# FrozenWolf-Cyber/Indic-CL-ASR

Measured on AMD Instinct MI355X. Metric: utterances/sec (15 s @16 kHz) Conformer-M RNNT-CTC+EWC train step, higher is better.
Workload: dtype bf16; 1 GPU; BASELINE configs[1]: Conformer-medium (d=256, 16L, H=640) hybrid RNNT-CTC + EWC, bs=32/GPU x 15 s, bf16 projections, freeze_encoder_till=12, 22x257 heads, fused_batch_size=4; global_batch=32, parallelism=dp1

## Files before the change

### include/indicasr.h

```cpp
#ifndef INDICASR_H
#define INDICASR_H

#include <stddef.h>
#include <stdint.h>

#ifdef __cplusplus
extern "C" {
#endif

typedef void* ia_stream_t;

enum ia_status {
    IA_OK = 0,
    IA_INVALID_VALUE = -1,
    IA_WORKSPACE_TOO_SMALL = -2,
    IA_LAUNCH_FAILED = -3,
    IA_UNSUPPORTED = -4,
};

const char* ia_version(void);

size_t ia_rnnt_workspace_bytes(int B, int T, int U1);
int ia_rnnt_loss(const float* logits, const int64_t* labels, const int64_t* act_lens, const int64_t* label_lens,
                 int B, int T, int U1, int V, int blank, float fastemit_lambda, float clamp,
                 float* costs, float* grads, void* workspace, size_t workspace_bytes, ia_stream_t stream);
int ia_rnnt_forward(const float* logits, const int64_t* labels, const int64_t* act_lens, const int64_t* label_lens,
                    int B, int T, int U1, int V, int blank, float fastemit_lambda, int need_backward, float* costs,
                    void* workspace, size_t workspace_bytes, ia_stream_t stream);
int ia_rnnt_backward(const float* logits, const int64_t* labels, const int64_t* act_lens, const int64_t* label_lens,
                     int B, int T, int U1, int V, int blank, float fastemit_lambda, float clamp,
                     const float* cost_grad, float* grads, void* workspace, size_t workspace_bytes, ia_stream_t stream,
                     void* grad_kernel_start_event, void* grad_kernel_stop_event);
int ia_rnnt_export_alphas_betas(const void* workspace, size_t workspace_bytes, const int64_t* act_lens,
                                const int64_t* label_lens, int B, int T, int U1, float* alphas, float* betas,
                                ia_stream_t stream);

int ia_joint_ld(int V);
int ia_joint_fwd(const void* f, const void* g, const void* W, const float* bias, const int64_t* labels,
                 const int64_t* act_lens, const int64_t* label_lens, int B, int T, int U1, int H, int V, int blank,
                 float dropout_p, unsigned seed, void* logits, int LD, void* workspace, size_t workspace_bytes,
                 ia_stream_t stream);
int ia_joint_fwd_box(const void* f, const void* g, const void* W, const float* bias, const int64_t* labels,
                     const int64_t* act_lens, const int64_t* label_lens, const int64_t* box_t, const int64_t* box_u, int B,
                     int T, int U1, int H, int V, int blank, float dropout_p, unsigned seed, void* logits, int LD,
                     void* workspace, size_t workspace_bytes, ia_stream_t stream);
int64_t ia_joint_extra_scratch_elems(void);
int ia_joint_extra_reduce(const void* logits, const void* teacher, const int64_t* box_t, const int64_t* box_u,
                          const float* w_sq, const float* w_kd, int B, int T, int U1, int V, int LD, float* sums4,
                          float* scratch, ia_stream_t stream);
int ia_joint_extra_grad(const void* logits, const void* teacher, const int64_t* box_t, const int64_t* box_u, const float* w_sq,
                        const float* w_kd, const float* upstream2, int B, int T, int U1, int V, int LD, void* E,
                        ia_stream_t stream);
int ia_lattice_add_f16(void* G, const void* E, int64_t n, ia_stream_t stream);
int ia_rnnt_lattice(const int64_t* act_lens, const int64_t* label_lens, int B, int T, int U1, float fastemit_lambda,
                    int need_backward, float* costs, void* workspace, size_t workspace_bytes, ia_stream_t stream);
int ia_joint_backward_g(void* logits_inout, const int64_t* labels, const int64_t* act_lens, const int64_t* label_lens,
                        int B, int T, int U1, int V, int LD, int blank, float fastemit_lambda, const float* cost_grad,
                        float kappa, void* gt_out, int S, int Kc, float* dbias_out, float* dbias_scratch, void* workspace,
                        size_t workspace_bytes, ia_stream_t stream, void* grad_kernel_start_event,
                        void* grad_kernel_stop_event);
int ia_joint_backward_g_skip(void* logits_inout, const int64_t* labels, const int64_t* act_lens, const int64_t* label_lens, int B,
                             int T, int U1, int V, int LD, int blank, float fastemit, const float* cost_grad, float kappa,
                             void* gt_out, int S, int Kc, float* dbias_out, float* dbias_scratch, void* workspace,
                             size_t workspace_bytes, int skip_dead_frames, ia_stream_t stream, void* ev_start, void* ev_stop);
int64_t ia_joint_backward_g_dbias_scratch_elems(int LD);
int ia_joint_hidden_t(const void* f, const void* g, void* hidden_t, int B, int T, int U1, int H, int LDH, int S, int Kc,
                      float dropout_p, unsigned seed, ia_stream_t stream);
int ia_joint_hidden(const void* f, const void* g, void* hidden, int B, int T, int U1, int H, int LDH, float dropout_p,
                    unsigned seed, ia_stream_t stream);
int ia_joint_dh_reduce(const void* dh, const void* f, const void* g, const int64_t* act_lens,
                       const int64_t* label_lens, float* df, float* dg, int B, int T, int U1, int H, float inv_kappa,
                       float dropout_p, unsigned seed, void* scratch, ia_stream_t stream);
size_t ia_joint_dh_reduce_scratch_bytes(int B, int T, int U1, int H);
int ia_joint_dh_fused_supported(int U1, int H, int LD);
int ia_joint_dh_k(void);
size_t ia_joint_dh_fused_scratch_bytes(int B, int T, int U1, int H);
int ia_joint_dh_fused(const void* G, const void* Wt, const void* f, const void* g, const int64_t* act_lens,
                      const int64_t* label_lens, float* df, float* dg, int B, int T, int U1, int H, int LD,
                      float inv_kappa, float dropout_p, unsigned seed, void* scratch, ia_stream_t stream);
int ia_joint_dh_fused_ex(const void* G, const void* Wt, const void* f, const void* g, const int64_t* act_lens,
                         const int64_t* label_lens, float* df, float* dg, void* df_bf16, void* dg_bf16, int zero_dead_df, int B,
                         int T, int U1, int H, int LD, float inv_kappa, float dropout_p, unsigned seed, void* scratch,
                         ia_stream_t stream);
int ia_joint_dw_fused_supported(int U1, int H, int LD);
int64_t ia_joint_dw_fused_scratch_elems(int B, int T, int U1, int H, int LD);
int ia_joint_dw_fused(const void* G, const void* f, const void* g, const int64_t* act_lens, int B, int T, int U1, int H, int LD,
                      float dropout_p, unsigned seed, float* dW, float* scratch, ia_stream_t stream);
int ia_joint_dw_fused_ex(const void* G, const void* f, const void* g, const int64_t* act_lens, const int64_t* label_lens, int B,
                         int T, int U1, int H, int LD, float dropout_p, unsigned seed, float* dW, float* scratch,
                         ia_stream_t stream);

int ia_gemm_bf16(const void* A, int lda, const void* W, int ldw, int M, int N, int K, const float* bias, int act,
                 float dropout_p, unsigned seed, float alpha, const float* R, int ldr, float* outF, int ldof,
                 void* outH, int ldoh, ia_stream_t stream);
int ia_gemm_bf16_ex(const void* A, int lda, const void* W, int ldw, int M, int N, int K, const float* bias, int act,
                    float dropout_p, unsigned seed, float alpha, const float* R, int ldr, float* outF, int ldof, void* outH,
                    int ldoh, void* out_pre, int ldpre, const void* aux, int ldaux, ia_stream_t stream);
int ia_gemm_bf16_ex2(const void* A, int lda, const void* W, int ldw, int M, int N, int K, const float* bias, int act,
                     float dropout_p, unsigned seed, float alpha, const float* R, int ldr, float* outF, int ldof, void* outH,
                     int ldoh, void* out_pre, int ldpre, const void* aux, int ldaux, int flags, ia_stream_t stream);
int ia_quantize_mxfp8(const void* x, int is_f32, int ld, int64_t M, int K, void* q, int ldq, void* scales, int lds, ia_stream_t stream);
int ia_gemm_mxfp8(const void* Aq, int lda, const void* a_scales, int ldsa, const void* Wq, int ldw, const void* w_scales, int ldsw,
                  int M, int N, int K, const float* bias, int act, float dropout_p, unsigned seed, float alpha, const float* R, int ldr,
                  float* outF, int ldof, void* outH, int ldoh, ia_stream_t stream);

int ia_greedy_decode_lds_bytes(int Hp, int Hj, int V);
int ia_greedy_rnnt_decode(const float* f_all, const int64_t* out_len, const float* EW, const float* Whh, const float* Wpred,
                          const float* bpred, const float* Whead, const float* bhead, int B, int T, int Hp, int Hj, int V,
                          int blank, int row_blank, int row_sos, int max_symbols, int* tokens, int cap, int* counts,
                          int* overflow, ia_stream_t stream);
int ia_greedy_rnnt_decode_bf16w(const float* f_all, const int64_t* out_len, const float* EW, const void* Whh_bf16,
                                const void* Wpred_bf16, const float* bpred, const void* Whead_bf16, const float* bhead, int B, int T,
                                int Hp, int Hj, int V, int blank, int row_blank, int row_sos, int max_symbols, int* tokens, int cap,
                                int* counts, int* overflow, ia_stream_t stream);
size_t ia_greedy_decode_scratch_bytes(int B, int Hp, int Hj);
int ia_greedy_decode_cluster(int B, int Hp, int Hj);
int ia_greedy_rnnt_decode_bf16w_ex(const float* f_all, const int64_t* out_len, const float* EW, const void* Whh_bf16,
                                   const void* Wpred_bf16, const float* bpred, const void* Whead_bf16, const float* bhead, int B,
                                   int T, int Hp, int Hj, int V, int blank, int row_blank, int row_sos, int max_symbols, int* tokens,
                                   int cap, int* counts, int* overflow, int cluster, void* scratch, size_t scratch_bytes,
                                   ia_stream_t stream);

int ia_edit_distance_batch(const int32_t* a, const int64_t* a_off, const int32_t* b, const int64_t* b_off, int n, int64_t* out);

int ia_quantize_fp8_rows(const void* x, int is_f32, int ld, int64_t M, int K, void* q, int ldq, float* scale, ia_stream_t stream);
int ia_gemm_fp8(const void* Aq, int lda, const float* a_scale, const void* Wq, int ldw, const float* w_scale, int M, int N, int K,
                const float* bias, int act, float dropout_p, unsigned seed, float alpha, const float* R, int ldr, float* outF,
                int ldof, void* outH, int ldoh, ia_stream_t stream);
int ia_subsample_conv1(const float* feats, int B, int Fm, int Tm, int C, const float* w1, const float* b1, void* out,
                       ia_stream_t stream);
int ia_subsample_conv2(const void* in_cl, int B, int T1, int F1, int C, const void* w2r, const float* b2, int N, void* out,
                       ia_stream_t stream);
int ia_gemm_bf16_ln_supported(int N, int K);
int ia_gemm_bf16_ln(const void* A, int lda, const void* W, int ldw, int M, int N, int K, const float* bias, float dropout_p,
                    unsigned seed, float alpha, const float* R, int ldr, float* outF, int ldof, const float* ln_g,
                    const float* ln_b, float ln_eps, void* outH, int ldoh, ia_stream_t stream);
int ia_layernorm(const float* x, int ldx, int N, int d, const float* g1, const float* b1, float eps, float* outF,
                 int ldf, const float* g2, const float* b2, void* outH, int ldh, ia_stream_t stream);
int ia_glu_dwconv(const void* x2, const int64_t* lens, int B, int T, int d, int ksz, const float* w, const float* bias,
                  float* z, float* bn_sum, float* bn_sumsq, float* scratch, ia_stream_t stream);
int64_t ia_dwconv_scratch_elems(int B, int T, int d, int ksz);
int ia_colsum_bf16(const void* x, int M, int N, int ld, float* out, ia_stream_t stream);
int ia_dwconv_time(const float* x, int B, int T, int d, int ksz, const float* w, const float* bias, int flip, float* y,
                   ia_stream_t stream);
int ia_dwconv_time_wgrad(const float* x, const float* dy, int B, int T, int d, int ksz, float* dw, float* db,
                         float* scratch, ia_stream_t stream);
int ia_dwconv_glu_bwd(const float* dz, const void* c2, const int64_t* lens, int B, int T, int d, int ksz, const float* w, void* dc2,
                      ia_stream_t stream);
int ia_dwconv_glu_wgrad(const void* c2, const int64_t* lens, const float* dy, int B, int T, int d, int ksz, float* dw, float* db,
                        float* scratch, ia_stream_t stream);
int ia_bn_silu(const float* z, int64_t n_rows, int d, const float* bn_sum, const float* bn_sumsq, const float* gamma,
               const float* beta, float* running_mean, float* running_var, int64_t* num_batches_tracked,
               float momentum, float eps, int training, void* out, ia_stream_t stream);

int ia_gemm_bnsilu_supported(int K);
int ia_gemm_bnsilu_bf16(const float* z, int ldz, int64_t n_rows, const float* bn_sum, const float* bn_sumsq,
                        const float* gamma, const float* beta, float* running_mean, float* running_var,
                        int64_t* num_batches_tracked, float momentum, float eps, int training, const void* W, int ldw, int M,
                        int N, int K, const float* bias, float dropout_p, unsigned seed, float alpha, const float* R, int ldr,
                        float* outF, int ldof, void* outH, int ldoh, const long long* bn_sums_fixed, ia_stream_t stream);
int ia_gemm_bnsilu_bf16_keep(const float* z, int ldz, int64_t n_rows, const float* bn_sum, const float* bn_sumsq,
                             const float* gamma, const float* beta, float* running_mean, float* running_var,
                             int64_t* num_batches_tracked, float momentum, float eps, int training, const void* W, int ldw, int M,
                             int N, int K, const float* bias, float dropout_p, unsigned seed, float alpha, const float* R, int ldr,
                             float* outF, int ldof, void* outH, int ldoh, const long long* bn_sums_fixed, void* outA, int ldoa,
                             ia_stream_t stream);
int ia_dwconv_gated_fixed(const void* g, const int64_t* lens, int B, int T, int d, int ksz, const float* w, const float* bias,
                          float* z, long long* bn_sums_fixed, ia_stream_t stream);
int ia_glu_dwconv_fixed(const void* x2, const int64_t* lens, int B, int T, int d, int ksz, const float* w, const float* bias,
                        float* z, long long* bn_sums_fixed, ia_stream_t stream);

int ia_relpos_attention_flash_supported(int T, int dk);
int ia_relpos_attention_flash(const void* qkv, const void* pos_proj, const float* bias_u, const float* bias_v,
                              const int64_t* lens, int B, int T, int H, int dk, float dropout_p, unsigned seed, void* ctx,
                              ia_stream_t stream);
int ia_relpos_attention_flash_lse(const void* qkv, const void* pos_proj, const float* bias_u, const float* bias_v,
                                  const int64_t* lens, int B, int T, int H, int dk, float dropout_p, unsigned seed, void* ctx,
                                  float* lse, ia_stream_t stream);
int ia_relpos_attention_local_supported(int T, int dk, int window);
int ia_relpos_attention_local(const void* qkv, const void* pos_proj, const float* bias_u, const float* bias_v,
                              const int64_t* lens, int B, int T, int H, int dk, int window, float dropout_p, unsigned seed,
                              void* ctx, ia_stream_t stream);
int ia_relpos_attention_local_lse(const void* qkv, const void* pos_proj, const float* bias_u, const float* bias_v,
                                  const int64_t* lens, int B, int T, int H, int dk, int window, float dropout_p, unsigned seed,
                                  void* ctx, float* lse, ia_stream_t stream);
int ia_relpos_attention_flash_bwd_dims(int T, int* Rs, int* pad0);
int64_t ia_relpos_attention_flash_bwd_ws_elems(int B, int T, int H, int dk);
int ia_relpos_attention_flash_bwd(const void* qkv, const void* pos_proj, const float* bias_u, const float* bias_v,
                                  const int64_t* lens, const void* ctx, const void* dctx, const float* lse, int B, int T, int H,
                                  int dk, float dropout_p, unsigned seed, void* dqkv, void* dpl, int pl_rows, float* dbias_u,
                                  float* dbias_v, void* dBand, void* QvHM, float* ws, ia_stream_t stream);
int ia_relpos_attention_local_bwd_dims(int T, int window, int* Rs, int* pad0);
int64_t ia_relpos_attention_local_bwd_ws_elems(int B, int T, int H, int dk, int window);
int ia_relpos_attention_local_bwd(const void* qkv, const void* pos_proj, const float* bias_u, const float* bias_v,
                                  const int64_t* lens, const void* ctx, const void* dctx, const float* lse, int B, int T, int H,
                                  int dk, int window, float dropout_p, unsigned seed, void* dqkv, void* dpl, int pl_rows,
                                  float* dbias_u, float* dbias_v, void* dBand, void* QvHM, float* ws, ia_stream_t stream);
int ia_relpos_attention_context_supported(int T, int dk, int style, int left, int right);
int ia_relpos_attention_context(const void* qkv, const void* pos_proj, const float* bias_u, const float* bias_v,
                                const int64_t* lens, int B, int T, int H, int dk, int style, int left, int right,
                                float dropout_p, unsigned seed, void* ctx, ia_stream_t stream);
int ia_relpos_attention_context_lse(const void* qkv, const void* pos_proj, const float* bias_u, const float* bias_v,
                                    const int64_t* lens, int B, int T, int H, int dk, int style, int left, int right,
                                    float dropout_p, unsigned seed, void* ctx, float* lse, ia_stream_t stream);
int ia_relpos_attention_context_bwd_dims(int T, int style, int left, int right, int* Rs, int* pad0);
int64_t ia_relpos_attention_context_bwd_ws_elems(int B, int T, int H, int dk, int style, int left, int right);
int ia_relpos_attention_context_bwd(const void* qkv, const void* pos_proj, const float* bias_u, const float* bias_v,
                                    const int64_t* lens, const void* ctx, const void* dctx, const float* lse, int B, int T, int H,
                                    int dk, int style, int left, int right, float dropout_p, unsigned seed, void* dqkv, void* dpl,
                                    int pl_rows, float* dbias_u, float* dbias_v, void* dBand, void* QvHM, float* ws,
                                    ia_stream_t stream);
size_t ia_attn_vt_elems(int B, int T, int H);
int ia_relpos_attention(const void* qkv, const void* pos_proj, const float* bias_u, const float* bias_v,
                        const int64_t* lens, int B, int T, int H, int dk, float dropout_p, unsigned seed,
                        void* vt_scratch, void* ctx, ia_stream_t stream);

size_t ia_lstm_scratch_bytes(int B, int H);
int ia_lstm_lds_bytes(int H, int backward);
int ia_lstm_forward(const float* Gx, const void* Whh_bf16, float* Hout, float* gates, float* Cs, int U, int B, int H,
                    void* scratch, size_t scratch_bytes, ia_stream_t stream);
int ia_lstm_backward(const float* dHout, const float* gates, const float* Cs, const void* WhhT_bf16, float* dG, int U,
                     int B, int H, void* scratch, size_t scratch_bytes, ia_stream_t stream);

int ia_feat_frames(const float* audio, int B, int L, int Tm, int win, int n_fft, int hop, float preemph, float dither,
                   unsigned seed, float* frames, int ldf, ia_stream_t stream);
int ia_gemm_f32(const float* A, int lda, const float* W, int ldw, int M, int N, int K, float* C, int ldc,
                ia_stream_t stream);
int ia_feat_power(const float* spec, int64_t M, int lds, int half, int nbins, float* power, int ldp, ia_stream_t stream);
int ia_feat_logmel_t(const float* mel, int B, int Tm, int F, int ldm, float guard, float* out, ia_stream_t stream);
int ia_feat_preemph(const float* audio, int B, int L, float preemph, float dither, unsigned seed, float* y,
                    ia_stream_t stream);
int ia_feat_logmel_fft_supported(int n_fft, int win, int n_mels, int n_chunks);
int ia_feat_logmel_fft(const float* y, int B, int L, int Tm, const float* window, int win, int n_fft, int hop,
                       const float* twiddle, const int* chunk_start, const float* chunk_vals, const int* filt_chunks,
                       int n_mels, int n_chunks, float guard, float* out, ia_stream_t stream);
int ia_feat_normalize(const float* x, const int64_t* seq_len, int B, int F, int T, float eps, const int* freq_starts,
                      const int* freq_widths, int n_freq_masks, const int* time_starts, const int* time_widths,
                      int n_time_masks, float mask_value, float* y, ia_stream_t stream);

size_t ia_ctc_workspace_bytes(int B, int T, int S);
int ia_ctc_forward(const float* log_probs, const int64_t* targets, const int64_t* input_lens, const int64_t* target_lens,
                   int B, int T, int V, int S, int blank, int zero_infinity, float* nll, void* workspace,
                   size_t workspace_bytes, ia_stream_t stream);
int ia_ctc_backward(const float* log_probs, const int64_t* targets, const int64_t* input_lens, const int64_t* target_lens,
                    int B, int T, int V, int S, int blank, const float* nll_grad, float* grad, void* workspace,
                    size_t workspace_bytes, ia_stream_t stream);

typedef struct ia_tn_problem {
    const void* dY; const void* X; float* dW; float* db;
    int ldy, ldx, M, n, k;
} ia_tn_problem;
int64_t ia_gemm_tn_grouped_scratch_elems(const ia_tn_problem* problems, int count);
int ia_gemm_tn_bf16_grouped(const ia_tn_problem* problems, int count, float* scratch, ia_stream_t stream);
int64_t ia_gemm_tn_scratch_elems(int M, int n, int k);
int ia_gemm_tn_bf16(const void* dY, int ldy, const void* X, int ldx, int M, int n, int k, float* dW, float* db,
                    float* scratch, ia_stream_t stream);

int ia_ffn_fused_supported(int d, int d_ff);
int ia_ffn_fused(float* x, int N, int d, int d_ff, const float* ln_g, const float* ln_b, float eps, const void* W1,
                 const float* b1, const void* W2, const float* b2, float alpha, float p_ff, unsigned seed_ff, float p_res,
                 unsigned seed_res, const float* ln2_g, const float* ln2_b, void* y_out, int ln2_to_y_only,
                 ia_stream_t stream);
int ia_ffn_fused_tail_supported(int d, int d_ff, int nt);
int ia_ffn_fused_tail(float* x, int N, int d, int d_ff, const float* ln_g, const float* ln_b, float eps, const void* W1,
                      const float* b1, const void* W2, const float* b2, float alpha, float p_ff, unsigned seed_ff, float p_res,
                      unsigned seed_res, const float* ln2_g, const float* ln2_b, void* y_out, int ln2_to_y_only, const void* Wt,
                      const float* bt, void* t_out, int nt, ia_stream_t stream);

typedef struct ia_block_params {
    const void *w_ff1a, *w_ff1b, *w_qkv, *w_pos, *w_out, *w_pw1, *w_pw2, *w_ff2a, *w_ff2b;
    const float *b_ff1a, *b_ff1b, *b_qkv, *b_out, *b_pw1, *b_pw2, *b_ff2a, *b_ff2b;
    const float *ln_ff1_g, *ln_ff1_b, *ln_att_g, *ln_att_b, *ln_conv_g, *ln_conv_b, *ln_ff2_g, *ln_ff2_b, *ln_out_g, *ln_out_b;
    const float *pos_u, *pos_v, *dw_w, *dw_b, *bn_g, *bn_b;
    float *bn_rm, *bn_rv;
    int64_t* bn_nbt;
    float ln_eps, bn_eps, bn_momentum, p_drop, p_ff, p_att, fc_factor;
    int d, d_ff, n_heads, ksz;
    const void* pl_cached;
    const void* w_pw1_glu;
    const float* b_pw1_glu;
    int att_window;
    int att_style;
    int att_left, att_right;
} ia_block_params;
size_t ia_conformer_prefix_ws_bytes(int B, int T, int d, int d_ff, int H, int ksz, int pos_rows);
int ia_conformer_prefix_fwd(const ia_block_params* layers, int n_layers, float* x, const void* pos_emb, int pos_rows,
                            const int64_t* lens, int B, int T, unsigned seed_base, unsigned seed_stride, int training,
                            void* workspace, size_t workspace_bytes, ia_stream_t stream);
size_t ia_conformer_prefix_ws_sums_offset(int B, int T, int d, int d_ff, int H, int ksz, int pos_rows);
int ia_conformer_prefix_fwd_seg(const ia_block_params* layers, int n_layers, float* x, const void* pos_emb, int pos_rows,
                                const int64_t* lens, int B, int T, unsigned seed_base, unsigned seed_stride, int training,
                                int seg_begin, int seg_end, int bn_synced, void* workspace, size_t workspace_bytes,
                                ia_stream_t stream);

typedef struct ia_block_saved {
    void *y1, *h1p, *h1; float* x1;
    void *y2, *qkv, *pl, *ctxv; float* x2;
    void *y3, *c2; float *z, *sums; void* c3; float* x3;
    void *y4, *h4p, *h4; float* x4;
    float* lse;
} ia_block_saved;
typedef struct ia_block_grads {
    float *w_ff1a, *b_ff1a, *w_ff1b, *b_ff1b, *w_qkv, *b_qkv, *w_pos, *w_out, *b_out, *w_pw1, *b_pw1, *w_pw2, *b_pw2;
    float *w_ff2a, *b_ff2a, *w_ff2b, *b_ff2b;
    float *ln_ff1_g, *ln_ff1_b, *ln_att_g, *ln_att_b, *ln_conv_g, *ln_conv_b, *ln_ff2_g, *ln_ff2_b, *ln_out_g, *ln_out_b;
    float *dw_w, *dw_b, *bn_g, *bn_b;
} ia_block_grads;
struct ia_block_params;
int ia_conformer_block_supported(int d, int d_ff, int H, int ksz, int T);
size_t ia_conformer_block_bwd_ws_bytes(int B, int T, int d, int d_ff, int ksz);
int ia_conformer_block_fwd(const struct ia_block_params* layer, const float* x0, const void* pos_emb, int pos_rows,
                           const int64_t* lens, int B, int T, unsigned seed, const ia_block_saved* saved, float* out,
                           float* dw_scratch, ia_stream_t stream);
int ia_conformer_block_bwd_a(const struct ia_block_params* layer, const ia_block_saved* saved, const ia_block_grads* grads,
                             const float* dout, const int64_t* lens, int B, int T, unsigned seed, void* workspace,
                             size_t workspace_bytes, float** dx2_out, void** dctx_out, ia_stream_t stream);
int ia_conformer_block_fwd_phase(const struct ia_block_params* layer, const float* x0, const void* pos_emb, int pos_rows,
                                 const int64_t* lens, int B, int T, unsigned seed, const ia_block_saved* saved, float* out,
                                 float* dw_scratch, int phase, ia_stream_t stream);
int ia_conformer_block_bwd_a_phase(const struct ia_block_params* layer, const ia_block_saved* saved, const ia_block_grads* grads,
                                   const float* dout, const int64_t* lens, int B, int T, unsigned seed, void* workspace,
                                   size_t workspace_bytes, float** dx2_out, void** dctx_out, int phase, const float* bn_S12,
                                   ia_stream_t stream);
int ia_conformer_block_bwd_b(const struct ia_block_params* layer, const ia_block_saved* saved, const ia_block_grads* grads,
                             const float* x0, const void* pos_emb, int pos_rows, const void* dqkv, const void* dpl, int B,
                             int T, unsigned seed, void* workspace, size_t workspace_bytes, float* dx0,
                             const void* add_table, int n_add, ia_stream_t stream);

int ia_layernorm_bwd(const float* x, int ldx, const float* dy_f32, const void* dy_bf16, int ldy, int N, int d,
                     const float* gamma, float eps, const float* dx_in, float* dx_out, int lddx, float* dgamma,
                     float* dbeta, float* scratch, ia_stream_t stream);
int ia_layernorm_bwd_drop(const float* x, int ldx, const float* dy_f32, const void* dy_bf16, int ldy, int N, int d,
                          const float* gamma, float eps, const float* dx_in, float* dx_out, int lddx, float* dgamma,
                          float* dbeta, float alpha, float dropout_p, unsigned seed, void* dx_bf16, int lddxh, float* scratch,
                          ia_stream_t stream);
typedef struct ia_finish_job { const float* part; int G, C, C0; float* out0; float* out1; } ia_finish_job;
int ia_layernorm_bwd_partial_rows(int N);
int ia_partials_finish_multi(const ia_finish_job* jobs, int count, ia_stream_t stream);
int64_t ia_layernorm_bwd_scratch_elems(int N, int d);
int ia_silu_dropout(const void* h_pre, int64_t M, int N, float dropout_p, unsigned seed, void* out, ia_stream_t stream);
int ia_silu_dropout_bwd(const void* h_pre, const void* dh, int64_t M, int N, float dropout_p, unsigned seed, void* out,
                        ia_stream_t stream);
int ia_scale_dropout_bf16(const float* dy, int64_t M, int N, float alpha, float dropout_p, unsigned seed, void* out,
                          ia_stream_t stream);
int ia_cast_pad_bf16(const float* src, int lds, int64_t M, int N, void* dst, int ldd, ia_stream_t stream);
int ia_bn_silu_bwd(const float* z, const void* dc3, int64_t n_rows, int d, const float* bn_sum, const float* bn_sumsq,
                   const float* gamma, const float* beta, float eps, float* S1, float* S2, float* dz, float* scratch,
                   ia_stream_t stream);
int64_t ia_bn_silu_bwd_scratch_elems(int64_t n_rows, int d);
int ia_bn_sync_finish(float* sums_and_count, int d, int64_t n_local_rows, float* running_mean, float* running_var,
                      int64_t* num_batches_tracked, float momentum, ia_stream_t stream);
int ia_bn_silu_bwd_reduce(const float* z, const void* dc3, int64_t n_rows, int d, const float* bn_sum, const float* bn_sumsq,
                          const float* gamma, const float* beta, float eps, float* S1, float* S2, float* scratch,
                          ia_stream_t stream);
int ia_bn_silu_bwd_apply(const float* z, const void* dc3, int64_t n_rows, int d, const float* bn_sum, const float* bn_sumsq,
                         const float* gamma, const float* beta, float eps, const float* S1, const float* S2, float* dz,
                         ia_stream_t stream);
int ia_glu_mask(const void* c2, const int64_t* lens, int B, int T, int d, float* G, ia_stream_t stream);
int ia_glu_bwd(const void* c2, const float* dG, const int64_t* lens, int B, int T, int d, void* dc2, ia_stream_t stream);

int ia_cl_chunk_elems(void);
int ia_cl_penalty(const float* theta, const float* theta_star, const float* weight, float coef, float* grad,
                  int accumulate, const int32_t* chunk_table, int nchunks, const float* seg_inv_numel,
                  float* seg_abs_mean, float* penalty_sum, ia_stream_t stream);
int ia_cl_fisher_accumulate(float* fisher, const float* grad, const float* loss_scalar, int64_t n, ia_stream_t stream);
int ia_cl_abs_accumulate(float* omega, const float* grad, int64_t n, ia_stream_t stream);
int ia_adamw_step(float* theta, const float* grad, float* exp_avg, float* exp_avg_sq, int64_t n, float lr, float beta1,
                  float beta2, float eps, float weight_decay, int step, float grad_scale, void* shadow_bf16,
                  ia_stream_t stream);
int ia_adamw_step_segmented(float* theta, const float* grad, float* exp_avg, float* exp_avg_sq, const int32_t* chunk_table,
                            int nchunks, int32_t* seg_active, int32_t* seg_step, int nseg, int all_active, float lr,
                            float beta1, float beta2, float eps, float weight_decay, float grad_scale, void* shadow_bf16,
                            ia_stream_t stream);
size_t ia_grad_norm_workspace_bytes(int nchunks);
int ia_grad_norm(const float* grad, const int32_t* chunk_table, int nchunks, const int32_t* seg_chunk_begin, int nseg,
                 float grad_scale, float max_norm, int32_t* seg_active, float* seg_norm, float* norm_state, void* workspace,
                 size_t workspace_bytes, ia_stream_t stream);
int ia_adamw_step_segmented_clipped(float* theta, const float* grad, float* exp_avg, float* exp_avg_sq,
                                    const int32_t* chunk_table, int nchunks, int32_t* seg_active, int32_t* seg_step, int nseg,
                                    int all_active, float lr, float beta1, float beta2, float eps, float weight_decay,
                                    float grad_scale, void* shadow_bf16, const float* norm_state, int skip_nonfinite,
                                    int32_t* counters, ia_stream_t stream);
int ia_adamw_step_segmented_si(float* theta, const float* grad, float* exp_avg, float* exp_avg_sq, const int32_t* chunk_table,
                               int nchunks, int32_t* seg_active, int32_t* seg_step, int nseg, int all_active, float lr,
                               float beta1, float beta2, float eps, float weight_decay, float grad_scale, void* shadow_bf16,
                               const float* norm_state, int skip_nonfinite, int32_t* counters, float* path_w,
                               const float* omega, const float* theta_star, float penalty_coef, ia_stream_t stream);
int ia_si_consolidate(const float* theta, float* theta_star, float* path_w, float* omega, float xi, int64_t n,
                      ia_stream_t stream);
int ia_adamw_step_segmented_rwalk(float* theta, const float* grad, float* exp_avg, float* exp_avg_sq,
                                  const int32_t* chunk_table, int nchunks, int32_t* seg_active, int32_t* seg_step, int nseg,
                                  int all_active, float beta1, float beta2, float eps, float grad_scale, void* shadow_bf16,
                                  const int32_t* seg_group, int ngroups, const float* group_lr, const float* group_weight_decay,
                                  const float* norm_state, int skip_nonfinite, int32_t* counters, float* fisher, float* path_w,
                                  float* anchor, float* score, const float* importance, const float* theta_star,
                                  float penalty_coef, float alpha, float fold_eps, int fold, ia_stream_t stream);
size_t ia_rwalk_workspace_bytes(int nchunks);
int ia_rwalk_consolidate(const float* theta, float* theta_star, const float* fisher, float* path_w, float* anchor, float* score,
                         float* score_acc, float* importance, float* maxima, float fold_eps, int normalize, int first, int64_t n,
                         const int32_t* chunk_table, int nchunks, void* workspace, size_t workspace_bytes, ia_stream_t stream);
size_t ia_agem_workspace_bytes(int nchunks);
int ia_agem_dots(const float* grad, const float* ref, const int32_t* chunk_table, int nchunks, int nseg, float grad_scale,
                 int32_t* seg_active, float* proj_state, void* workspace, size_t workspace_bytes, ia_stream_t stream);
int ia_grad_norm_projected(const float* grad, const int32_t* chunk_table, int nchunks, const int32_t* seg_chunk_begin, int nseg,
                           float grad_scale, float max_norm, const int32_t* seg_active, float* seg_norm, float* norm_state,
                           void* workspace, size_t workspace_bytes, const float* ref, const float* proj_state,
                           ia_stream_t stream);
int ia_adamw_step_segmented_projected(float* theta, const float* grad, float* exp_avg, float* exp_avg_sq,
                                      const int32_t* chunk_table, int nchunks, int32_t* seg_active, int32_t* seg_step, int nseg,
                                      int all_active, float lr, float beta1, float beta2, float eps, float weight_decay,
                                      float grad_scale, void* shadow_bf16, const float* norm_state, int skip_nonfinite,
                                      int32_t* counters, const float* ref, const float* proj_state, int32_t* proj_counters,
                                      ia_stream_t stream);
#define IA_GEM_MAX_TASKS 16
#define IA_GEM_STATE_FLOATS 20
#define IA_GEM_SUMS_DOUBLES 272
size_t ia_gem_workspace_bytes(int nchunks, int max_tasks);
int ia_gem_dots(const float* x, const float* refs, int64_t stride, int ntasks, const int32_t* chunk_table, int nchunks, int nseg,
                float grad_scale, int32_t* seg_active, int gram_row, double* gem_sums, void* workspace, size_t workspace_bytes,
                ia_stream_t stream);
int ia_gem_solve(const double* gem_sums, float* gem_state, int ntasks, float memory_strength, float eps, ia_stream_t stream);
int ia_grad_norm_gem(const float* grad, const int32_t* chunk_table, int nchunks, const int32_t* seg_chunk_begin, int nseg,
                     float grad_scale, float max_norm, const int32_t* seg_active, float* seg_norm, float* norm_state,
                     void* workspace, size_t workspace_bytes, const float* refs, int64_t stride, int ntasks,
                     const float* gem_state, ia_stream_t stream);
int ia_adamw_step_segmented_gem(float* theta, const float* grad, float* exp_avg, float* exp_avg_sq, const int32_t* chunk_table,
                                int nchunks, int32_t* seg_active, int32_t* seg_step, int nseg, int all_active, float beta1,
                                float beta2, float eps, float grad_scale, void* shadow_bf16, const int32_t* seg_group, int ngroups,
                                const float* group_lr, const float* group_weight_decay, const float* norm_state,
                                int skip_nonfinite, int32_t* counters, const float* refs, int64_t stride, int ntasks,
                                const float* gem_state, int32_t* gem_counters, ia_stream_t stream);
#define IA_OGD_MAX_ROWS 4096
size_t ia_ogd_workspace_bytes(int nchunks, int max_rows);
int ia_ogd_dots(const float* x, const float* basis, int64_t stride, int64_t numel, int nrows, const int32_t* chunk_table,
                int nchunks, int nseg, const int32_t* seg_scope, int32_t* seg_active, int with_sq, double* dots64,
                float* dots32, void* workspace, size_t workspace_bytes, ia_stream_t stream);
int ia_ogd_project(const float* x, const float* basis, int64_t stride, int64_t numel, int nrows, const float* coef, float alpha,
                   const int32_t* chunk_table, int nchunks, int nseg, const int32_t* seg_scope, const int32_t* seg_active,
                   float* dst, ia_stream_t stream);
#define IA_MAX_PARAM_GROUPS 64
int ia_adamw_step_segmented_grouped(float* theta, const float* grad, float* exp_avg, float* exp_avg_sq,
                                    const int32_t* chunk_table, int nchunks, int32_t* seg_active, int32_t* seg_step, int nseg,
                                    int all_active, float beta1, float beta2, float eps, float grad_scale, void* shadow_bf16,
                                    const int32_t* seg_group, int ngroups, const float* group_lr,
                                    const float* group_weight_decay, const float* norm_state, int skip_nonfinite,
                                    int32_t* counters, float* path_w, const float* omega, const float* theta_star,
                                    float penalty_coef, const float* ref, const float* proj_state, int32_t* proj_counters,
                                    ia_stream_t stream);
#define IA_MASK_FREE 0
#define IA_MASK_MASKED 1
#define IA_MASK_FROZEN 2
int ia_adamw_step_segmented_masked(float* theta, const float* grad, float* exp_avg, float* exp_avg_sq, const int32_t* chunk_table,
                                   int nchunks, int32_t* seg_active, int32_t* seg_step, int nseg, int all_active, float beta1,
                                   float beta2, float eps, float grad_scale, void* shadow_bf16, const int32_t* seg_group,
                                   int ngroups, const float* group_lr, const float* group_weight_decay, const float* norm_state,
                                   int skip_nonfinite, int32_t* counters, const float* base, float* scores,
                                   const int32_t* seg_kind, float threshold, ia_stream_t stream);
int ia_mask_pack(const float* scores, const int32_t* chunk_table, int nchunks, const int32_t* seg_kind, int nseg, float threshold,
                 uint64_t* bits, int64_t nwords, int32_t* seg_kept, ia_stream_t stream);
int ia_mask_apply(float* theta, const float* base, const uint64_t* bits, int64_t nwords, const int32_t* chunk_table, int nchunks,
                  const int32_t* seg_kind, int nseg, void* shadow_bf16, ia_stream_t stream);
int ia_adamw_step_segmented_packed(float* theta, const float* grad, float* exp_avg, float* exp_avg_sq, const int32_t* chunk_table,
                                   int nchunks, int32_t* seg_active, int32_t* seg_step, int nseg, int all_active, float beta1,
                                   float beta2, float eps, float grad_scale, void* shadow_bf16, const int32_t* seg_group,
                                   int ngroups, const float* group_lr, const float* group_weight_decay, const float* norm_state,
                                   int skip_nonfinite, int32_t* counters, const uint8_t* owner, const int32_t* seg_kind,
                                   int train_owner, ia_stream_t stream);
int ia_grad_norm_packed(const float* grad, const int32_t* chunk_table, int nchunks, const int32_t* seg_chunk_begin, int nseg,
                        float grad_scale, float max_norm, int32_t* seg_active, float* seg_norm, float* norm_state,
                        void* workspace, size_t workspace_bytes, const uint8_t* owner, const int32_t* seg_kind, int train_owner,
                        ia_stream_t stream);
size_t ia_pack_prune_workspace_bytes(int nseg);
int ia_pack_prune(float* theta, float* exp_avg, float* exp_avg_sq, uint8_t* owner, const int32_t* chunk_table, int nchunks,
                  const int32_t* seg_kind, int nseg, float fraction, int task, void* shadow_bf16, int32_t* seg_counts,
                  void* workspace, size_t workspace_bytes, ia_stream_t stream);
int ia_pack_apply(float* theta, const float* base, const uint8_t* owner, const int32_t* chunk_table, int nchunks,
                  const int32_t* seg_kind, int nseg, int lo, int hi, void* shadow_bf16, ia_stream_t stream);
#define IA_LORA_MAX_RANK 64
int ia_lora_tile_rows(void);
int ia_lora_tile_cols(void);
size_t ia_lora_workspace_bytes(int64_t m, int64_t n, int rank);
int ia_lora_grad(const float* grad, const float* factors, float* factor_grad, const int64_t* tensors, int ntensors,
                 const int32_t* tiles, int ntiles, const int32_t* factor_chunk_table, int nfchunks, int rank, float scale,
                 float grad_scale, const float* norm_state, int skip_nonfinite, int all_active, int32_t* factor_active,
                 void* workspace, size_t workspace_bytes, size_t workspace_needed, ia_stream_t stream);
int ia_lora_apply(float* theta, const float* base, const float* factors, const int64_t* tensors, int ntensors,
                  const int32_t* seg_tensor, const int32_t* chunk_table, int nchunks, int nseg, int rank, float scale,
                  void* shadow_bf16, const float* norm_state, int skip_nonfinite, ia_stream_t stream);
int ia_adamw_step_segmented_kinds(float* theta, const float* grad, float* exp_avg, float* exp_avg_sq, const int32_t* chunk_table,
                                  int nchunks, int32_t* seg_active, int32_t* seg_step, int nseg, int all_active, float beta1,
                                  float beta2, float eps, float grad_scale, void* shadow_bf16, const int32_t* seg_group,
                                  int ngroups, const float* group_lr, const float* group_weight_decay, const float* norm_state,
                                  int skip_nonfinite, int32_t* counters, const int32_t* seg_kind, int flags_preset,
                                  ia_stream_t stream);
#define IA_MERGE_MAX_TASKS 32
int ia_merge_linear(float* theta, const float* base, const float* vectors, int64_t stride, int ntasks, const float* coef,
                    float scale, const int32_t* chunk_table, int nchunks, void* shadow_bf16, ia_stream_t stream);
size_t ia_merge_trim_workspace_bytes(int ntasks, int nscope);
int ia_merge_trim(const float* vectors, int64_t stride, int ntasks, const int32_t* chunk_table, int nchunks,
                  const int32_t* seg_of_scope, int nscope, float trim, uint32_t* cutoffs, void* workspace,
                  size_t workspace_bytes, ia_stream_t stream);
int ia_merge_ties(float* theta, const float* base, const float* vectors, int64_t stride, int ntasks, const uint32_t* cutoffs,
                  const int32_t* seg_of_scope, int nscope, float scale, const int32_t* chunk_table, int nchunks, int nseg,
                  void* shadow_bf16, int32_t* seg_counts, ia_stream_t stream);
int ia_merge_fisher(float* theta, const float* base, const float* vectors, const float* importances, int64_t stride, int ntasks,
                    const float* coef, float floor, float scale, const int32_t* chunk_table, int nchunks, int nseg,
                    void* shadow_bf16, int32_t* seg_counts, ia_stream_t stream);
int ia_merge_linear_dare(float* theta, const float* base, const float* vectors, int64_t stride, int ntasks, const float* coef,
                         float scale, const int32_t* chunk_table, int nchunks, void* shadow_bf16, uint32_t seed,
                         uint32_t keep_threshold, float keep_prob, ia_stream_t stream);
int ia_merge_ties_dare(float* theta, const float* base, const float* vectors, int64_t stride, int ntasks, float scale,
                       const int32_t* chunk_table, int nchunks, int nseg, void* shadow_bf16, int32_t* seg_counts, uint32_t seed,
                       uint32_t keep_threshold, float keep_prob, ia_stream_t stream);

typedef struct ia_wave_params {
    int32_t n_in, n_out;
    int32_t new_sr;
    int32_t shift_pre, shift_post;
    int32_t noise_shift, noise_stage;
    uint32_t noise_seed;
    float gain, noise_amp;
    int32_t pad[2];
} ia_wave_params;
int ia_wave_augment_tile(void);
int ia_wave_augment(const float* x, int B, int L_in, float* y, int L_out, const ia_wave_params* params, const float* table,
                    int zero_crossings, int sr, int min_new_sr, ia_stream_t stream);

int ia_ctc_row_lse(const float* logits, int ld, int64_t M, int V, float* lse, ia_stream_t stream);
int ia_ctc_forward_logits(const float* logits, int ld, const float* lse, const int64_t* targets, const int64_t* input_lens,
                          const int64_t* target_lens, int B, int T, int V, int S, int blank, int zero_infinity, float* nll,
                          void* workspace, size_t workspace_bytes, ia_stream_t stream);
int ia_ctc_backward_logits(const float* logits, int ld, const float* lse, const int64_t* targets, const int64_t* input_lens,
                           const int64_t* target_lens, int B, int T, int V, int S, int blank, const float* nll_grad,
                           float grad_scale, void* grad_bf16, int ldg, void* workspace, size_t workspace_bytes, ia_stream_t stream);

int ia_ctc_align_max_targets(void);
size_t ia_ctc_align_workspace_bytes(int B, int T, int S);
int ia_ctc_align(const float* lp, int ld, const float* lse, const int64_t* targets, const int64_t* input_lens,
                 const int64_t* target_lens, int B, int T, int V, int S, int blank, int32_t* path, int32_t* spans, float* score,
                 void* workspace, size_t workspace_bytes, ia_stream_t stream);

int ia_ctc_beam_max_width(void);
size_t ia_ctc_beam_workspace_bytes(int B, int T, int V, int W);
int ia_ctc_beam_search(const float* x, const float* lse, const int64_t* in_lens, int B, int T, int ld, int V, int blank, int W,
                       float token_min_logp, int32_t* tokens, int32_t* lengths, float* scores, void* workspace,
                       size_t workspace_bytes, ia_stream_t stream);

typedef struct ia_ngram_lm {
    const int32_t* states; const float* backoff; const int32_t* arcs; const float* arc_logp; const float* uni_logp;
    const int32_t* uni_next;
    int32_t n_states, n_arcs, n_tokens, order, start; float unk_logp;
} ia_ngram_lm;
int ia_ctc_beam_lm_max_order(void);
size_t ia_ctc_beam_lm_workspace_bytes(int B, int T, int V, int W);
int ia_ctc_beam_search_lm(const float* x, const float* lse, const int64_t* in_lens, int B, int T, int ld, int V, int blank, int W,
                          float token_min_logp, const ia_ngram_lm* lm, float alpha, float beta, int32_t* tokens, int32_t* lengths,
                          float* scores, void* workspace, size_t workspace_bytes, ia_stream_t stream);

typedef struct ia_axpy_row {
    float* dst; const float* src; long long n; float scale; int pad;
} ia_axpy_row;
typedef struct ia_tr_job { const void* in; void* out; int rows, cols; } ia_tr_job;
int ia_transpose16_multi(const ia_tr_job* jobs_host, int njobs, ia_stream_t stream);
int ia_swap01_cast(const void* in, int in_bf16, int n0, int n1, int H, void* out, int out_bf16, ia_stream_t stream);
int ia_select_rows_cast(const float* W, int ldw, const float* bias, int row0, int nrows, int extra_row, int K, int rows_out,
                        float scale, int out_f16, void* out, void* outT, int ldt, float* bias_out, ia_stream_t stream);
int ia_rows_scatter_add(float* dst, int ldd, const float* src, int lds, int row0, int nrows, int extra_row, int K, float scale,
                        float* bias_dst, const float* bias_src, ia_stream_t stream);
int ia_loss_combine(const float* costs, const float* nll, int B, float ctc_weight, const int* flag0, const int* flag1,
                    const int* flag2, const int* flag3, float* out4, float* total, ia_stream_t stream);
int ia_loss_combine_bwd(const float* gout, int B, float ctc_weight, float* g_costs, float* g_nll, ia_stream_t stream);
int ia_embed_sos(const float* E, const int64_t* tokens, int B, int U, int H, int n_rows, int time_major, int out_bf16, void* out,
                 ia_stream_t stream);
int ia_embed_sos_bwd(const void* dX, int dx_bf16, const int64_t* tokens, int B, int U, int H, int n_rows, int pad_row,
                     int time_major, float scale, float* dE, ia_stream_t stream);
int ia_multi_axpy(const ia_axpy_row* rows_host, int nrows, int max_blocks_per_row, ia_stream_t stream);

int ia_peak_stream_copy(const void* src, void* dst, size_t bytes, ia_stream_t stream);
int ia_peak_mfma_bf16(float* sink, int workgroups, int iters, ia_stream_t stream);
double ia_peak_mfma_bf16_flops(int workgroups, int iters);

#ifdef __cplusplus
}
#endif
#endif
```

### indic_cl_asr_amd/_lib.py

```python
import ctypes
import os
import subprocess

_HERE = os.path.dirname(os.path.abspath(__file__))
LIB_PATH = os.environ.get("IA_LIB_PATH") or os.path.join(_HERE, "libindicasr_hip.so")

IA_OK = 0
_STATUS = {-1: "IA_INVALID_VALUE", -2: "IA_WORKSPACE_TOO_SMALL", -3: "IA_LAUNCH_FAILED", -4: "IA_UNSUPPORTED"}

_c = ctypes
_vp, _i, _f, _sz = _c.c_void_p, _c.c_int, _c.c_float, _c.c_size_t
_i64 = _c.c_int64

class BlockParams(_c.Structure):
    _fields_ = ([(n, _c.c_void_p) for n in (
        "w_ff1a", "w_ff1b", "w_qkv", "w_pos", "w_out", "w_pw1", "w_pw2", "w_ff2a", "w_ff2b",
        "b_ff1a", "b_ff1b", "b_qkv", "b_out", "b_pw1", "b_pw2", "b_ff2a", "b_ff2b",
        "ln_ff1_g", "ln_ff1_b", "ln_att_g", "ln_att_b", "ln_conv_g", "ln_conv_b", "ln_ff2_g", "ln_ff2_b", "ln_out_g", "ln_out_b",
        "pos_u", "pos_v", "dw_w", "dw_b", "bn_g", "bn_b", "bn_rm", "bn_rv", "bn_nbt")]
        + [(n, _c.c_float) for n in ("ln_eps", "bn_eps", "bn_momentum", "p_drop", "p_ff", "p_att", "fc_factor")]
        + [(n, _c.c_int) for n in ("d", "d_ff", "n_heads", "ksz")]
        + [("pl_cached", _c.c_void_p), ("w_pw1_glu", _c.c_void_p), ("b_pw1_glu", _c.c_void_p), ("att_window", _c.c_int),
           ("att_style", _c.c_int), ("att_left", _c.c_int), ("att_right", _c.c_int)])


class BlockSaved(_c.Structure):
    _fields_ = [(n, _c.c_void_p) for n in ("y1", "h1p", "h1", "x1", "y2", "qkv", "pl", "ctxv", "x2", "y3", "c2", "z", "sums",
                                           "c3", "x3", "y4", "h4p", "h4", "x4", "lse")]


class TnProblem(_c.Structure):
    _fields_ = [("dY", _c.c_void_p), ("X", _c.c_void_p), ("dW", _c.c_void_p), ("db", _c.c_void_p),
                ("ldy", _c.c_int), ("ldx", _c.c_int), ("M", _c.c_int), ("n", _c.c_int), ("k", _c.c_int)]


class BlockGrads(_c.Structure):
    _fields_ = [(n, _c.c_void_p) for n in (
        "w_ff1a", "b_ff1a", "w_ff1b", "b_ff1b", "w_qkv", "b_qkv", "w_pos", "w_out", "b_out", "w_pw1", "b_pw1", "w_pw2", "b_pw2",
        "w_ff2a", "b_ff2a", "w_ff2b", "b_ff2b",
        "ln_ff1_g", "ln_ff1_b", "ln_att_g", "ln_att_b", "ln_conv_g", "ln_conv_b", "ln_ff2_g", "ln_ff2_b", "ln_out_g", "ln_out_b",
        "dw_w", "dw_b", "bn_g", "bn_b")]


class NGramLM(_c.Structure):
    _fields_ = ([(n, _c.c_void_p) for n in ("states", "backoff", "arcs", "arc_logp", "uni_logp", "uni_next")]
                + [(n, _c.c_int32) for n in ("n_states", "n_arcs", "n_tokens", "order", "start")] + [("unk_logp", _c.c_float)])


class WaveParams(_c.Structure):
    _fields_ = ([(n, _c.c_int32) for n in ("n_in", "n_out", "new_sr", "shift_pre", "shift_post", "noise_shift", "noise_stage")]
                + [("noise_seed", _c.c_uint32), ("gain", _c.c_float), ("noise_amp", _c.c_float), ("pad", _c.c_int32 * 2)])


SIGNATURES = {
    "ia_version": (_c.c_char_p, []),
    "ia_wave_augment_tile": (_i, []),
    "ia_wave_augment": (_i, [_vp, _i, _i, _vp, _i, _vp, _vp, _i, _i, _i, _vp]),
    "ia_gemm_bf16_ex2": (_i, [_vp, _i, _vp, _i, _i, _i, _i, _vp, _i, _f, _c.c_uint, _f, _vp, _i, _vp, _i, _vp, _i, _vp, _i, _vp, _i, _i, _vp]),
    "ia_transpose16_multi": (_i, [_vp, _i, _vp]),
    "ia_swap01_cast": (_i, [_vp, _i, _i, _i, _i, _vp, _i, _vp]),
    "ia_ctc_row_lse": (_i, [_vp, _i, _i64, _i, _vp, _vp]),
    "ia_ctc_forward_logits": (_i, [_vp, _i, _vp, _vp, _vp, _vp, _i, _i, _i, _i, _i, _i, _vp, _vp, _sz, _vp]),
    "ia_ctc_backward_logits": (_i, [_vp, _i, _vp, _vp, _vp, _vp, _i, _i, _i, _i, _i, _vp, _f, _vp, _i, _vp, _sz, _vp]),
    "ia_select_rows_cast": (_i, [_vp, _i, _vp, _i, _i, _i, _i, _i, _f, _i, _vp, _vp, _i, _vp, _vp]),
    "ia_rows_scatter_add": (_i, [_vp, _i, _vp, _i, _i, _i, _i, _i, _f, _vp, _vp, _vp]),
    "ia_loss_combine": (_i, [_vp, _vp, _i, _f, _vp, _vp, _vp, _vp, _vp, _vp, _vp]),
    "ia_loss_combine_bwd": (_i, [_vp, _i, _f, _vp, _vp, _vp]),
    "ia_embed_sos": (_i, [_vp, _vp, _i, _i, _i, _i, _i, _i, _vp, _vp]),
    "ia_embed_sos_bwd": (_i, [_vp, _i, _vp, _i, _i, _i, _i, _i, _i, _f, _vp, _vp]),
    "ia_multi_axpy": (_i, [_vp, _i, _i, _vp]),
    "ia_peak_stream_copy": (_i, [_vp, _vp, _sz, _vp]),
    "ia_peak_mfma_bf16": (_i, [_vp, _i, _i, _vp]),
    "ia_peak_mfma_bf16_flops": (_c.c_double, [_i, _i]),
    "ia_rnnt_workspace_bytes": (_sz, [_i, _i, _i]),
    "ia_rnnt_loss": (_i, [_vp, _vp, _vp, _vp, _i, _i, _i, _i, _i, _f, _f, _vp, _vp, _vp, _sz, _vp]),
    "ia_rnnt_forward": (_i, [_vp, _vp, _vp, _vp, _i, _i, _i, _i, _i, _f, _i, _vp, _vp, _sz, _vp]),
    "ia_rnnt_backward": (_i, [_vp, _vp, _vp, _vp, _i, _i, _i, _i, _i, _f, _f, _vp, _vp, _vp, _sz, _vp, _vp, _vp]),
    "ia_rnnt_export_alphas_betas": (_i, [_vp, _sz, _vp, _vp, _i, _i, _i, _vp, _vp, _vp]),
    "ia_joint_ld": (_i, [_i]),
    "ia_joint_fwd": (_i, [_vp, _vp, _vp, _vp, _vp, _vp, _vp, _i, _i, _i, _i, _i, _i, _f, _c.c_uint, _vp, _i, _vp, _sz, _vp]),
    "ia_joint_fwd_box": (_i, [_vp, _vp, _vp, _vp, _vp, _vp, _vp, _vp, _vp, _i, _i, _i, _i, _i, _i, _f, _c.c_uint, _vp, _i, _vp, _sz, _vp]),
    "ia_joint_extra_scratch_elems": (_i64, []),
    "ia_joint_extra_reduce": (_i, [_vp, _vp, _vp, _vp, _vp, _vp, _i, _i, _i, _i, _i, _vp, _vp, _vp]),
    "ia_joint_extra_grad": (_i, [_vp, _vp, _vp, _vp, _vp, _vp, _vp, _i, _i, _i, _i, _i, _vp, _vp]),
    "ia_lattice_add_f16": (_i, [_vp, _vp, _i64, _vp]),
    "ia_relpos_attention_flash_lse": (_i, [_vp, _vp, _vp, _vp, _vp, _i, _i, _i, _i, _f, _c.c_uint, _vp, _vp, _vp]),
    "ia_relpos_attention_flash_bwd_dims": (_i, [_i, _c.POINTER(_c.c_int), _c.POINTER(_c.c_int)]),
    "ia_relpos_attention_flash_bwd_ws_elems": (_i64, [_i, _i, _i, _i]),
    "ia_relpos_attention_flash_bwd": (_i, [_vp, _vp, _vp, _vp, _vp, _vp, _vp, _vp, _i, _i, _i, _i, _f, _c.c_uint, _vp, _vp, _i, _vp,
                                           _vp, _vp, _vp, _vp, _vp]),
    "ia_relpos_attention_local_lse": (_i, [_vp, _vp, _vp, _vp, _vp, _i, _i, _i, _i, _i, _f, _c.c_uint, _vp, _vp, _vp]),
    "ia_relpos_attention_local_bwd_dims": (_i, [_i, _i, _c.POINTER(_c.c_int), _c.POINTER(_c.c_int)]),
    "ia_relpos_attention_local_bwd_ws_elems": (_i64, [_i, _i, _i, _i, _i]),
    "ia_relpos_attention_local_bwd": (_i, [_vp, _vp, _vp, _vp, _vp, _vp, _vp, _vp, _i, _i, _i, _i, _i, _f, _c.c_uint, _vp, _vp, _i, _vp,
                                           _vp, _vp, _vp, _vp, _vp]),
    "ia_relpos_attention_context_lse": (_i, [_vp, _vp, _vp, _vp, _vp, _i, _i, _i, _i, _i, _i, _i, _f, _c.c_uint, _vp, _vp, _vp]),
    "ia_relpos_attention_context_bwd_dims": (_i, [_i, _i, _i, _i, _c.POINTER(_c.c_int), _c.POINTER(_c.c_int)]),
    "ia_relpos_attention_context_bwd_ws_elems": (_i64, [_i, _i, _i, _i, _i, _i, _i]),
    "ia_relpos_attention_context_bwd": (_i, [_vp, _vp, _vp, _vp, _vp, _vp, _vp, _vp, _i, _i, _i, _i, _i, _i, _i, _f, _c.c_uint, _vp, _vp,
                                             _i, _vp, _vp, _vp, _vp, _vp, _vp]),
    "ia_quantize_fp8_rows": (_i, [_vp, _i, _i, _i64, _i, _vp, _i, _vp, _vp]),
    "ia_gemm_fp8": (_i, [_vp, _i, _vp, _vp, _i, _vp, _i, _i, _i, _vp, _i, _f, _c.c_uint, _f, _vp, _i, _vp, _i, _vp, _i, _vp]),
    "ia_gemm_tn_grouped_scratch_elems": (_i64, [_vp, _i]),
    "ia_gemm_tn_bf16_grouped": (_i, [_vp, _i, _vp, _vp]),
    "ia_greedy_decode_lds_bytes": (_i, [_i, _i, _i]),
    "ia_greedy_rnnt_decode": (_i, [_vp, _vp, _vp, _vp, _vp, _vp, _vp, _vp, _i, _i, _i, _i, _i, _i, _i, _i, _i, _vp, _i, _vp, _vp, _vp]),
    "ia_greedy_rnnt_decode_bf16w": (_i, [_vp, _vp, _vp, _vp, _vp, _vp, _vp, _vp, _i, _i, _i, _i, _i, _i, _i, _i, _i, _vp, _i, _vp, _vp, _vp]),
    "ia_edit_distance_batch": (_i, [_vp, _vp, _vp, _vp, _i, _vp]),
    "ia_greedy_decode_scratch_bytes": (_sz, [_i, _i, _i]),
    "ia_greedy_decode_cluster": (_i, [_i, _i, _i]),
    "ia_greedy_rnnt_decode_bf16w_ex": (_i, [_vp, _vp, _vp, _vp, _vp, _vp, _vp, _vp, _i, _i, _i, _i, _i, _i, _i, _i, _i, _vp, _i, _vp, _vp, _i, _vp, _sz, _vp]),
    "ia_quantize_mxfp8": (_i, [_vp, _i, _i, _i64, _i, _vp, _i, _vp, _i, _vp]),
    "ia_gemm_mxfp8": (_i, [_vp, _i, _vp, _i, _vp, _i, _vp, _i, _i, _i, _i, _vp, _i, _f, _c.c_uint, _f, _vp, _i, _vp, _i, _vp, _i, _vp]),
    "ia_cast_pad_bf16": (_i, [_vp, _i, _i64, _i, _vp, _i, _vp]),
    "ia_rnnt_lattice": (_i, [_vp, _vp, _i, _i, _i, _f, _i, _vp, _vp, _sz, _vp]),
    "ia_joint_backward_g": (_i, [_vp, _vp, _vp, _vp, _i, _i, _i, _i, _i, _i, _f, _vp, _f, _vp, _i, _i, _vp, _vp, _vp, _sz, _vp, _vp,
                                 _vp]),
    "ia_joint_backward_g_skip": (_i, [_vp, _vp, _vp, _vp, _i, _i, _i, _i, _i, _i, _f, _vp, _f, _vp, _i, _i, _vp, _vp, _vp, _sz, _i, _vp,
                                      _vp, _vp]),
    "ia_joint_backward_g_dbias_scratch_elems": (_i64, [_i]),
    "ia_joint_hidden_t": (_i, [_vp, _vp, _vp, _i, _i, _i, _i, _i, _i, _i, _f, _c.c_uint, _vp]),
    "ia_joint_hidden": (_i, [_vp, _vp, _vp, _i, _i, _i, _i, _i, _f, _c.c_uint, _vp]),
    "ia_joint_dh_reduce": (_i, [_vp, _vp, _vp, _vp, _vp, _vp, _vp, _i, _i, _i, _i, _f, _f, _c.c_uint, _vp, _vp]),
    "ia_joint_dh_reduce_scratch_bytes": (_sz, [_i, _i, _i, _i]),
    "ia_joint_dh_fused_supported": (_i, [_i, _i, _i]),
    "ia_joint_dh_k": (_i, []),
    "ia_joint_dh_fused": (_i, [_vp, _vp, _vp, _vp, _vp, _vp, _vp, _vp, _i, _i, _i, _i, _i, _f, _f, _c.c_uint, _vp, _vp]),
    "ia_joint_dh_fused_ex": (_i, [_vp, _vp, _vp, _vp, _vp, _vp, _vp, _vp, _vp, _vp, _i, _i, _i, _i, _i, _i, _f, _f, _c.c_uint, _vp, _vp]),
    "ia_joint_dh_fused_scratch_bytes": (_sz, [_i, _i, _i, _i]),
    "ia_joint_dw_fused_supported": (_i, [_i, _i, _i]),
    "ia_joint_dw_fused_scratch_elems": (_i64, [_i, _i, _i, _i, _i]),
    "ia_joint_dw_fused": (_i, [_vp, _vp, _vp, _vp, _i, _i, _i, _i, _i, _f, _c.c_uint, _vp, _vp, _vp]),
    "ia_gemm_bf16_ln_supported": (_i, [_i, _i]),
    "ia_gemm_bf16_ln": (_i, [_vp, _i, _vp, _i, _i, _i, _i, _vp, _f, _c.c_uint, _f, _vp, _i, _vp, _i, _vp, _vp, _f, _vp, _i, _vp]),
    "ia_joint_dw_fused_ex": (_i, [_vp, _vp, _vp, _vp, _vp, _i, _i, _i, _i, _i, _f, _c.c_uint, _vp, _vp, _vp]),
    "ia_gemm_bf16": (_i, [_vp, _i, _vp, _i, _i, _i, _i, _vp, _i, _f, _c.c_uint, _f, _vp, _i, _vp, _i, _vp, _i, _vp]),
    "ia_gemm_bf16_ex": (_i, [_vp, _i, _vp, _i, _i, _i, _i, _vp, _i, _f, _c.c_uint, _f, _vp, _i, _vp, _i, _vp, _i, _vp, _i, _vp, _i, _vp]),
    "ia_subsample_conv1": (_i, [_vp, _i, _i, _i, _i, _vp, _vp, _vp, _vp]),
    "ia_subsample_conv2": (_i, [_vp, _i, _i, _i, _i, _vp, _vp, _i, _vp, _vp]),
    "ia_layernorm": (_i, [_vp, _i, _i, _i, _vp, _vp, _f, _vp, _i, _vp, _vp, _vp, _i, _vp]),
    "ia_glu_dwconv": (_i, [_vp, _vp, _i, _i, _i, _i, _vp, _vp, _vp, _vp, _vp, _vp, _vp]),
    "ia_dwconv_scratch_elems": (_i64, [_i, _i, _i, _i]),
    "ia_colsum_bf16": (_i, [_vp, _i, _i, _i, _vp, _vp]),
    "ia_dwconv_time": (_i, [_vp, _i, _i, _i, _i, _vp, _vp, _i, _vp, _vp]),
    "ia_dwconv_time_wgrad": (_i, [_vp, _vp, _i, _i, _i, _i, _vp, _vp, _vp, _vp]),
    "ia_dwconv_glu_bwd": (_i, [_vp, _vp, _vp, _i, _i, _i, _i, _vp, _vp, _vp]),
    "ia_dwconv_glu_wgrad": (_i, [_vp, _vp, _vp, _i, _i, _i, _i, _vp, _vp, _vp, _vp]),
    "ia_bn_silu": (_i, [_vp, _i64, _i, _vp, _vp, _vp, _vp, _vp, _vp, _vp, _f, _f, _i, _vp, _vp]),
    "ia_gemm_bnsilu_supported": (_i, [_i]),
    "ia_gemm_bnsilu_bf16": (_i, [_vp, _i, _i64, _vp, _vp, _vp, _vp, _vp, _vp, _vp, _f, _f, _i, _vp, _i, _i, _i, _i, _vp, _f, _c.c_uint, _f,
                                 _vp, _i, _vp, _i, _vp, _i, _vp, _vp]),
    "ia_gemm_bnsilu_bf16_keep": (_i, [_vp, _i, _i64, _vp, _vp, _vp, _vp, _vp, _vp, _vp, _f, _f, _i, _vp, _i, _i, _i, _i, _vp, _f, _c.c_uint,
                                      _f, _vp, _i, _vp, _i, _vp, _i, _vp, _vp, _i, _vp]),
    "ia_glu_dwconv_fixed": (_i, [_vp, _vp, _i, _i, _i, _i, _vp, _vp, _vp, _vp, _vp]),
    "ia_dwconv_gated_fixed": (_i, [_vp, _vp, _i, _i, _i, _i, _vp, _vp, _vp, _vp, _vp]),
    "ia_attn_vt_elems": (_sz, [_i, _i, _i]),
    "ia_relpos_attention": (_i, [_vp, _vp, _vp, _vp, _vp, _i, _i, _i, _i, _f, _c.c_uint, _vp, _vp, _vp]),
    "ia_relpos_attention_flash_supported": (_i, [_i, _i]),
    "ia_relpos_attention_flash": (_i, [_vp, _vp, _vp, _vp, _vp, _i, _i, _i, _i, _f, _c.c_uint, _vp, _vp]),
    "ia_relpos_attention_local_supported": (_i, [_i, _i, _i]),
    "ia_relpos_attention_context_supported": (_i, [_i, _i, _i, _i, _i]),
    "ia_relpos_attention_context": (_i, [_vp, _vp, _vp, _vp, _vp, _i, _i, _i, _i, _i, _i, _i, _f, _c.c_uint, _vp, _vp]),
    "ia_relpos_attention_local": (_i, [_vp, _vp, _vp, _vp, _vp, _i, _i, _i, _i, _i, _f, _c.c_uint, _vp, _vp]),
    "ia_lstm_scratch_bytes": (_sz, [_i, _i]),
    "ia_lstm_lds_bytes": (_i, [_i, _i]),
    "ia_lstm_forward": (_i, [_vp, _vp, _vp, _vp, _vp, _i, _i, _i, _vp, _sz, _vp]),
    "ia_lstm_backward": (_i, [_vp, _vp, _vp, _vp, _vp, _i, _i, _i, _vp, _sz, _vp]),
    "ia_feat_frames": (_i, [_vp, _i, _i, _i, _i, _i, _i, _f, _f, _c.c_uint, _vp, _i, _vp]),
    "ia_gemm_f32": (_i, [_vp, _i, _vp, _i, _i, _i, _i, _vp, _i, _vp]),
    "ia_feat_power": (_i, [_vp, _i64, _i, _i, _i, _vp, _i, _vp]),
    "ia_feat_logmel_t": (_i, [_vp, _i, _i, _i, _i, _f, _vp, _vp]),
    "ia_feat_preemph": (_i, [_vp, _i, _i, _f, _f, _c.c_uint, _vp, _vp]),
    "ia_feat_logmel_fft_supported": (_i, [_i, _i, _i, _i]),
    "ia_feat_logmel_fft": (_i, [_vp, _i, _i, _i, _vp, _i, _i, _i, _vp, _vp, _vp, _vp, _i, _i, _f, _vp, _vp]),
    "ia_feat_normalize": (_i, [_vp, _vp, _i, _i, _i, _f, _vp, _vp, _i, _vp, _vp, _i, _f, _vp, _vp]),
    "ia_ctc_workspace_bytes": (_sz, [_i, _i, _i]),
    "ia_ctc_forward": (_i, [_vp, _vp, _vp, _vp, _i, _i, _i, _i, _i, _i, _vp, _vp, _sz, _vp]),
    "ia_ctc_backward": (_i, [_vp, _vp, _vp, _vp, _i, _i, _i, _i, _i, _vp, _vp, _vp, _sz, _vp]),
    "ia_ctc_align_max_targets": (_i, []),
    "ia_ctc_align_workspace_bytes": (_sz, [_i, _i, _i]),
    "ia_ctc_align": (_i, [_vp, _i, _vp, _vp, _vp, _vp, _i, _i, _i, _i, _i, _vp, _vp, _vp, _vp, _sz, _vp]),
    "ia_ctc_beam_max_width": (_i, []),
    "ia_ctc_beam_workspace_bytes": (_sz, [_i, _i, _i, _i]),
    "ia_ctc_beam_search": (_i, [_vp, _vp, _vp, _i, _i, _i, _i, _i, _i, _f, _vp, _vp, _vp, _vp, _sz, _vp]),
    "ia_ctc_beam_lm_max_order": (_i, []),
    "ia_ctc_beam_lm_workspace_bytes": (_sz, [_i, _i, _i, _i]),
    "ia_ctc_beam_search_lm": (_i, [_vp, _vp, _vp, _i, _i, _i, _i, _i, _i, _f, _c.POINTER(NGramLM), _f, _f, _vp, _vp, _vp, _vp, _sz,
                                   _vp]),
    "ia_gemm_tn_scratch_elems": (_i64, [_i, _i, _i]),
    "ia_gemm_tn_bf16": (_i, [_vp, _i, _vp, _i, _i, _i, _i, _vp, _vp, _vp, _vp]),
    "ia_ffn_fused_supported": (_i, [_i, _i]),
    "ia_ffn_fused": (_i, [_vp, _i, _i, _i, _vp, _vp, _f, _vp, _vp, _vp, _vp, _f, _f, _c.c_uint, _f, _c.c_uint, _vp, _vp, _vp, _i, _vp]),
    "ia_ffn_fused_tail_supported": (_i, [_i, _i, _i]),
    "ia_ffn_fused_tail": (_i, [_vp, _i, _i, _i, _vp, _vp, _f, _vp, _vp, _vp, _vp, _f, _f, _c.c_uint, _f, _c.c_uint, _vp, _vp, _vp, _i,
                               _vp, _vp, _vp, _i, _vp]),
    "ia_conformer_prefix_ws_bytes": (_sz, [_i, _i, _i, _i, _i, _i, _i]),
    "ia_conformer_prefix_ws_sums_offset": (_sz, [_i, _i, _i, _i, _i, _i, _i]),
    "ia_conformer_prefix_fwd_seg": (_i, [_vp, _i, _vp, _vp, _i, _vp, _i, _i, _c.c_uint, _c.c_uint, _i, _i, _i, _i, _vp, _sz, _vp]),
    "ia_conformer_prefix_fwd": (_i, [_vp, _i, _vp, _vp, _i, _vp, _i, _i, _c.c_uint, _c.c_uint, _i, _vp, _sz, _vp]),
    "ia_conformer_block_supported": (_i, [_i, _i, _i, _i, _i]),
    "ia_conformer_block_bwd_ws_bytes": (_sz, [_i, _i, _i, _i, _i]),
    "ia_conformer_block_fwd": (_i, [_vp, _vp, _vp, _i, _vp, _i, _i, _c.c_uint, _vp, _vp, _vp, _vp]),
    "ia_conformer_block_fwd_phase": (_i, [_vp, _vp, _vp, _i, _vp, _i, _i, _c.c_uint, _vp, _vp, _vp, _i, _vp]),
    "ia_conformer_block_bwd_a": (_i, [_vp, _vp, _vp, _vp, _vp, _i, _i, _c.c_uint, _vp, _sz, _vp, _vp, _vp]),
    "ia_conformer_block_bwd_a_phase": (_i, [_vp, _vp, _vp, _vp, _vp, _i, _i, _c.c_uint, _vp, _sz, _vp, _vp, _i, _vp, _vp]),
    "ia_conformer_block_bwd_b": (_i, [_vp, _vp, _vp, _vp, _vp, _i, _vp, _vp, _i, _i, _c.c_uint, _vp, _sz, _vp, _vp, _i, _vp]),
    "ia_layernorm_bwd": (_i, [_vp, _i, _vp, _vp, _i, _i, _i, _vp, _f, _vp, _vp, _i, _vp, _vp, _vp, _vp]),
    "ia_layernorm_bwd_drop": (_i, [_vp, _i, _vp, _vp, _i, _i, _i, _vp, _f, _vp, _vp, _i, _vp, _vp, _f, _f, _c.c_uint, _vp, _i, _vp, _vp]),
    "ia_layernorm_bwd_partial_rows": (_i, [_i]),
    "ia_partials_finish_multi": (_i, [_vp, _i, _vp]),
    "ia_layernorm_bwd_scratch_elems": (_i64, [_i, _i]),
    "ia_silu_dropout": (_i, [_vp, _i64, _i, _f, _c.c_uint, _vp, _vp]),
    "ia_silu_dropout_bwd": (_i, [_vp, _vp, _i64, _i, _f, _c.c_uint, _vp, _vp]),
    "ia_scale_dropout_bf16": (_i, [_vp, _i64, _i, _f, _f, _c.c_uint, _vp, _vp]),
    "ia_bn_silu_bwd": (_i, [_vp, _vp, _i64, _i, _vp, _vp, _vp, _vp, _f, _vp, _vp, _vp, _vp, _vp]),
    "ia_bn_silu_bwd_scratch_elems": (_i64, [_i64, _i]),
    "ia_bn_sync_finish": (_i, [_vp, _i, _i64, _vp, _vp, _vp, _f, _vp]),
    "ia_bn_silu_bwd_reduce": (_i, [_vp, _vp, _i64, _i, _vp, _vp, _vp, _vp, _f, _vp, _vp, _vp, _vp]),
    "ia_bn_silu_bwd_apply": (_i, [_vp, _vp, _i64, _i, _vp, _vp, _vp, _vp, _f, _vp, _vp, _vp, _vp]),
    "ia_glu_mask": (_i, [_vp, _vp, _i, _i, _i, _vp, _vp]),
    "ia_glu_bwd": (_i, [_vp, _vp, _vp, _i, _i, _i, _vp, _vp]),
    "ia_cl_chunk_elems": (_i, []),
    "ia_cl_penalty": (_i, [_vp, _vp, _vp, _f, _vp, _i, _vp, _i, _vp, _vp, _vp, _vp]),
    "ia_cl_fisher_accumulate": (_i, [_vp, _vp, _vp, _i64, _vp]),
    "ia_cl_abs_accumulate": (_i, [_vp, _vp, _i64, _vp]),
    "ia_adamw_step": (_i, [_vp, _vp, _vp, _vp, _i64, _f, _f, _f, _f, _f, _i, _f, _vp, _vp]),
    "ia_adamw_step_segmented": (_i, [_vp, _vp, _vp, _vp, _vp, _i, _vp, _vp, _i, _i, _f, _f, _f, _f, _f, _f, _vp, _vp]),
    "ia_grad_norm_workspace_bytes": (_sz, [_i]),
    "ia_grad_norm": (_i, [_vp, _vp, _i, _vp, _i, _f, _f, _vp, _vp, _vp, _vp, _sz, _vp]),
    "ia_adamw_step_segmented_clipped": (_i, [_vp, _vp, _vp, _vp, _vp, _i, _vp, _vp, _i, _i, _f, _f, _f, _f, _f, _f, _vp, _vp, _i,
                                             _vp, _vp]),
    "ia_adamw_step_segmented_si": (_i, [_vp, _vp, _vp, _vp, _vp, _i, _vp, _vp, _i, _i, _f, _f, _f, _f, _f, _f, _vp, _vp, _i,
                                        _vp, _vp, _vp, _vp, _f, _vp]),
    "ia_si_consolidate": (_i, [_vp, _vp, _vp, _vp, _f, _i64, _vp]),
    "ia_adamw_step_segmented_rwalk": (_i, [_vp, _vp, _vp, _vp, _vp, _i, _vp, _vp, _i, _i, _f, _f, _f, _f, _vp, _vp, _i, _vp, _vp,
                                           _vp, _i, _vp, _vp, _vp, _vp, _vp, _vp, _vp, _f, _f, _f, _i, _vp]),
    "ia_rwalk_workspace_bytes": (_sz, [_i]),
    "ia_rwalk_consolidate": (_i, [_vp, _vp, _vp, _vp, _vp, _vp, _vp, _vp, _vp, _f, _i, _i, _i64, _vp, _i, _vp, _sz, _vp]),
    "ia_agem_workspace_bytes": (_sz, [_i]),
    "ia_agem_dots": (_i, [_vp, _vp, _vp, _i, _i, _f, _vp, _vp, _vp, _sz, _vp]),
    "ia_grad_norm_projected": (_i, [_vp, _vp, _i, _vp, _i, _f, _f, _vp, _vp, _vp, _vp, _sz, _vp, _vp, _vp]),
    "ia_adamw_step_segmented_projected": (_i, [_vp, _vp, _vp, _vp, _vp, _i, _vp, _vp, _i, _i, _f, _f, _f, _f, _f, _f, _vp, _vp, _i,
                                               _vp, _vp, _vp, _vp, _vp]),
    "ia_gem_workspace_bytes": (_sz, [_i, _i]),
    "ia_gem_dots": (_i, [_vp, _vp, _i64, _i, _vp, _i, _i, _f, _vp, _i, _vp, _vp, _sz, _vp]),
    "ia_gem_solve": (_i, [_vp, _vp, _i, _f, _f, _vp]),
    "ia_grad_norm_gem": (_i, [_vp, _vp, _i, _vp, _i, _f, _f, _vp, _vp, _vp, _vp, _sz, _vp, _i64, _i, _vp, _vp]),
    "ia_adamw_step_segmented_gem": (_i, [_vp, _vp, _vp, _vp, _vp, _i, _vp, _vp, _i, _i, _f, _f, _f, _f, _vp, _vp, _i, _vp, _vp,
                                         _vp, _i, _vp, _vp, _i64, _i, _vp, _vp, _vp]),
    "ia_ogd_workspace_bytes": (_sz, [_i, _i]),
    "ia_ogd_dots": (_i, [_vp, _vp, _i64, _i64, _i, _vp, _i, _i, _vp, _vp, _i, _vp, _vp, _vp, _sz, _vp]),
    "ia_ogd_project": (_i, [_vp, _vp, _i64, _i64, _i, _vp, _f, _vp, _i, _i, _vp, _vp, _vp, _vp]),
    "ia_adamw_step_segmented_grouped": (_i, [_vp, _vp, _vp, _vp, _vp, _i, _vp, _vp, _i, _i, _f, _f, _f, _f, _vp, _vp, _i, _vp, _vp,
                                             _vp, _i, _vp, _vp, _vp, _vp, _f, _vp, _vp, _vp, _vp]),
    "ia_adamw_step_segmented_masked": (_i, [_vp, _vp, _vp, _vp, _vp, _i, _vp, _vp, _i, _i, _f, _f, _f, _f, _vp, _vp, _i, _vp, _vp,
                                            _vp, _i, _vp, _vp, _vp, _vp, _f, _vp]),
    "ia_mask_pack": (_i, [_vp, _vp, _i, _vp, _i, _f, _vp, _i64, _vp, _vp]),
    "ia_mask_apply": (_i, [_vp, _vp, _vp, _i64, _vp, _i, _vp, _i, _vp, _vp]),
    "ia_adamw_step_segmented_packed": (_i, [_vp, _vp, _vp, _vp, _vp, _i, _vp, _vp, _i, _i, _f, _f, _f, _f, _vp, _vp, _i, _vp, _vp,
                                            _vp, _i, _vp, _vp, _vp, _i, _vp]),
    "ia_grad_norm_packed": (_i, [_vp, _vp, _i, _vp, _i, _f, _f, _vp, _vp, _vp, _vp, _sz, _vp, _vp, _i, _vp]),
    "ia_pack_prune_workspace_bytes": (_sz, [_i]),
    "ia_pack_prune": (_i, [_vp, _vp, _vp, _vp, _vp, _i, _vp, _i, _f, _i, _vp, _vp, _vp, _sz, _vp]),
    "ia_pack_apply": (_i, [_vp, _vp, _vp, _vp, _i, _vp, _i, _i, _i, _vp, _vp]),
    "ia_lora_tile_rows": (_i, []),
    "ia_lora_tile_cols": (_i, []),
    "ia_lora_workspace_bytes": (_sz, [_i64, _i64, _i]),
    "ia_lora_grad": (_i, [_vp, _vp, _vp, _vp, _i, _vp, _i, _vp, _i, _i, _f, _f, _vp, _i, _i, _vp, _vp, _sz, _sz, _vp]),
    "ia_lora_apply": (_i, [_vp, _vp, _vp, _vp, _i, _vp, _vp, _i, _i, _i, _f, _vp, _vp, _i, _vp]),
    "ia_adamw_step_segmented_kinds": (_i, [_vp, _vp, _vp, _vp, _vp, _i, _vp, _vp, _i, _i, _f, _f, _f, _f, _vp, _vp, _i, _vp, _vp,
                                           _vp, _i, _vp, _vp, _i, _vp]),
    "ia_merge_linear": (_i, [_vp, _vp, _vp, _i64, _i, _vp, _f, _vp, _i, _vp, _vp]),
    "ia_merge_trim_workspace_bytes": (_sz, [_i, _i]),
    "ia_merge_trim": (_i, [_vp, _i64, _i, _vp, _i, _vp, _i, _f, _vp, _vp, _sz, _vp]),
    "ia_merge_ties": (_i, [_vp, _vp, _vp, _i64, _i, _vp, _vp, _i, _f, _vp, _i, _i, _vp, _vp, _vp]),
    "ia_merge_fisher": (_i, [_vp, _vp, _vp, _vp, _i64, _i, _vp, _f, _f, _vp, _i, _i, _vp, _vp, _vp]),
    "ia_merge_linear_dare": (_i, [_vp, _vp, _vp, _i64, _i, _vp, _f, _vp, _i, _vp, _c.c_uint32, _c.c_uint32, _f, _vp]),
    "ia_merge_ties_dare": (_i, [_vp, _vp, _vp, _i64, _i, _f, _vp, _i, _i, _vp, _vp, _c.c_uint32, _c.c_uint32, _f, _vp]),
}

_lib = None


def build(verbose=False):
    out = None if verbose else subprocess.DEVNULL
    subprocess.check_call(["make", "-C", os.path.join(_HERE, "csrc")], stdout=out)


def lib():
    global _lib
    if _lib is None:
        if not os.path.exists(LIB_PATH):
            raise RuntimeError(
                f"{LIB_PATH} is missing: the HIP extension is the product path and has no fallback. "
                "Build it with `python -c 'import __graft_entry__ as g; g.build()'` or `make -C indic_cl_asr_amd/csrc`.")
        import torch
        l = ctypes.CDLL(LIB_PATH)
        for name, (res, args) in SIGNATURES.items():
            fn = getattr(l, name)
            fn.restype, fn.argtypes = res, args
        _lib = l
    return _lib


def check(status, what):
    if status != IA_OK:
        raise RuntimeError(f"{what} failed with status {status} ({_STATUS.get(status, 'unknown')})")


def version():
    return lib().ia_version().decode()


def stream_ptr():
    import torch
    return ctypes.c_void_p(torch.cuda.current_stream().cuda_stream)


def ptr(t):
    return ctypes.c_void_p(t.data_ptr()) if t is not None else None
```

### indic_cl_asr_amd/csrc/block_train.hip

```cpp
#include <hip/hip_bf16.h>
#include <hip/hip_runtime.h>

#include <cstdint>

#include <cstdlib>

#include "ia_common.h"

namespace {

inline size_t up256(size_t x) { return (x + 255) / 256 * 256; }

#define IA_TRY(call)                  \
    do {                              \
        const int rc_ = (call);       \
        if (rc_ != IA_OK) return rc_; \
    } while (0)

__global__ __launch_bounds__(256) void transpose_bf16_kernel(const unsigned short* __restrict__ in, int rows, int cols,
                                                             unsigned short* __restrict__ out) {
    __shared__ unsigned short tile[64][72];
    const int tiles_c = (cols + 63) / 64;
    const int tr = blockIdx.x / tiles_c, tc = blockIdx.x - tr * tiles_c;
    const int r0 = tr * 64, c0 = tc * 64;
    for (int i = threadIdx.x; i < 64 * 8; i += 256) {
        const int r = i >> 3, v = i & 7;
        uint4 x = make_uint4(0, 0, 0, 0);
        if (r0 + r < rows && c0 + v * 8 < cols) x = *reinterpret_cast<const uint4*>(in + (size_t)(r0 + r) * cols + c0 + v * 8);
        *reinterpret_cast<uint4*>(&tile[r][v * 8]) = x;
    }
    __syncthreads();
    for (int i = threadIdx.x; i < 64 * 8; i += 256) {
        const int c = i >> 3, v = i & 7;
        if (c0 + c < cols && r0 + v * 8 < rows) {
            union { uint4 u; unsigned short h[8]; } o;
#pragma unroll
            for (int j = 0; j < 8; ++j) o.h[j] = tile[v * 8 + j][c];
            *reinterpret_cast<uint4*>(out + (size_t)(c0 + c) * rows + r0 + v * 8) = o.u;
        }
    }
}

int transpose_bf16(const void* in, int rows, int cols, void* out, hipStream_t st) {
    if (rows % 8 != 0 || cols % 8 != 0) return IA_UNSUPPORTED;
    const int grid = ((rows + 63) / 64) * ((cols + 63) / 64);
    hipLaunchKernelGGL(transpose_bf16_kernel, dim3(grid), dim3(256), 0, st, (const unsigned short*)in, rows, cols, (unsigned short*)out);
    IA_RETURN_IF_LAUNCH_FAILED();
    return IA_OK;
}

struct TrJob { const unsigned short* in; unsigned short* out; int rows, cols, tile_begin, tiles_c; };
struct TrJobs { TrJob j[8]; int count; };
__global__ __launch_bounds__(256) void transpose_bf16_multi_kernel(TrJobs jobs) {
    __shared__ unsigned short tile[64][72];
    int ji = 0;
#pragma unroll
    for (int i = 1; i < 8; ++i)
        if (i < jobs.count && (int)blockIdx.x >= jobs.j[i].tile_begin) ji = i;
    const TrJob& J = jobs.j[ji];
    const int local = blockIdx.x - J.tile_begin;
    const int tr = local / J.tiles_c, tc = local - tr * J.tiles_c;
    const int r0 = tr * 64, c0 = tc * 64, rows = J.rows, cols = J.cols;
    for (int i = threadIdx.x; i < 64 * 8; i += 256) {
        const int r = i >> 3, v = i & 7;
        uint4 x = make_uint4(0, 0, 0, 0);
        if (r0 + r < rows && c0 + v * 8 < cols) x = *reinterpret_cast<const uint4*>(J.in + (size_t)(r0 + r) * cols + c0 + v * 8);
        *reinterpret_cast<uint4*>(&tile[r][v * 8]) = x;
    }
    __syncthreads();
    for (int i = threadIdx.x; i < 64 * 8; i += 256) {
        const int c = i >> 3, v = i & 7;
        if (c0 + c < cols && r0 + v * 8 < rows) {
            union { uint4 u; unsigned short h[8]; } o;
#pragma unroll
            for (int j = 0; j < 8; ++j) o.h[j] = tile[v * 8 + j][c];
            *reinterpret_cast<uint4*>(J.out + (size_t)(c0 + c) * rows + r0 + v * 8) = o.u;
        }
    }
}
struct TrList { TrJobs jobs; int tiles; };
inline void tr_add(TrList* l, const void* in, int rows, int cols, void* out) {
    TrJob& J = l->jobs.j[l->jobs.count++];
    J.in = (const unsigned short*)in; J.out = (unsigned short*)out; J.rows = rows; J.cols = cols;
    J.tile_begin = l->tiles; J.tiles_c = (cols + 63) / 64;
    l->tiles += ((rows + 63) / 64) * J.tiles_c;
}
int tr_launch(const TrList& l, hipStream_t st) {
    for (int i = 0; i < l.jobs.count; ++i)
        if (l.jobs.j[i].rows % 8 != 0 || l.jobs.j[i].cols % 8 != 0) return IA_UNSUPPORTED;
    hipLaunchKernelGGL(transpose_bf16_multi_kernel, dim3(l.tiles), dim3(256), 0, st, l.jobs);
    IA_RETURN_IF_LAUNCH_FAILED();
    return IA_OK;
}

struct AddRow { float* dst; const float* src; int64_t n; };
__global__ __launch_bounds__(256) void multi_add_kernel(const AddRow* __restrict__ table, int rows) {
    for (int k = blockIdx.y; k < rows; k += gridDim.y) {
        const AddRow r = table[k];
        const int64_t n4 = ((reinterpret_cast<uintptr_t>(r.dst) | reinterpret_cast<uintptr_t>(r.src)) & 15) ? 0 : (r.n >> 2);
        for (int64_t i = (int64_t)blockIdx.x * 256 + threadIdx.x; i < n4; i += (int64_t)gridDim.x * 256) {
            float4 a = reinterpret_cast<float4*>(r.dst)[i];
            const float4 b = reinterpret_cast<const float4*>(r.src)[i];
            a.x += b.x; a.y += b.y; a.z += b.z; a.w += b.w;
            reinterpret_cast<float4*>(r.dst)[i] = a;
        }
        for (int64_t i = (n4 << 2) + (int64_t)blockIdx.x * 256 + threadIdx.x; i < r.n; i += (int64_t)gridDim.x * 256) r.dst[i] += r.src[i];
    }
}

struct BwdWs {
    size_t dxa, dxb, dB, dB1, dB2, dB3, dh, dhp, dy, dc3, dz, dG, dc2, dctx, wt, scr, total;
};

size_t max3(size_t a, size_t b, size_t c) { return a > b ? (a > c ? a : c) : (b > c ? b : c); }

BwdWs bwd_ws(int B, int T, int d, int d_ff, int ksz) {
    const size_t N = (size_t)B * T;
    BwdWs w;
    size_t o = 0;
    w.dxa = o;  o = up256(o + N * d * 4);
    w.dxb = o;  o = up256(o + N * d * 4);
    w.dB = o;   o = up256(o + N * d * 2);
    w.dB1 = o;  o = up256(o + N * d * 2);
    w.dB2 = o;  o = up256(o + N * d * 2);
    w.dB3 = o;  o = up256(o + N * d * 2);
    w.dh = o;   o = up256(o + N * d_ff * 2);
    w.dhp = o;  o = up256(o + N * d_ff * 2);
    w.dy = o;   o = up256(o + N * d * 2);
    w.dc3 = o;  o = up256(o + N * d * 2);
    w.dz = o;   o = up256(o + N * d * 4);
    w.dG = o;   o = up256(o + (size_t)5 * (size_t)ia_layernorm_bwd_scratch_elems((int)N, d) * 4);
    w.dc2 = o;  o = up256(o + N * 2 * d * 2);
    w.dctx = o; o = up256(o + N * d * 2);
    w.wt = o;   o = up256(o + ((size_t)4 * d_ff * d + (size_t)7 * d * d) * 2);
    size_t scr = (size_t)ia_layernorm_bwd_scratch_elems((int)N, d);
    const int shapes[5][2] = {{d, d_ff}, {d_ff, d}, {d, d}, {2 * d, d}, {3 * d, d}};
    for (int i = 0; i < 5; ++i) {
        const size_t e = (size_t)ia_gemm_tn_scratch_elems((int)N, shapes[i][0], shapes[i][1]);
        scr = e > scr ? e : scr;
    }
    scr = max3(scr, (size_t)ia_bn_silu_bwd_scratch_elems((int64_t)N, d), (size_t)ia_dwconv_scratch_elems(B, T, d, ksz));
    {
        const ia_tn_problem ga[5] = {{nullptr, nullptr, nullptr, nullptr, d, d_ff, (int)N, d, d_ff},
                                     {nullptr, nullptr, nullptr, nullptr, d_ff, d, (int)N, d_ff, d},
                                     {nullptr, nullptr, nullptr, nullptr, d, d, (int)N, d, d},
                                     {nullptr, nullptr, nullptr, nullptr, 2 * d, d, (int)N, 2 * d, d},
                                     {nullptr, nullptr, nullptr, nullptr, d, d, (int)N, d, d}};
        const ia_tn_problem gb[4] = {{nullptr, nullptr, nullptr, nullptr, 3 * d, d, (int)N, 3 * d, d},
                                     {nullptr, nullptr, nullptr, nullptr, d, d, (int)(N > (size_t)64 * 512 ? N : (size_t)64 * 512), d, d},
                                     {nullptr, nullptr, nullptr, nullptr, d, d_ff, (int)N, d, d_ff},
                                     {nullptr, nullptr, nullptr, nullptr, d_ff, d, (int)N, d_ff, d}};
        scr = max3(scr, (size_t)ia_gemm_tn_grouped_scratch_elems(ga, 5), (size_t)ia_gemm_tn_grouped_scratch_elems(gb, 4));
        scr = max3(scr, (size_t)ia_gemm_tn_grouped_scratch_elems(gb, 2), (size_t)ia_gemm_tn_grouped_scratch_elems(gb + 2, 2));
        ia_tn_problem gall[9];
        for (int i = 0; i < 5; ++i) gall[i] = ga[i];
        for (int i = 0; i < 4; ++i) gall[5 + i] = gb[i];
        scr = scr > (size_t)ia_gemm_tn_grouped_scratch_elems(gall, 9) ? scr : (size_t)ia_gemm_tn_grouped_scratch_elems(gall, 9);
    }
    w.scr = o;  o = up256(o + scr * 4);
    w.total = o;
    return w;
}

int linear_bwd(const void* dY, const void* X, const void* W, int M, int n, int k, void* dX, float* dW, float* db, void* wt,
               float* scr, ia_stream_t stream) {
    if (dX) {
        IA_TRY(transpose_bf16(W, n, k, wt, (hipStream_t)stream));
        IA_TRY(ia_gemm_bf16(dY, n, wt, n, M, k, n, nullptr, 0, 0.f, 0, 1.f, nullptr, 0, nullptr, 0, dX, k, stream));
    }
    return ia_gemm_tn_bf16(dY, n, X, k, M, n, k, dW, db, scr, stream);
}

bool tn_grouping_enabled() {
    static const bool on = [] { const char* e = getenv("IA_TN_GROUPED"); return !(e && e[0] == '0'); }();
    return on;
}
int flush_group(const ia_tn_problem* grp, int ngrp, float* scr, ia_stream_t stream) {
    if (tn_grouping_enabled()) return ia_gemm_tn_bf16_grouped(grp, ngrp, scr, stream);
    for (int i = 0; i < ngrp; ++i)
        IA_TRY(ia_gemm_tn_bf16(grp[i].dY, grp[i].ldy, grp[i].X, grp[i].ldx, grp[i].M, grp[i].n, grp[i].k, grp[i].dW, grp[i].db, scr, stream));
    return IA_OK;
}
int linear_bwd_deferred(const void* dY, const void* X, const void* W, int M, int n, int k, void* dX, float* dW, float* db, const void* wt,
                        ia_tn_problem* grp, int* ngrp, ia_stream_t stream) {
    (void)W;
    if (dX) IA_TRY(ia_gemm_bf16(dY, n, wt, n, M, k, n, nullptr, 0, 0.f, 0, 1.f, nullptr, 0, nullptr, 0, dX, k, stream));
    grp[*ngrp] = ia_tn_problem{dY, X, dW, db, n, k, M, n, k};
    ++*ngrp;
    return IA_OK;
}

struct SideCtx {
    hipStream_t s = nullptr;
    hipEvent_t ev[8] = {};
    bool ok = false, tried = false;
    bool a_pending = false;
};
SideCtx* side_ctx() {
    static SideCtx ctx[16];
    const char* e = getenv("IA_WGRAD_SIDE");
    if (!(e && e[0] == '1')) return nullptr;
    int dev = 0;
    if (hipGetDevice(&dev) != hipSuccess || dev < 0 || dev >= 16) return nullptr;
    SideCtx& c = ctx[dev];
    if (!c.tried) {
        c.tried = true;
        bool ok = hipStreamCreateWithFlags(&c.s, hipStreamNonBlocking) == hipSuccess;
        for (int i = 0; ok && i < 8; ++i) ok = hipEventCreateWithFlags(&c.ev[i], hipEventDisableTiming) == hipSuccess;
        c.ok = ok;
    }
    return c.ok ? &c : nullptr;
}
struct PendingGroup { ia_tn_problem grp[8]; int n = 0; const void* ws = nullptr; };
PendingGroup* pending_group() {
    static PendingGroup pg[16];
    int dev = 0;
    if (hipGetDevice(&dev) != hipSuccess || dev < 0 || dev >= 16) return nullptr;
    return &pg[dev];
}
bool merged_wgrads() {
    const char* e = getenv("IA_TN_MERGE");
    return !(e && e[0] == '0') && tn_grouping_enabled();
}

int stream_after(hipStream_t from, hipStream_t to, hipEvent_t ev) {
    if (hipEventRecord(ev, from) != hipSuccess || hipStreamWaitEvent(to, ev, 0) != hipSuccess) return IA_LAUNCH_FAILED;
    return IA_OK;
}

}

extern "C" size_t ia_conformer_block_bwd_ws_bytes(int B, int T, int d, int d_ff, int ksz) {
    if (B <= 0 || T <= 0 || d <= 0 || d_ff <= 0 || ksz <= 0) return 0;
    return bwd_ws(B, T, d, d_ff, ksz).total;
}

extern "C" int ia_conformer_block_supported(int d, int d_ff, int H, int ksz, int T) {
    if (d <= 0 || H <= 0 || d % H != 0) return 0;
    const int dk = d / H;
    return (d % 8 == 0 && d <= 1024 && d_ff % 8 == 0 && ksz <= 31 && (ksz & 1) == 1 && dk <= 64 && dk % 4 == 0 && T >= 1) ? 1 : 0;
}

extern "C" int ia_conformer_block_fwd(const ia_block_params* Lp, const float* x0, const void* pos_emb, int pos_rows,
                                      const int64_t* lens, int B, int T, unsigned seed, const ia_block_saved* Sp, float* out,
                                      float* dw_scratch, ia_stream_t stream) {
    return ia_conformer_block_fwd_phase(Lp, x0, pos_emb, pos_rows, lens, B, T, seed, Sp, out, dw_scratch, 0, stream);
}

extern "C" int ia_conformer_block_fwd_phase(const ia_block_params* Lp, const float* x0, const void* pos_emb, int pos_rows,
                                            const int64_t* lens, int B, int T, unsigned seed, const ia_block_saved* Sp,
                                            float* out, float* dw_scratch, int phase, ia_stream_t stream) {
    if (phase < 0 || phase > 2) return IA_INVALID_VALUE;
    if (!Lp || !x0 || !pos_emb || !lens || !Sp || !out || !dw_scratch || B <= 0 || T <= 0) return IA_INVALID_VALUE;
    const ia_block_params& L = *Lp;
    const ia_block_saved& S = *Sp;
    const int d = L.d, d_ff = L.d_ff, H = L.n_heads, dk = d / (H > 0 ? H : 1), ksz = L.ksz, N = B * T;
    if (!ia_conformer_block_supported(d, d_ff, H, ksz, T) || pos_rows < 2 * T - 1 || L.att_window != 0 || L.att_style != 0) return IA_UNSUPPORTED;
    const float p = L.p_drop, pff = L.p_ff, patt = L.p_att;
    if (phase != 2) {
    IA_TRY(ia_layernorm(x0, d, N, d, L.ln_ff1_g, L.ln_ff1_b, L.ln_eps, nullptr, 0, nullptr, nullptr, S.y1, d, stream));
    IA_TRY(ia_gemm_bf16_ex(S.y1, d, L.w_ff1a, d, N, d_ff, d, L.b_ff1a, 1, pff, seed + 1, 1.f, nullptr, 0, nullptr, 0, S.h1, d_ff,
                           S.h1p, d_ff, nullptr, 0, stream));
    IA_TRY(ia_gemm_bf16(S.h1, d_ff, L.w_ff1b, d_ff, N, d, d_ff, L.b_ff1b, 0, p, seed + 2, L.fc_factor, x0, d, S.x1, d, nullptr, 0, stream));
    IA_TRY(ia_layernorm(S.x1, d, N, d, L.ln_att_g, L.ln_att_b, L.ln_eps, nullptr, 0, nullptr, nullptr, S.y2, d, stream));
    IA_TRY(ia_gemm_bf16(S.y2, d, L.w_qkv, d, N, 3 * d, d, L.b_qkv, 0, 0.f, 0, 1.f, nullptr, 0, nullptr, 0, S.qkv, 3 * d, stream));
    IA_TRY(ia_gemm_bf16(pos_emb, d, L.w_pos, d, pos_rows, d, d, nullptr, 0, 0.f, 0, 1.f, nullptr, 0, nullptr, 0, S.pl, d, stream));
    IA_TRY(ia_relpos_attention_flash_lse(S.qkv, S.pl, L.pos_u, L.pos_v, lens, B, T, H, dk, patt, seed + 7, S.ctxv, S.lse, stream));
    IA_TRY(ia_gemm_bf16(S.ctxv, d, L.w_out, d, N, d, d, L.b_out, 0, p, seed + 3, 1.f, S.x1, d, S.x2, d, nullptr, 0, stream));
    IA_TRY(ia_layernorm(S.x2, d, N, d, L.ln_conv_g, L.ln_conv_b, L.ln_eps, nullptr, 0, nullptr, nullptr, S.y3, d, stream));
    IA_TRY(ia_gemm_bf16(S.y3, d, L.w_pw1, d, N, 2 * d, d, L.b_pw1, 0, 0.f, 0, 1.f, nullptr, 0, nullptr, 0, S.c2, 2 * d, stream));
    IA_TRY(ia_glu_dwconv(S.c2, lens, B, T, d, ksz, L.dw_w, L.dw_b, S.z, S.sums, S.sums + d, dw_scratch, stream));
    }
    if (phase == 1) return IA_OK;
    const bool synced = phase == 2;
    if (ia_gemm_bnsilu_supported(d)) {
        IA_TRY(ia_gemm_bnsilu_bf16_keep(S.z, d, N, S.sums, S.sums + d, L.bn_g, L.bn_b, synced ? nullptr : L.bn_rm,
                                        synced ? nullptr : L.bn_rv, synced ? nullptr : L.bn_nbt, L.bn_momentum, L.bn_eps, 1, L.w_pw2,
                                        d, N, d, d, L.b_pw2, p, seed + 4, 1.f, S.x2, d, S.x3, d, nullptr, 0, nullptr, S.c3, d, stream));
    } else {
        IA_TRY(ia_bn_silu(S.z, N, d, S.sums, S.sums + d, L.bn_g, L.bn_b, synced ? nullptr : L.bn_rm, synced ? nullptr : L.bn_rv,
                          synced ? nullptr : L.bn_nbt, L.bn_momentum, L.bn_eps, 1, S.c3, stream));
        IA_TRY(ia_gemm_bf16(S.c3, d, L.w_pw2, d, N, d, d, L.b_pw2, 0, p, seed + 4, 1.f, S.x2, d, S.x3, d, nullptr, 0, stream));
    }
    IA_TRY(ia_layernorm(S.x3, d, N, d, L.ln_ff2_g, L.ln_ff2_b, L.ln_eps, nullptr, 0, nullptr, nullptr, S.y4, d, stream));
    IA_TRY(ia_gemm_bf16_ex(S.y4, d, L.w_ff2a, d, N, d_ff, d, L.b_ff2a, 1, pff, seed + 5, 1.f, nullptr, 0, nullptr, 0, S.h4, d_ff,
                           S.h4p, d_ff, nullptr, 0, stream));
    IA_TRY(ia_gemm_bf16(S.h4, d_ff, L.w_ff2b, d_ff, N, d, d_ff, L.b_ff2b, 0, p, seed + 6, L.fc_factor, S.x3, d, S.x4, d, nullptr, 0, stream));
    return ia_layernorm(S.x4, d, N, d, L.ln_out_g, L.ln_out_b, L.ln_eps, out, d, nullptr, nullptr, nullptr, 0, stream);
}

extern "C" int ia_conformer_block_bwd_a(const ia_block_params* Lp, const ia_block_saved* Sp, const ia_block_grads* Gp,
                                        const float* dout, const int64_t* lens, int B, int T, unsigned seed, void* workspace,
                                        size_t workspace_bytes, float** dx2_out, void** dctx_out, ia_stream_t stream) {
    return ia_conformer_block_bwd_a_phase(Lp, Sp, Gp, dout, lens, B, T, seed, workspace, workspace_bytes, dx2_out, dctx_out, 0, nullptr,
                                          stream);
}

extern "C" int ia_conformer_block_bwd_a_phase(const ia_block_params* Lp, const ia_block_saved* Sp, const ia_block_grads* Gp,
                                              const float* dout, const int64_t* lens, int B, int T, unsigned seed,
                                              void* workspace, size_t workspace_bytes, float** dx2_out, void** dctx_out,
                                              int phase, const float* bn_S12, ia_stream_t stream) {
    if (phase < 0 || phase > 2 || (phase == 2 && !bn_S12)) return IA_INVALID_VALUE;
    if (!Lp || !Sp || !Gp || !dout || !lens || !workspace || !dx2_out || !dctx_out || B <= 0 || T <= 0) return IA_INVALID_VALUE;
    const ia_block_params& L = *Lp;
    const ia_block_saved& S = *Sp;
    const ia_block_grads& G = *Gp;
    const int d = L.d, d_ff = L.d_ff, ksz = L.ksz, N = B * T;
    const BwdWs w = bwd_ws(B, T, d, d_ff, ksz);
    if (workspace_bytes < w.total) return IA_WORKSPACE_TOO_SMALL;
    char* ws = (char*)workspace;
    float *dxa = (float*)(ws + w.dxa), *dxb = (float*)(ws + w.dxb), *dz = (float*)(ws + w.dz), *scr = (float*)(ws + w.scr);
    float* lnp = (float*)(ws + w.dG);
    const size_t lnp_set = (size_t)ia_layernorm_bwd_scratch_elems(N, d);
    void *dB = ws + w.dB, *dB1 = ws + w.dB1, *dB2 = ws + w.dB2, *dhp = ws + w.dhp, *dy = ws + w.dy, *dc3 = ws + w.dc3, *dc2 = ws + w.dc2,
         *dctx = ws + w.dctx, *wt = ws + w.wt;
    const float p = L.p_drop, pff = L.p_ff;
    ia_tn_problem grp[8];
    int ngrp = 0;
    char* wtb = (char*)wt;
    void *wt_ff2b = wtb, *wt_ff2a = wtb + (size_t)d * d_ff * 2, *wt_pw2 = wtb + (size_t)2 * d * d_ff * 2,
         *wt_pw1 = wtb + ((size_t)2 * d * d_ff + (size_t)d * d) * 2, *wt_out = wtb + ((size_t)2 * d * d_ff + (size_t)3 * d * d) * 2;
    if (phase != 2) {
        TrList tl{};
        tr_add(&tl, L.w_ff2b, d, d_ff, wt_ff2b); tr_add(&tl, L.w_ff2a, d_ff, d, wt_ff2a); tr_add(&tl, L.w_pw2, d, d, wt_pw2);
        tr_add(&tl, L.w_pw1, 2 * d, d, wt_pw1); tr_add(&tl, L.w_out, d, d, wt_out);
        IA_TRY(tr_launch(tl, (hipStream_t)stream));
    }
    if (phase != 2) {
    IA_TRY(ia_layernorm_bwd_drop(S.x4, d, dout, nullptr, d, N, d, L.ln_out_g, L.ln_eps, nullptr, dxa, d, nullptr, nullptr,
                                 L.fc_factor, p, seed + 6, dB, d, lnp + 0 * lnp_set, stream));
    IA_TRY(ia_gemm_bf16_ex(dB, d, wt_ff2b, d, N, d_ff, d, nullptr, 3, pff, seed + 5, 1.f, nullptr, 0, nullptr, 0, dhp, d_ff, nullptr, 0,
                           S.h4p, d_ff, stream));
    IA_TRY(linear_bwd_deferred(dB, S.h4, L.w_ff2b, N, d, d_ff, nullptr, G.w_ff2b, G.b_ff2b, wt_ff2b, grp, &ngrp, stream));
    IA_TRY(linear_bwd_deferred(dhp, S.y4, L.w_ff2a, N, d_ff, d, dy, G.w_ff2a, G.b_ff2a, wt_ff2a, grp, &ngrp, stream));
    IA_TRY(ia_layernorm_bwd_drop(S.x3, d, nullptr, dy, d, N, d, L.ln_ff2_g, L.ln_eps, dxa, dxb, d, nullptr, nullptr, 1.f, p,
                                 seed + 4, dB1, d, lnp + 1 * lnp_set, stream));
    IA_TRY(linear_bwd_deferred(dB1, S.c3, L.w_pw2, N, d, d, dc3, G.w_pw2, G.b_pw2, wt_pw2, grp, &ngrp, stream));
    if (phase == 0)
        IA_TRY(ia_bn_silu_bwd(S.z, dc3, N, d, S.sums, S.sums + d, L.bn_g, L.bn_b, L.bn_eps, G.bn_b, G.bn_g, dz, scr, stream));
    else
        IA_TRY(ia_bn_silu_bwd_reduce(S.z, dc3, N, d, S.sums, S.sums + d, L.bn_g, L.bn_b, L.bn_eps, G.bn_b, G.bn_g, scr, stream));
    }
    if (phase == 1) {
        IA_TRY(flush_group(grp, ngrp, scr, stream));
        return IA_OK;
    }
    if (phase == 2)
        IA_TRY(ia_bn_silu_bwd_apply(S.z, dc3, N, d, S.sums, S.sums + d, L.bn_g, L.bn_b, L.bn_eps, bn_S12, bn_S12 + d, dz, stream));
    IA_TRY(ia_dwconv_glu_bwd(dz, S.c2, lens, B, T, d, ksz, L.dw_w, dc2, stream));
    SideCtx* side = phase == 0 ? side_ctx() : nullptr;
    hipStream_t main = (hipStream_t)stream;
    if (side) {
        IA_TRY(stream_after(main, side->s, side->ev[0]));
        IA_TRY(ia_dwconv_glu_wgrad(S.c2, lens, dz, B, T, d, ksz, G.dw_w, G.dw_b, scr, (ia_stream_t)side->s));
    } else {
        IA_TRY(ia_dwconv_glu_wgrad(S.c2, lens, dz, B, T, d, ksz, G.dw_w, G.dw_b, scr, stream));
    }
    IA_TRY(linear_bwd_deferred(dc2, S.y3, L.w_pw1, N, 2 * d, d, dy, G.w_pw1, G.b_pw1, wt_pw1, grp, &ngrp, stream));
    IA_TRY(ia_layernorm_bwd_drop(S.x2, d, nullptr, dy, d, N, d, L.ln_conv_g, L.ln_eps, dxb, dxa, d, nullptr, nullptr, 1.f, p,
                                 seed + 3, dB2, d, lnp + 2 * lnp_set, stream));
    IA_TRY(linear_bwd_deferred(dB2, S.ctxv, L.w_out, N, d, d, dctx, G.w_out, G.b_out, wt_out, grp, &ngrp, stream));
    if (side) {
        IA_TRY(stream_after(main, side->s, side->ev[1]));
        IA_TRY(flush_group(grp, ngrp, scr, (ia_stream_t)side->s));
        if (hipEventRecord(side->ev[2], side->s) != hipSuccess) return IA_LAUNCH_FAILED;
        side->a_pending = true;
    } else if (phase == 0 && merged_wgrads() && pending_group()) {
        PendingGroup* pg = pending_group();
        for (int i = 0; i < ngrp; ++i) pg->grp[i] = grp[i];
        pg->n = ngrp; pg->ws = workspace;
    } else {
        IA_TRY(flush_group(grp, ngrp, scr, stream));
    }
    *dx2_out = dxa;
    *dctx_out = dctx;
    return IA_OK;
}

extern "C" int ia_conformer_block_bwd_b(const ia_block_params* Lp, const ia_block_saved* Sp, const ia_block_grads* Gp,
                                        const float* x0, const void* pos_emb, int pos_rows, const void* dqkv, const void* dpl,
                                        int B, int T, unsigned seed, void* workspace, size_t workspace_bytes, float* dx0,
                                        const void* add_table, int n_add, ia_stream_t stream) {
    if (!Lp || !Sp || !Gp || !x0 || !pos_emb || !dqkv || !dpl || !workspace || !dx0 || B <= 0 || T <= 0) return IA_INVALID_VALUE;
    const ia_block_params& L = *Lp;
    const ia_block_saved& S = *Sp;
    const ia_block_grads& G = *Gp;
    const int d = L.d, d_ff = L.d_ff, ksz = L.ksz, N = B * T;
    const BwdWs w = bwd_ws(B, T, d, d_ff, ksz);
    if (workspace_bytes < w.total) return IA_WORKSPACE_TOO_SMALL;
    char* ws = (char*)workspace;
    float *dxa = (float*)(ws + w.dxa), *dxb = (float*)(ws + w.dxb), *scr = (float*)(ws + w.scr);
    float* lnp = (float*)(ws + w.dG);
    const size_t lnp_set = (size_t)ia_layernorm_bwd_scratch_elems(N, d);
    PendingGroup* pg = pending_group();
    const bool carried = pg && pg->n > 0 && pg->ws == workspace;
    void *dB = ws + (carried ? w.dB3 : w.dB), *dhp = ws + (carried ? w.dh : w.dhp), *dy = ws + w.dy, *wt = ws + w.wt;
    const float p = L.p_drop, pff = L.p_ff;
    ia_tn_problem grp[12];
    int ngrp = 0;
    if (carried) {
        for (int i = 0; i < pg->n; ++i) grp[ngrp++] = pg->grp[i];
        pg->n = 0;
    }
    char* wtb = (char*)wt + ((size_t)2 * d * d_ff + (size_t)4 * d * d) * 2;
    void *wt_qkv = wtb, *wt_ff1b = wtb + (size_t)3 * d * d * 2, *wt_ff1a = wtb + ((size_t)3 * d * d + (size_t)d * d_ff) * 2;
    {
        TrList tl{};
        tr_add(&tl, L.w_qkv, 3 * d, d, wt_qkv); tr_add(&tl, L.w_ff1b, d, d_ff, wt_ff1b); tr_add(&tl, L.w_ff1a, d_ff, d, wt_ff1a);
        IA_TRY(tr_launch(tl, (hipStream_t)stream));
    }
    SideCtx* side = carried ? nullptr : side_ctx();
    hipStream_t main = (hipStream_t)stream;
    IA_TRY(linear_bwd_deferred(dqkv, S.y2, L.w_qkv, N, 3 * d, d, dy, G.w_qkv, G.b_qkv, wt_qkv, grp, &ngrp, stream));
    grp[ngrp++] = ia_tn_problem{dpl, pos_emb, G.w_pos, nullptr, d, d, pos_rows, d, d};
    if (side) {
        IA_TRY(stream_after(main, side->s, side->ev[3]));
        IA_TRY(flush_group(grp, ngrp, scr, (ia_stream_t)side->s));
        ngrp = 0;
        if (side->a_pending) {
            if (hipStreamWaitEvent(main, side->ev[2], 0) != hipSuccess) return IA_LAUNCH_FAILED;
            side->a_pending = false;
        }
    }
    IA_TRY(ia_layernorm_bwd_drop(S.x1, d, nullptr, dy, d, N, d, L.ln_att_g, L.ln_eps, dxa, dxb, d, nullptr, nullptr, L.fc_factor,
                                 p, seed + 2, dB, d, lnp + 3 * lnp_set, stream));
    IA_TRY(ia_gemm_bf16_ex(dB, d, wt_ff1b, d, N, d_ff, d, nullptr, 3, pff, seed + 1, 1.f, nullptr, 0, nullptr, 0, dhp, d_ff, nullptr, 0,
                           S.h1p, d_ff, stream));
    IA_TRY(linear_bwd_deferred(dB, S.h1, L.w_ff1b, N, d, d_ff, nullptr, G.w_ff1b, G.b_ff1b, wt_ff1b, grp, &ngrp, stream));
    if (side) {
        grp[ngrp++] = ia_tn_problem{dhp, S.y1, G.w_ff1a, G.b_ff1a, d_ff, d, N, d_ff, d};
        IA_TRY(stream_after(main, side->s, side->ev[4]));
        IA_TRY(flush_group(grp, ngrp, scr, (ia_stream_t)side->s));
        ngrp = 0;
        IA_TRY(ia_gemm_bf16(dhp, d_ff, wt_ff1a, d_ff, N, d, d_ff, nullptr, 0, 0.f, 0, 1.f, nullptr, 0, nullptr, 0, dy, d, stream));
    } else {
        IA_TRY(linear_bwd_deferred(dhp, S.y1, L.w_ff1a, N, d_ff, d, dy, G.w_ff1a, G.b_ff1a, wt_ff1a, grp, &ngrp, stream));
    }
    IA_TRY(ia_layernorm_bwd(x0, d, nullptr, dy, d, N, d, L.ln_ff1_g, L.ln_eps, dxb, dx0, d, nullptr, nullptr, lnp + 4 * lnp_set, stream));
    if (side) {
        IA_TRY(stream_after(main, side->s, side->ev[5]));
        stream = (ia_stream_t)side->s;
    } else {
        IA_TRY(flush_group(grp, ngrp, scr, stream));
    }
    {
        const int rows = ia_layernorm_bwd_partial_rows(N);
        const ia_finish_job jobs[5] = {{lnp + 0 * lnp_set, rows, 2 * d, d, G.ln_out_g, G.ln_out_b},
                                       {lnp + 1 * lnp_set, rows, 2 * d, d, G.ln_ff2_g, G.ln_ff2_b},
                                       {lnp + 2 * lnp_set, rows, 2 * d, d, G.ln_conv_g, G.ln_conv_b},
                                       {lnp + 3 * lnp_set, rows, 2 * d, d, G.ln_att_g, G.ln_att_b},
                                       {lnp + 4 * lnp_set, rows, 2 * d, d, G.ln_ff1_g, G.ln_ff1_b}};
        IA_TRY(ia_partials_finish_multi(jobs, 5, stream));
    }
    if (add_table && n_add > 0) {
        hipLaunchKernelGGL(multi_add_kernel, dim3(64, n_add < 64 ? n_add : 64), dim3(256), 0, (hipStream_t)stream,
                           (const AddRow*)add_table, n_add);
        IA_RETURN_IF_LAUNCH_FAILED();
    }
    if (side) IA_TRY(stream_after(side->s, main, side->ev[6]));
    return IA_OK;
}
```

### indic_cl_asr_amd/csrc/ffn_fused.hip

```cpp
#include <type_traits>
#include <hip/hip_bf16.h>

#include <stdlib.h>

#include "ia_common.h"
#include "dropout_mask.h"

namespace {

typedef __bf16 bf8 __attribute__((ext_vector_type(8)));
typedef float f16v __attribute__((ext_vector_type(16)));

constexpr int FF_M = 64;
constexpr int FF_THREADS = 512;
constexpr int FF_JC = 128;

struct FfnArgs {
    float* x; int N;
    const float* ln_g; const float* ln_b; float eps;
    const __bf16* W1; const float* b1;
    const __bf16* W2; const float* b2;
    int dff;
    float alpha;
    unsigned thr_ff, seed_ff; float ks_ff;
    unsigned thr_res, seed_res; float ks_res;
    const float* ln2_g; const float* ln2_b;
    __bf16* y_out;
    int ln2_y_only;
    int mode;
    const __bf16* Wt; const float* bt; __bf16* t_out; int nt;
};

__device__ __forceinline__ float half_wave_sum(float v) {
    v += IA_DPP_F(0.f, v, 0xB1, 0xF);
    v += IA_DPP_F(0.f, v, 0x4E, 0xF);
    v += IA_DPP_F(0.f, v, 0x141, 0xF);
    v += IA_DPP_F(0.f, v, 0x140, 0xF);
    v += __shfl_xor(v, 16, 64);
    return v;
}

template <int D, bool DROP_FF, bool DIAG, bool TAIL = false>
__global__ __launch_bounds__(FF_THREADS, 2) void ffn_fused_kernel(FfnArgs a) {
    const int mode = DIAG ? a.mode : 0;
    static_assert(D == 256, "wave decomposition below is written for d_model = 256");
    constexpr int SLOT = 32768;
    constexpr int YROW = D * 2;
    constexpr int XROW = FF_JC * 2;
    constexpr int EROW = D * 4 + 16;
    extern __shared__ __attribute__((aligned(16))) unsigned char smem[];
    unsigned char* sRing = smem;
    unsigned char* sX = smem + 4 * SLOT;
    float* sB1 = reinterpret_cast<float*>(smem + 4 * SLOT + FF_M * XROW);
    unsigned char* sY = smem + 3 * SLOT;
    unsigned char* sE = smem;

    const int tid = threadIdx.x, lane = tid & 63, wave = tid >> 6;
    const int l31 = lane & 31, hh = lane >> 5, sw = l31 & 15;
    const int mi = wave & 1, q = wave >> 1;
    const int m0 = blockIdx.x * FF_M;
    const int nchunks = a.dff / FF_JC;
    const int total = nchunks * 4;
    if ((mode & 4) && (blockIdx.x & 1)) return;

    const int wv = __builtin_amdgcn_readfirstlane(wave);
    const unsigned off1 = (unsigned)((16 * wv + (lane >> 4)) * (D * 2) + (((lane & 15) ^ (lane >> 4)) * 16));
    const unsigned off2 = (unsigned)((32 * wv + (lane >> 3)) * (a.dff * 2) + (((lane & 7) ^ (lane >> 4)) * 16));
    auto issue_slot = [&](int sq) {
        int kindB, c, h;
        if (sq < 4) { kindB = 0; c = sq >> 1; h = sq & 1; }
        else if (sq < total - 4) { const int r = sq - 4, j = 2 + (r >> 2), k = r & 3; kindB = k >> 1; c = kindB ? j - 2 : j; h = k & 1; }
        else { const int r = sq - (total - 4); kindB = 1; c = nchunks - 2 + (r >> 1); h = r & 1; }
        unsigned char* dst = sRing + (sq & 3) * SLOT + wv * 4096;
        const unsigned char* base;
        unsigned off, stride, xm1;
        if (DIAG && (mode & 8)) {
            base = reinterpret_cast<const unsigned char*>(kindB ? a.W2 : a.W1) + (size_t)(c * 2 + h) * SLOT;
            off = (unsigned)(wv * 4096 + lane * 16); stride = 1024; xm1 = 0;
        } else {
            base = kindB ? reinterpret_cast<const unsigned char*>(a.W2) + (size_t)(c * FF_JC + h * 64) * 2
                         : reinterpret_cast<const unsigned char*>(a.W1) + ((size_t)c * FF_JC * D + h * 128) * 2;
            off = kindB ? off2 : off1;
            stride = kindB ? (unsigned)(16 * a.dff) : (unsigned)(4 * D * 2);
            xm1 = kindB ? 0u : 64u;
        }
#pragma unroll
        for (int i = 0; i < 4; ++i) {
            const unsigned xm = (unsigned)(i & 1) * 64u + (unsigned)(i >> 1) * 2u * xm1;
            const unsigned vo = (off ^ xm) + (unsigned)i * stride;
            ia_lds_dma16(base + vo, dst + i * 1024);
        }
    };
    int sq = 0;
    auto step_sync = [&](int vm) {
        if (vm == 8) asm volatile("s_waitcnt vmcnt(8)" ::: "memory");
        else if (vm == 4) asm volatile("s_waitcnt vmcnt(4)" ::: "memory");
        else asm volatile("s_waitcnt vmcnt(0)" ::: "memory");
        asm volatile("s_waitcnt lgkmcnt(0)" ::: "memory");
        __builtin_amdgcn_s_barrier();
    };
    auto issue_next = [&](bool issue) {
        if (issue && !(mode & 1)) issue_slot(sq + 3);
        ++sq;
    };

    issue_slot(0); issue_slot(1); issue_slot(2);
    for (int i = tid; i < a.dff; i += FF_THREADS) sB1[i] = a.b1[i];

#pragma unroll
    for (int pass = 0; pass < FF_M / 16; ++pass) {
        const int r = pass * 16 + (tid >> 5), vec = tid & 31;
        const int gm = (m0 + r < a.N) ? (m0 + r) : (a.N - 1);
        const float4 x0 = *reinterpret_cast<const float4*>(a.x + (size_t)gm * D + vec * 8);
        const float4 x1 = *reinterpret_cast<const float4*>(a.x + (size_t)gm * D + vec * 8 + 4);
        float v[8] = {x0.x, x0.y, x0.z, x0.w, x1.x, x1.y, x1.z, x1.w};
        float s = 0.f;
#pragma unroll
        for (int j = 0; j < 8; ++j) s += v[j];
        const float mean = half_wave_sum(s) * (1.f / D);
        float qq = 0.f;
#pragma unroll
        for (int j = 0; j < 8; ++j) { v[j] -= mean; qq += v[j] * v[j]; }
        const float rstd = rsqrtf(half_wave_sum(qq) * (1.f / D) + a.eps);
        const float4 g0 = *reinterpret_cast<const float4*>(a.ln_g + vec * 8), g1 = *reinterpret_cast<const float4*>(a.ln_g + vec * 8 + 4);
        const float4 c0 = *reinterpret_cast<const float4*>(a.ln_b + vec * 8), c1 = *reinterpret_cast<const float4*>(a.ln_b + vec * 8 + 4);
        const float gg[8] = {g0.x, g0.y, g0.z, g0.w, g1.x, g1.y, g1.z, g1.w};
        const float bb[8] = {c0.x, c0.y, c0.z, c0.w, c1.x, c1.y, c1.z, c1.w};
        union { uint4 u; __bf16 h[8]; } o;
#pragma unroll
        for (int j = 0; j < 8; ++j) o.h[j] = (__bf16)(v[j] * rstd * gg[j] + bb[j]);
        const int phys = (vec & 16) | ((vec & 15) ^ (r & 15));
        *reinterpret_cast<uint4*>(sY + r * YROW + phys * 16) = o.u;
    }
    __syncthreads();
    constexpr int KS = D / 16;
    bf8 yf[KS];
    const int t16 = (hh ^ sw) * 16;
    {
        const unsigned char* yrow = sY + (mi * 32 + l31) * YROW;
#pragma unroll
        for (int s = 0; s < KS; ++s) yf[s] = *reinterpret_cast<const bf8*>(yrow + ((s & 8) * 32) + (((s & 7) * 32) ^ t16));
    }

    f16v o[2];
#pragma unroll
    for (int nt = 0; nt < 2; ++nt)
#pragma unroll
        for (int r = 0; r < 16; ++r) o[nt][r] = 0.f;

    const unsigned char* w1row = sRing + (q * 32 + l31) * 256;
    const int w2sw = (((q * 64 + l31) >> 1) & 7);
    const unsigned char* w2row = sRing + (q * 64 + l31) * 128;
    const unsigned char* xrow = sX + (mi * 32 + l31) * XROW;
    const unsigned gm_drop = (unsigned)(m0 + mi * 32 + l31);
    const bool do_mfma = !(mode & 2);
    const unsigned sm_ff = ia_dm_hash32(a.seed_ff);

    struct Act { float v[4]; unsigned w; };
    auto act_begin = [&](int c, int g, Act& st) {
        if (DROP_FF) st.w = ia_dm_word24(sm_ff, gm_drop * (unsigned)(a.dff >> 2) + (unsigned)((c * FF_JC + q * 32 + g * 8 + hh * 4) >> 2));
    };
    auto bias_init = [&](int c, f16v& acc) {
        float4 b0, b1v, b2v, b3;
        const unsigned baddr = (unsigned)(4 * SLOT + FF_M * XROW) + (unsigned)((c * FF_JC + q * 32 + hh * 4) * 4);
        asm volatile("ds_read_b128 %0, %4\n\tds_read_b128 %1, %4 offset:32\n\tds_read_b128 %2, %4 offset:64\n\t"
                     "ds_read_b128 %3, %4 offset:96\n\ts_waitcnt lgkmcnt(0)"
                     : "=&v"(b0), "=&v"(b1v), "=&v"(b2v), "=&v"(b3) : "v"(baddr) : "memory");
        acc[0] = b0.x; acc[1] = b0.y; acc[2] = b0.z; acc[3] = b0.w; acc[4] = b1v.x; acc[5] = b1v.y; acc[6] = b1v.z; acc[7] = b1v.w;
        acc[8] = b2v.x; acc[9] = b2v.y; acc[10] = b2v.z; acc[11] = b2v.w; acc[12] = b3.x; acc[13] = b3.y; acc[14] = b3.z; acc[15] = b3.w;
    };
    typedef float f2v __attribute__((ext_vector_type(2)));
    auto act_stage = [&](int g, const f16v& acc, Act& st, int k) {
        if (k < 4) {
            const int pr = k >> 1;
            if (!(k & 1)) {
                f2v t = {acc[4 * g + 2 * pr], acc[4 * g + 2 * pr + 1]};
                asm volatile("" : "+v"(t));
                const f2v m = t * (f2v){-1.44269504088896341f, -1.44269504088896341f};
                f2v e = {__builtin_amdgcn_exp2f(m.x), __builtin_amdgcn_exp2f(m.y)};
                asm volatile("" : "+v"(e));
                st.v[2 * pr] = e.x; st.v[2 * pr + 1] = e.y;
            } else {
                f2v e = {st.v[2 * pr], st.v[2 * pr + 1]};
                asm volatile("" : "+v"(e));
                const f2v d = e + (f2v){1.f, 1.f};
                const f2v r = {__builtin_amdgcn_rcpf(d.x), __builtin_amdgcn_rcpf(d.y)};
                f2v o2 = (f2v){acc[4 * g + 2 * pr], acc[4 * g + 2 * pr + 1]} * r;
                asm volatile("" : "+v"(o2));
                st.v[2 * pr] = o2.x; st.v[2 * pr + 1] = o2.y;
            }
        } else if (DROP_FF) {
            const int i = k - 4;
            float t = st.v[i];
            asm volatile("" : "+v"(t));
            t = (((st.w >> (8 * i)) & 0xFFu) >= a.thr_ff) ? t : 0.f;
            asm volatile("" : "+v"(t));
            st.v[i] = t;
        }
    };
    auto act_end = [&](const Act& st) -> uint2 {
        typedef __bf16 bf2v __attribute__((ext_vector_type(2)));
        union { uint2 u; bf2v h[2]; } pk;
        pk.h[0] = __builtin_convertvector((f2v){st.v[0], st.v[1]}, bf2v);
        pk.h[1] = __builtin_convertvector((f2v){st.v[2], st.v[3]}, bf2v);
        return pk.u;
    };
    auto interval = [&](auto isB, auto ngc, int pos, int p, f16v& accT, int c, int g0, const f16v& accS, uint2* out, bool issue = true, int cinit = -1) {
        constexpr bool IS_B = decltype(isB)::value;
        constexpr int NG = decltype(ngc)::value;
        bf8 fa[4][2], fb[4];
        auto load_batch = [&](int b) {
            if (!do_mfma) return;
            if (!IS_B) {
                fa[b][0] = *reinterpret_cast<const bf8*>(w1row + pos * SLOT + (((2 * b) * 32) ^ t16));
                fa[b][1] = *reinterpret_cast<const bf8*>(w1row + pos * SLOT + (((2 * b + 1) * 32) ^ t16));
            } else {
                const int woff = pos * SLOT + (((b * 2 + hh) ^ w2sw) * 16);
                fb[b] = *reinterpret_cast<const bf8*>(xrow + (((p * 8 + b * 2 + hh) ^ sw) * 16));
                fa[b][0] = *reinterpret_cast<const bf8*>(w2row + woff);
                fa[b][1] = *reinterpret_cast<const bf8*>(w2row + 32 * 128 + woff);
            }
        };
        load_batch(0); load_batch(1);
        issue_next(issue);
        if (cinit >= 0) bias_init(cinit, accT);
        Act st[NG > 0 ? NG : 1];
#pragma unroll
        for (int i = 0; i < NG; ++i) act_begin(c, g0 + i, st[i]);
#pragma unroll
        for (int s = 0; s < 8; ++s) {
            if (do_mfma) {
                if (!IS_B) { accT = __builtin_amdgcn_mfma_f32_32x32x16_bf16(fa[s >> 1][s & 1], yf[p * 8 + s], accT, 0, 0, 0); asm volatile("" : "+v"(accT)); }
                else { o[s & 1] = __builtin_amdgcn_mfma_f32_32x32x16_bf16(fa[s >> 1][s & 1], fb[s >> 1], o[s & 1], 0, 0, 0); asm volatile("" : "+v"(o[s & 1])); }
            }
            if (NG == 1) act_stage(g0, accS, st[0], s);
            if (NG == 2) { act_stage(g0 + (s >> 2), accS, st[NG > 1 ? (s >> 2) : 0], 2 * (s & 3)); act_stage(g0 + (s >> 2), accS, st[NG > 1 ? (s >> 2) : 0], 2 * (s & 3) + 1); }
            if ((s & 1) && (s >> 1) + 2 < 4) load_batch((s >> 1) + 2);
        }
#pragma unroll
        for (int i = 0; i < NG; ++i) {
            out[i] = act_end(st[i]);
            asm volatile("" :: "v"(out[i].x), "v"(out[i].y));
        }
    };
    const std::integral_constant<bool, false> PA{};
    const std::integral_constant<bool, true> PB{};
    const std::integral_constant<int, 0> G0{};
    const std::integral_constant<int, 1> G1{};
    const std::integral_constant<int, 2> G2{};
    auto store_x = [&](const uint2 (&xp)[4]) {
#pragma unroll
        for (int g = 0; g < 4; ++g) {
            const unsigned xaddr = (unsigned)(4 * SLOT) + (unsigned)((mi * 32 + l31) * XROW + (((q * 4 + g) ^ sw) * 16) + hh * 8);
            asm volatile("ds_write_b64 %0, %1" :: "v"(xaddr), "v"(xp[g]) : "memory");
        }
    };

    f16v acc, accn;
    uint2 xp[4];
    step_sync(8); interval(PA, G0, 0, 0, acc, 0, 0, acc, nullptr, true, 0);
    step_sync(8); interval(PA, G0, 1, 1, acc, 0, 0, acc, nullptr);
    step_sync(8); interval(PA, G2, 2, 0, accn, 0, 0, acc, xp, true, 1);
    step_sync(8); interval(PA, G2, 3, 1, accn, 0, 2, acc, xp + 2);
    acc = accn;
    for (int j = 2; j < nchunks; ++j) {
        step_sync(8); store_x(xp); interval(PA, G1, 0, 0, accn, j - 1, 0, acc, xp, true, j);
        step_sync(8); interval(PA, G1, 1, 1, accn, j - 1, 1, acc, xp + 1);
        step_sync(8); interval(PB, G1, 2, 0, accn, j - 1, 2, acc, xp + 2);
        step_sync(8); interval(PB, G1, 3, 1, accn, j - 1, 3, acc, xp + 3);
        acc = accn;
    }
    {
        uint2 xl[4];
        step_sync(8); store_x(xp);
        asm volatile("s_waitcnt lgkmcnt(0)" ::: "memory");
        __builtin_amdgcn_s_barrier();
        interval(PB, G2, 0, 0, accn, nchunks - 1, 0, acc, xl, true);
        step_sync(8); interval(PB, G2, 1, 1, accn, nchunks - 1, 2, acc, xl + 2, false);
        step_sync(4); store_x(xl);
        asm volatile("s_waitcnt lgkmcnt(0)" ::: "memory");
        __builtin_amdgcn_s_barrier();
        interval(PB, G0, 2, 0, accn, 0, 0, acc, nullptr, false);
        step_sync(0); interval(PB, G0, 3, 1, accn, 0, 0, acc, nullptr, false);
    }
    __syncthreads();
    int tide = tid;
    asm volatile("" : "+v"(tide));

#pragma unroll
    for (int nt = 0; nt < 2; ++nt)
#pragma unroll
        for (int g = 0; g < 4; ++g) {
            const int n0 = q * 64 + nt * 32 + g * 8 + hh * 4;
            *reinterpret_cast<float4*>(sE + (mi * 32 + l31) * EROW + n0 * 4) =
                make_float4(o[nt][4 * g], o[nt][4 * g + 1], o[nt][4 * g + 2], o[nt][4 * g + 3]);
        }
    __syncthreads();
#pragma unroll
    for (int pass = 0; pass < FF_M / 16; ++pass) {
        const int r = pass * 16 + (tide >> 5), vec = tide & 31;
        const int gm = m0 + r;
        const bool live = gm < a.N;
        const int gmc = live ? gm : (a.N - 1);
        const float4 e0 = *reinterpret_cast<const float4*>(sE + r * EROW + vec * 32);
        const float4 e1 = *reinterpret_cast<const float4*>(sE + r * EROW + vec * 32 + 16);
        float v[8] = {e0.x, e0.y, e0.z, e0.w, e1.x, e1.y, e1.z, e1.w};
        const float4 b0 = *reinterpret_cast<const float4*>(a.b2 + vec * 8), b1 = *reinterpret_cast<const float4*>(a.b2 + vec * 8 + 4);
        if (DROP_FF) {
#pragma unroll
            for (int j = 0; j < 8; ++j) v[j] *= a.ks_ff;
        }
        v[0] += b0.x; v[1] += b0.y; v[2] += b0.z; v[3] += b0.w; v[4] += b1.x; v[5] += b1.y; v[6] += b1.z; v[7] += b1.w;
        float sc = a.alpha;
        if (a.thr_res > 0) {
            const unsigned mk = ia_keep8(a.seed_res, (unsigned)gmc, (unsigned)D, (unsigned)(vec * 8), a.thr_res);
#pragma unroll
            for (int j = 0; j < 8; ++j)
                if (!((mk >> j) & 1u)) v[j] = 0.f;
            sc *= a.ks_res;
        }
        const float4 r0 = *reinterpret_cast<const float4*>(a.x + (size_t)gmc * D + vec * 8);
        const float4 r1 = *reinterpret_cast<const float4*>(a.x + (size_t)gmc * D + vec * 8 + 4);
        const float rr[8] = {r0.x, r0.y, r0.z, r0.w, r1.x, r1.y, r1.z, r1.w};
#pragma unroll
        for (int j = 0; j < 8; ++j) v[j] = v[j] * sc + rr[j];
        if (a.ln2_y_only && live) {
            *reinterpret_cast<float4*>(a.x + (size_t)gm * D + vec * 8) = make_float4(v[0], v[1], v[2], v[3]);
            *reinterpret_cast<float4*>(a.x + (size_t)gm * D + vec * 8 + 4) = make_float4(v[4], v[5], v[6], v[7]);
        }
        if (a.ln2_g) {
            float s = 0.f;
#pragma unroll
            for (int j = 0; j < 8; ++j) s += v[j];
            const float mean = half_wave_sum(s) * (1.f / D);
            float qq = 0.f;
#pragma unroll
            for (int j = 0; j < 8; ++j) { v[j] -= mean; qq += v[j] * v[j]; }
            const float rstd = rsqrtf(half_wave_sum(qq) * (1.f / D) + a.eps);
            const float4 g0 = *reinterpret_cast<const float4*>(a.ln2_g + vec * 8), g1 = *reinterpret_cast<const float4*>(a.ln2_g + vec * 8 + 4);
            const float4 c0 = *reinterpret_cast<const float4*>(a.ln2_b + vec * 8), c1 = *reinterpret_cast<const float4*>(a.ln2_b + vec * 8 + 4);
            const float gg[8] = {g0.x, g0.y, g0.z, g0.w, g1.x, g1.y, g1.z, g1.w};
            const float bb[8] = {c0.x, c0.y, c0.z, c0.w, c1.x, c1.y, c1.z, c1.w};
#pragma unroll
            for (int j = 0; j < 8; ++j) v[j] = v[j] * rstd * gg[j] + bb[j];
        }
        union { uint4 u; __bf16 h[8]; } ob;
        if (TAIL || a.y_out) {
#pragma unroll
            for (int j = 0; j < 8; ++j) ob.h[j] = (__bf16)v[j];
        }
        if (TAIL)
            *reinterpret_cast<uint4*>(sY + r * YROW + ((vec & 16) | ((vec & 15) ^ (r & 15))) * 16) = ob.u;
        if (live) {
            if (!a.ln2_y_only) {
                *reinterpret_cast<float4*>(a.x + (size_t)gm * D + vec * 8) = make_float4(v[0], v[1], v[2], v[3]);
                *reinterpret_cast<float4*>(a.x + (size_t)gm * D + vec * 8 + 4) = make_float4(v[4], v[5], v[6], v[7]);
            }
            if (a.y_out) *reinterpret_cast<uint4*>(a.y_out + (size_t)gm * D + vec * 8) = ob.u;
        }
    }
    if constexpr (TAIL) {
        __syncthreads();
        const unsigned char* Wt = reinterpret_cast<const unsigned char*>(a.Wt);
        const int nslots = a.nt / 64;
        const int c16 = lane & 15, q4 = lane >> 4, cg = wave & 3, fh = wave >> 2;
        unsigned toff[4];
#pragma unroll
        for (int i = 0; i < 4; ++i) {
            const int row = 2 * (4 * wv + i) + (lane >> 5);
            const int pc = lane & 31;
            toff[i] = (unsigned)((row * D + ((pc & 16) | ((pc & 15) ^ (row & 15))) * 8) * 2);
        }
        auto issue_t = [&](int sl) {
            unsigned char* dst = sRing + (sl & 3) * SLOT + wv * 4096;
            const unsigned char* base = Wt + (size_t)sl * (64 * D * 2);
#pragma unroll
            for (int i = 0; i < 4; ++i) ia_lds_dma16(base + toff[i], dst + i * 1024);
        };
        for (int i = tid; i < a.nt; i += FF_THREADS) sB1[i] = a.bt ? a.bt[i] : 0.f;
        issue_t(0);
        if (nslots > 1) issue_t(1);
        if (nslots > 2) issue_t(2);
        bf8 yt[2][8];
        {
            const unsigned ybase = (unsigned)(3 * SLOT) + (unsigned)((fh * 32 + c16) * YROW);
#pragma unroll
            for (int tl = 0; tl < 2; ++tl)
#pragma unroll
                for (int ks = 0; ks < 8; ++ks) {
                    const unsigned ad = ybase + (unsigned)(tl * 16 * YROW) + (unsigned)((((4 * ks + q4) & 16) | (((4 * ks + q4) & 15) ^ c16)) * 16);
                    asm volatile("ds_read_b128 %0, %1" : "=&v"(yt[tl][ks]) : "v"(ad));
                }
            asm volatile("s_waitcnt lgkmcnt(0)" : "+v"(yt[0][0]), "+v"(yt[0][1]), "+v"(yt[0][2]), "+v"(yt[0][3]), "+v"(yt[0][4]), "+v"(yt[0][5]),
                         "+v"(yt[0][6]), "+v"(yt[0][7]), "+v"(yt[1][0]), "+v"(yt[1][1]), "+v"(yt[1][2]), "+v"(yt[1][3]), "+v"(yt[1][4]),
                         "+v"(yt[1][5]), "+v"(yt[1][6]), "+v"(yt[1][7]));
        }
        typedef float f4v __attribute__((ext_vector_type(4)));
        unsigned ooff[2];
        bool olive[2];
#pragma unroll
        for (int tl = 0; tl < 2; ++tl) {
            const int gm = m0 + fh * 32 + tl * 16 + c16;
            olive[tl] = gm < a.N;
            ooff[tl] = (unsigned)((olive[tl] ? gm : 0) * a.nt + cg * 16 + 4 * q4);
        }
        for (int sl = 0; sl < nslots; ++sl) {
            const int later = nslots - 1 - sl;
            if (later >= 2) asm volatile("s_waitcnt vmcnt(8)" ::: "memory");
            else if (later == 1) asm volatile("s_waitcnt vmcnt(4)" ::: "memory");
            else asm volatile("s_waitcnt vmcnt(0)" ::: "memory");
            __builtin_amdgcn_s_barrier();
            if (sl + 3 < nslots) issue_t(sl + 3);
            const unsigned wbase = (unsigned)((sl & 3) * SLOT) + (unsigned)((cg * 16 + c16) * YROW);
            bf8 wf[8];
#pragma unroll
            for (int ks = 0; ks < 8; ++ks) {
                const unsigned ad = wbase + (unsigned)((((4 * ks + q4) & 16) | (((4 * ks + q4) & 15) ^ c16)) * 16);
                asm volatile("ds_read_b128 %0, %1" : "=&v"(wf[ks]) : "v"(ad));
            }
            asm volatile("s_waitcnt lgkmcnt(0)" : "+v"(wf[0]), "+v"(wf[1]), "+v"(wf[2]), "+v"(wf[3]), "+v"(wf[4]), "+v"(wf[5]), "+v"(wf[6]), "+v"(wf[7]));
            f4v t0 = {0.f, 0.f, 0.f, 0.f}, t1 = {0.f, 0.f, 0.f, 0.f};
#pragma unroll
            for (int ks = 0; ks < 8; ++ks) {
                t0 = __builtin_amdgcn_mfma_f32_16x16x32_bf16(wf[ks], yt[0][ks], t0, 0, 0, 0);
                t1 = __builtin_amdgcn_mfma_f32_16x16x32_bf16(wf[ks], yt[1][ks], t1, 0, 0, 0);
            }
            float4 bv;
            {
                const unsigned baddr = (unsigned)(4 * SLOT + FF_M * XROW) + (unsigned)((sl * 64 + cg * 16 + 4 * q4) * 4);
                asm volatile("ds_read_b128 %0, %1\n\ts_waitcnt lgkmcnt(0)" : "=&v"(bv) : "v"(baddr) : "memory");
            }
            __bf16* orow = a.t_out + (size_t)sl * 64;
#pragma unroll
            for (int tl = 0; tl < 2; ++tl) {
                const f4v t = tl ? t1 : t0;
                union { uint2 u; __bf16 h[4]; } pk;
                pk.h[0] = (__bf16)(t[0] + bv.x); pk.h[1] = (__bf16)(t[1] + bv.y); pk.h[2] = (__bf16)(t[2] + bv.z); pk.h[3] = (__bf16)(t[3] + bv.w);
                if (olive[tl]) *reinterpret_cast<uint2*>(orow + ooff[tl]) = pk.u;
            }
        }
    }
}

}

extern "C" int ia_ffn_fused_supported(int d, int d_ff) { return (d == 256 && d_ff >= 2 * FF_JC && d_ff % FF_JC == 0 && d_ff <= 2048) ? 1 : 0; }

namespace {
int ffn_launch(float* x, int N, int d, int d_ff, const float* ln_g, const float* ln_b, float eps, const void* W1,
               const float* b1, const void* W2, const float* b2, float alpha, float p_ff, unsigned seed_ff,
               float p_res, unsigned seed_res, const float* ln2_g, const float* ln2_b, void* y_out,
               int ln2_to_y_only, const void* Wt, const float* bt, void* t_out, int nt, ia_stream_t stream);
}

extern "C" int ia_ffn_fused(float* x, int N, int d, int d_ff, const float* ln_g, const float* ln_b, float eps, const void* W1,
                            const float* b1, const void* W2, const float* b2, float alpha, float p_ff, unsigned seed_ff,
                            float p_res, unsigned seed_res, const float* ln2_g, const float* ln2_b, void* y_out,
                            int ln2_to_y_only, ia_stream_t stream) {
    return ffn_launch(x, N, d, d_ff, ln_g, ln_b, eps, W1, b1, W2, b2, alpha, p_ff, seed_ff, p_res, seed_res, ln2_g, ln2_b, y_out,
                      ln2_to_y_only, nullptr, nullptr, nullptr, 0, stream);
}

extern "C" int ia_ffn_fused_tail_supported(int d, int d_ff, int nt) { return (ia_ffn_fused_supported(d, d_ff) && nt > 0 && nt % 64 == 0) ? 1 : 0; }

extern "C" int ia_ffn_fused_tail(float* x, int N, int d, int d_ff, const float* ln_g, const float* ln_b, float eps, const void* W1,
                                 const float* b1, const void* W2, const float* b2, float alpha, float p_ff, unsigned seed_ff,
                                 float p_res, unsigned seed_res, const float* ln2_g, const float* ln2_b, void* y_out,
                                 int ln2_to_y_only, const void* Wt, const float* bt, void* t_out, int nt, ia_stream_t stream) {
    if (!Wt || !t_out || !ln2_g || !ln2_b) return IA_INVALID_VALUE;
    if (!ia_ffn_fused_tail_supported(d, d_ff, nt)) return IA_UNSUPPORTED;
    if (!ia_is_aligned(Wt, 16) || !ia_is_aligned(t_out, 16) || (bt && !ia_is_aligned(bt, 16))) return IA_INVALID_VALUE;
    if ((long long)N * nt >= (1ll << 31) || nt > d_ff) return IA_UNSUPPORTED;
    return ffn_launch(x, N, d, d_ff, ln_g, ln_b, eps, W1, b1, W2, b2, alpha, p_ff, seed_ff, p_res, seed_res, ln2_g, ln2_b, y_out,
                      ln2_to_y_only, Wt, bt, t_out, nt, stream);
}

namespace {
int ffn_launch(float* x, int N, int d, int d_ff, const float* ln_g, const float* ln_b, float eps, const void* W1,
               const float* b1, const void* W2, const float* b2, float alpha, float p_ff, unsigned seed_ff,
               float p_res, unsigned seed_res, const float* ln2_g, const float* ln2_b, void* y_out,
               int ln2_to_y_only, const void* Wt, const float* bt, void* t_out, int nt, ia_stream_t stream) {
    if (!x || !ln_g || !ln_b || !W1 || !b1 || !W2 || !b2 || N <= 0 || (ln2_g && !ln2_b)) return IA_INVALID_VALUE;
    if (!ia_ffn_fused_supported(d, d_ff)) return IA_UNSUPPORTED;
    if (p_ff < 0.f || p_ff >= 1.f || p_res < 0.f || p_res >= 1.f) return IA_INVALID_VALUE;
    if (!ia_is_aligned(x, 16) || !ia_is_aligned(W1, 16) || !ia_is_aligned(W2, 16) || !ia_is_aligned(b1, 16) ||
        !ia_is_aligned(b2, 16) || !ia_is_aligned(ln_g, 16) || !ia_is_aligned(ln_b, 16) || (ln2_g && !ia_is_aligned(ln2_g, 16)) ||
        (ln2_b && !ia_is_aligned(ln2_b, 16)) || (y_out && !ia_is_aligned(y_out, 16)))
        return IA_INVALID_VALUE;
    FfnArgs a;
    a.x = x; a.N = N; a.ln_g = ln_g; a.ln_b = ln_b; a.eps = eps;
    a.W1 = (const __bf16*)W1; a.b1 = b1; a.W2 = (const __bf16*)W2; a.b2 = b2; a.dff = d_ff; a.alpha = alpha;
    const ia_dropout_t drop_ff = ia_dropout_rule(p_ff), drop_res = ia_dropout_rule(p_res);
    a.thr_ff = drop_ff.thr; a.ks_ff = drop_ff.keep_scale; a.seed_ff = seed_ff;
    a.thr_res = drop_res.thr; a.ks_res = drop_res.keep_scale; a.seed_res = seed_res;
    if (ln2_to_y_only && (!ln2_g || (!y_out && !Wt))) return IA_INVALID_VALUE;
    a.ln2_g = ln2_g; a.ln2_b = ln2_b; a.y_out = (__bf16*)y_out; a.ln2_y_only = ln2_to_y_only ? 1 : 0;
    a.Wt = (const __bf16*)Wt; a.bt = bt; a.t_out = (__bf16*)t_out; a.nt = nt;
    if (d_ff > 2048) return IA_UNSUPPORTED;
    const int LDS = 4 * 32768 + FF_M * FF_JC * 2 + d_ff * 4;
    static_assert(FF_M * (256 * 4 + 16) <= 4 * 32768, "epilogue tile aliases the ring");
    { const char* e = getenv("IA_FFN_MODE"); a.mode = (e && *e) ? atoi(e) : 0; }
    const dim3 grid((N + FF_M - 1) / FF_M), blk(FF_THREADS);
    if (Wt) {
        if (a.thr_ff > 0) {
            IA_SET_MAX_LDS_ONCE((ffn_fused_kernel<256, true, false, true>), LDS);
            hipLaunchKernelGGL((ffn_fused_kernel<256, true, false, true>), grid, blk, LDS, (hipStream_t)stream, a);
        } else {
            IA_SET_MAX_LDS_ONCE((ffn_fused_kernel<256, false, false, true>), LDS);
            hipLaunchKernelGGL((ffn_fused_kernel<256, false, false, true>), grid, blk, LDS, (hipStream_t)stream, a);
        }
    } else if (a.mode) {
        IA_SET_MAX_LDS_ONCE((ffn_fused_kernel<256, true, true>), LDS);
        hipLaunchKernelGGL((ffn_fused_kernel<256, true, true>), grid, blk, LDS, (hipStream_t)stream, a);
    } else if (a.thr_ff > 0) {
        IA_SET_MAX_LDS_ONCE((ffn_fused_kernel<256, true, false>), LDS);
        hipLaunchKernelGGL((ffn_fused_kernel<256, true, false>), grid, blk, LDS, (hipStream_t)stream, a);
    } else {
        IA_SET_MAX_LDS_ONCE((ffn_fused_kernel<256, false, false>), LDS);
        hipLaunchKernelGGL((ffn_fused_kernel<256, false, false>), grid, blk, LDS, (hipStream_t)stream, a);
    }
    IA_RETURN_IF_LAUNCH_FAILED();
    return IA_OK;
}
}
```

### indic_cl_asr_amd/ops/block.py

```python
import torch

from .. import _lib
from . import fast


def _ptr(t):
    return _lib.ptr(t)


def _ln_bwd(x, ln, dy_f32=None, dy_bf16=None, dx_in=None):
    N, d = x.shape
    dev = x.device
    dx = torch.empty(N, d, dtype=torch.float32, device=dev)
    dgb = torch.empty(2, d, dtype=torch.float32, device=dev)
    dy = dy_f32 if dy_f32 is not None else dy_bf16
    L = _lib.lib()
    st = L.ia_layernorm_bwd(_ptr(x), x.stride(0), _ptr(dy_f32), _ptr(dy_bf16), dy.stride(0), N, d, _ptr(ln.weight),
                            float(ln.eps), _ptr(dx_in), _ptr(dx), d, _ptr(dgb[0]), _ptr(dgb[1]),
                            _ptr(fast.scratch(dev, L.ia_layernorm_bwd_scratch_elems(N, d))), _lib.stream_ptr())
    _lib.check(st, "ia_layernorm_bwd")
    return dx, dgb[0], dgb[1]


def _branch_grad(dxr, alpha, p, seed):
    N, d = dxr.shape
    out = torch.empty(N, d, dtype=torch.bfloat16, device=dxr.device)
    st = _lib.lib().ia_scale_dropout_bf16(_ptr(dxr), N, d, float(alpha), float(p), int(seed) & 0xFFFFFFFF, _ptr(out),
                                          _lib.stream_ptr())
    _lib.check(st, "ia_scale_dropout_bf16")
    return out


def _lin_bwd(dyb, xb, wb, need_dx=True):
    M, n = dyb.shape
    k = xb.shape[1]
    dx = torch.mm(dyb, wb) if need_dx else None
    L = _lib.lib()
    buf = torch.empty(n * k + n, dtype=torch.float32, device=dyb.device)
    dW, db = buf[:n * k].view(n, k), buf[n * k:]
    st = L.ia_gemm_tn_bf16(_ptr(dyb), dyb.stride(0), _ptr(xb), xb.stride(0), M, n, k, _ptr(dW), _ptr(db),
                           _ptr(fast.scratch(dyb.device, L.ia_gemm_tn_scratch_elems(M, n, k))), _lib.stream_ptr())
    _lib.check(st, "ia_gemm_tn_bf16")
    return dx, dW, db


def _silu_dropout(h_pre, p, seed):
    M, N = h_pre.shape
    out = torch.empty_like(h_pre)
    _lib.check(_lib.lib().ia_silu_dropout(_ptr(h_pre), M, N, float(p), int(seed) & 0xFFFFFFFF, _ptr(out), _lib.stream_ptr()),
               "ia_silu_dropout")
    return out


def _silu_dropout_bwd(h_pre, dh, p, seed):
    M, N = h_pre.shape
    out = torch.empty_like(h_pre)
    _lib.check(_lib.lib().ia_silu_dropout_bwd(_ptr(h_pre), _ptr(dh), M, N, float(p), int(seed) & 0xFFFFFFFF, _ptr(out),
                                              _lib.stream_ptr()), "ia_silu_dropout_bwd")
    return out


DIRECT_ACCUMULATE = True


def block_supported(layer, x2d, T):
    d = x2d.shape[-1]
    bn = layer.conv.batch_norm
    w = getattr(layer.self_attn, "att_window", None)
    c = getattr(layer.self_attn, "att_context", None)
    if c is not None:
        att_ok = w is None and fast.attention_context_supported(T, layer.self_attn.d_k, c)
    else:
        att_ok = (fast.attention_flash_supported(T, layer.self_attn.d_k) if w is None
                  else fast.attention_local_supported(T, layer.self_attn.d_k, w))
    return (x2d.is_cuda and d % 8 == 0 and d <= 1024 and fast.bn_module_ok(bn)
            and layer.conv.depthwise_conv.weight.shape[-1] <= 31 and att_ok)


class _ConformerBlockFn(torch.autograd.Function):
    @staticmethod
    def forward(ctx, x, layer, lens, pe, B, T, seed, *params):
        L = _lib.lib()
        N, d = x.shape
        dev = x.device
        tr = layer.training
        p = float(layer.dropout.p) if tr else 0.0
        ff1, ff2, att, cv = layer.feed_forward1, layer.feed_forward2, layer.self_attn, layer.conv
        pff1 = float(ff1.dropout.p) if tr else 0.0
        pff2 = float(ff2.dropout.p) if tr else 0.0
        patt = float(att.dropout_rate) if tr else 0.0
        window = getattr(att, "att_window", None)
        context = getattr(att, "att_context", None)
        W = dict(w1=fast.bf16_shadow(ff1.linear1.weight), w2=fast.bf16_shadow(ff1.linear2.weight),
                 wqkv=fast.bf16_shadow(att.linear_q.weight, att.linear_k.weight, att.linear_v.weight),
                 wpos=fast.bf16_shadow(att.linear_pos.weight), wo=fast.bf16_shadow(att.linear_out.weight),
                 wp1=fast.bf16_shadow(cv.pointwise_conv1.weight), wp2=fast.bf16_shadow(cv.pointwise_conv2.weight),
                 w1b=fast.bf16_shadow(ff2.linear1.weight), w2b=fast.bf16_shadow(ff2.linear2.weight))
        new = lambda: torch.empty(N, d, dtype=torch.float32, device=dev)
        x0 = x.contiguous()
        y1 = fast.layernorm(x0, layer.norm_feed_forward1.weight, layer.norm_feed_forward1.bias, layer.norm_feed_forward1.eps)
        _, h1p = fast.gemm(y1, W["w1"], ff1.linear1.bias)
        h1 = _silu_dropout(h1p, pff1, seed + 1)
        x1, _ = fast.gemm(h1, W["w2"], ff1.linear2.bias, dropout_p=p, seed=seed + 2, alpha=layer.fc_factor, residual=x0,
                          out_f32=new(), want_bf16=False)
        y2 = fast.layernorm(x1, layer.norm_self_att.weight, layer.norm_self_att.bias, layer.norm_self_att.eps)
        _, qkv = fast.gemm(y2, W["wqkv"], fast.f32_cat(att.linear_q.bias, att.linear_k.bias, att.linear_v.bias))
        _, pl = fast.gemm(pe, W["wpos"])
        if context is not None:
            ctxv, lse = fast.relpos_attention_context(qkv, pl, att.pos_bias_u, att.pos_bias_v, lens, B, T, att.h, att.d_k, context, patt,
                                                      seed + 7, want_lse=True)
        elif window is None:
            ctxv, lse = fast.relpos_attention_flash(qkv, pl, att.pos_bias_u, att.pos_bias_v, lens, B, T, att.h, att.d_k, patt, seed + 7,
                                                    want_lse=True)
        else:
            ctxv, lse = fast.relpos_attention_local(qkv, pl, att.pos_bias_u, att.pos_bias_v, lens, B, T, att.h, att.d_k, window, patt,
                                                    seed + 7, want_lse=True)
        x2, _ = fast.gemm(ctxv, W["wo"], att.linear_out.bias, dropout_p=p, seed=seed + 3, residual=x1, out_f32=new(),
                          want_bf16=False)
        y3 = fast.layernorm(x2, layer.norm_conv.weight, layer.norm_conv.bias, layer.norm_conv.eps)
        _, c2 = fast.gemm(y3, W["wp1"], cv.pointwise_conv1.bias)
        bn = cv.batch_norm
        use_batch = bool(tr or not bn.track_running_stats)
        c3, z, sums = fast.glu_dwconv_bn_silu_fast(c2, lens, B, T, d, cv.depthwise_conv.weight, cv.depthwise_conv.bias, bn, tr,
                                                   keep=True)
        x3, _ = fast.gemm(c3, W["wp2"], cv.pointwise_conv2.bias, dropout_p=p, seed=seed + 4, residual=x2, out_f32=new(),
                          want_bf16=False)
        y4 = fast.layernorm(x3, layer.norm_feed_forward2.weight, layer.norm_feed_forward2.bias, layer.norm_feed_forward2.eps)
        _, h4p = fast.gemm(y4, W["w1b"], ff2.linear1.bias)
        h4 = _silu_dropout(h4p, pff2, seed + 5)
        x4, _ = fast.gemm(h4, W["w2b"], ff2.linear2.bias, dropout_p=p, seed=seed + 6, alpha=layer.fc_factor, residual=x3,
                          out_f32=new(), want_bf16=False)
        out = new()
        fast.layernorm(x4, layer.norm_out.weight, layer.norm_out.bias, layer.norm_out.eps, out_f32=out, want_bf16=False)
        if not use_batch:
            raise RuntimeError("trainable fused block expects train-mode BatchNorm (batch statistics)")
        ctx.S = dict(x0=x0, y1=y1, h1p=h1p, h1=h1, x1=x1, y2=y2, qkv=qkv, pl=pl, ctxv=ctxv, lse=lse, x2=x2, y3=y3, c2=c2, z=z, sums=sums,
                     c3=c3, x3=x3, y4=y4, h4p=h4p, h4=h4, x4=x4, W=W, pe=pe, lens=lens)
        ctx.meta = (layer, B, T, seed, p, pff1, pff2, patt, (window, context), [n for n, _ in layer.named_parameters()],
                    [q.requires_grad for q in params], params)
        return out

    @staticmethod
    def backward(ctx, dout):
        L = _lib.lib()
        S = ctx.S
        ctx.S = None
        layer, B, T, seed, p, pff1, pff2, patt, (window, context), names, req, params = ctx.meta
        W = S["W"]
        ff1, ff2, att, cv = layer.feed_forward1, layer.feed_forward2, layer.self_attn, layer.conv
        d = S["x0"].shape[1]
        N = B * T
        dev = dout.device
        G = {}
        dout = dout.float().contiguous()
        dx4, G["norm_out.weight"], G["norm_out.bias"] = _ln_bwd(S["x4"], layer.norm_out, dy_f32=dout)
        dB = _branch_grad(dx4, layer.fc_factor, p, seed + 6)
        dh, G["feed_forward2.linear2.weight"], G["feed_forward2.linear2.bias"] = _lin_bwd(dB, S["h4"], W["w2b"])
        dhp = _silu_dropout_bwd(S["h4p"], dh, pff2, seed + 5)
        dy, G["feed_forward2.linear1.weight"], G["feed_forward2.linear1.bias"] = _lin_bwd(dhp, S["y4"], W["w1b"])
        dx3, G["norm_feed_forward2.weight"], G["norm_feed_forward2.bias"] = _ln_bwd(S["x3"], layer.norm_feed_forward2,
                                                                                  dy_bf16=dy, dx_in=dx4)
        del dx4, dh, dhp
        dB = _branch_grad(dx3, 1.0, p, seed + 4)
        dc3, dWp2, G["conv.pointwise_conv2.bias"] = _lin_bwd(dB, S["c3"], W["wp2"])
        G["conv.pointwise_conv2.weight"] = dWp2.unsqueeze(-1)
        bn = cv.batch_norm
        S12 = torch.empty(2, d, dtype=torch.float32, device=dev)
        dz = torch.empty(N, d, dtype=torch.float32, device=dev)
        sums = S["sums"]
        group = fast.bn_sync_group(bn)
        bn_scr = _ptr(fast.scratch(dev, L.ia_bn_silu_bwd_scratch_elems(N, d)))
        if group is None:
            _lib.check(L.ia_bn_silu_bwd(_ptr(S["z"]), _ptr(dc3), N, d, _ptr(sums[:d]), _ptr(sums[d:2 * d]), _ptr(bn.weight),
                                        _ptr(bn.bias), float(bn.eps), _ptr(S12[0]), _ptr(S12[1]), _ptr(dz), bn_scr,
                                        _lib.stream_ptr()), "ia_bn_silu_bwd")
        else:
            import torch.distributed as dist
            _lib.check(L.ia_bn_silu_bwd_reduce(_ptr(S["z"]), _ptr(dc3), N, d, _ptr(sums[:d]), _ptr(sums[d:2 * d]), _ptr(bn.weight),
                                               _ptr(bn.bias), float(bn.eps), _ptr(S12[0]), _ptr(S12[1]), bn_scr,
                                               _lib.stream_ptr()), "ia_bn_silu_bwd_reduce")
            Sg = torch.cat([S12.reshape(-1), torch.full((1,), float(N), dtype=torch.float32, device=dev)])
            dist.all_reduce(Sg, group=group)
            Sg = Sg[:2 * d] * (float(N) / Sg[2 * d])
            _lib.check(L.ia_bn_silu_bwd_apply(_ptr(S["z"]), _ptr(dc3), N, d, _ptr(sums[:d]), _ptr(sums[d:2 * d]), _ptr(bn.weight),
                                              _ptr(bn.bias), float(bn.eps), _ptr(Sg[:d]), _ptr(Sg[d:]), _ptr(dz),
                                              _lib.stream_ptr()), "ia_bn_silu_bwd_apply")
        G["conv.batch_norm.bias"], G["conv.batch_norm.weight"] = S12[0], S12[1]
        ksz = cv.depthwise_conv.weight.shape[-1]
        w2 = cv.depthwise_conv.weight.detach().float().reshape(d, ksz).contiguous()
        dG = torch.empty(N, d, dtype=torch.float32, device=dev)
        _lib.check(L.ia_dwconv_time(_ptr(dz), B, T, d, ksz, _ptr(w2), None, 1, _ptr(dG), _lib.stream_ptr()), "ia_dwconv_time")
        Gm = torch.empty(N, d, dtype=torch.float32, device=dev)
        _lib.check(L.ia_glu_mask(_ptr(S["c2"]), _ptr(S["lens"]), B, T, d, _ptr(Gm), _lib.stream_ptr()), "ia_glu_mask")
        dwd = torch.empty(d, ksz, dtype=torch.float32, device=dev)
        dbd = torch.empty(d, dtype=torch.float32, device=dev)
        _lib.check(L.ia_dwconv_time_wgrad(_ptr(Gm), _ptr(dz), B, T, d, ksz, _ptr(dwd), _ptr(dbd),
                                          _ptr(fast.scratch(dev, L.ia_dwconv_scratch_elems(B, T, d, ksz))), _lib.stream_ptr()),
                   "ia_dwconv_time_wgrad")
        G["conv.depthwise_conv.weight"], G["conv.depthwise_conv.bias"] = dwd.view(d, 1, ksz), dbd
        dc2 = torch.empty(N, 2 * d, dtype=torch.bfloat16, device=dev)
        _lib.check(L.ia_glu_bwd(_ptr(S["c2"]), _ptr(dG), _ptr(S["lens"]), B, T, d, _ptr(dc2), _lib.stream_ptr()), "ia_glu_bwd")
        dy, dWp1, G["conv.pointwise_conv1.bias"] = _lin_bwd(dc2, S["y3"], W["wp1"])
        G["conv.pointwise_conv1.weight"] = dWp1.unsqueeze(-1)
        dx2, G["norm_conv.weight"], G["norm_conv.bias"] = _ln_bwd(S["x2"], layer.norm_conv, dy_bf16=dy, dx_in=dx3)
        del dx3, dz, dG, Gm, dc2, dc3
        dB = _branch_grad(dx2, 1.0, p, seed + 3)
        dctx, G["self_attn.linear_out.weight"], G["self_attn.linear_out.bias"] = _lin_bwd(dB, S["ctxv"], W["wo"])
        if context is not None:
            dqkv, dpl, du, dv = fast.relpos_attention_context_bwd(S["qkv"], S["pl"], att.pos_bias_u, att.pos_bias_v, S["lens"], S["ctxv"],
                                                                  dctx, S["lse"], B, T, att.h, att.d_k, context, patt, seed + 7)
        elif window is None:
            dqkv, dpl, du, dv = fast.relpos_attention_flash_bwd(S["qkv"], S["pl"], att.pos_bias_u, att.pos_bias_v, S["lens"], S["ctxv"],
                                                                dctx, S["lse"], B, T, att.h, att.d_k, patt, seed + 7)
        else:
            dqkv, dpl, du, dv = fast.relpos_attention_local_bwd(S["qkv"], S["pl"], att.pos_bias_u, att.pos_bias_v, S["lens"], S["ctxv"],
                                                                dctx, S["lse"], B, T, att.h, att.d_k, window, patt, seed + 7)
        G["self_attn.pos_bias_u"], G["self_attn.pos_bias_v"] = du, dv
        dy, dWqkv, dbqkv = _lin_bwd(dqkv, S["y2"], W["wqkv"])
        for i, nm in enumerate(("q", "k", "v")):
            G[f"self_attn.linear_{nm}.weight"] = dWqkv[i * d:(i + 1) * d]
            G[f"self_attn.linear_{nm}.bias"] = dbqkv[i * d:(i + 1) * d]
        G["self_attn.linear_pos.weight"] = _lin_bwd(dpl, S["pe"], None, need_dx=False)[1]
        dx1, G["norm_self_att.weight"], G["norm_self_att.bias"] = _ln_bwd(S["x1"], layer.norm_self_att, dy_bf16=dy, dx_in=dx2)
        del dx2, dqkv, dctx
        dB = _branch_grad(dx1, layer.fc_factor, p, seed + 2)
        dh, G["feed_forward1.linear2.weight"], G["feed_forward1.linear2.bias"] = _lin_bwd(dB, S["h1"], W["w2"])
        dhp = _silu_dropout_bwd(S["h1p"], dh, pff1, seed + 1)
        dy, G["feed_forward1.linear1.weight"], G["feed_forward1.linear1.bias"] = _lin_bwd(dhp, S["y1"], W["w1"])
        dx0, G["norm_feed_forward1.weight"], G["norm_feed_forward1.bias"] = _ln_bwd(S["x0"], layer.norm_feed_forward1,
                                                                                  dy_bf16=dy, dx_in=dx1)
        outs, dst, src = [], [], []
        for n, r, q in zip(names, req, params):
            if not r:
                outs.append(None)
            elif DIRECT_ACCUMULATE and q.grad is not None and q.grad.dtype == torch.float32:
                dst.append(q.grad); src.append(G[n].reshape(q.grad.shape)); outs.append(None)
            else:
                outs.append(G[n].reshape(q.shape))
        if dst:
            torch._foreach_add_(dst, src)
        return (dx0, None, None, None, None, None, None) + tuple(outs)


def pad_pos_emb(pos_emb, d):
    pe = pos_emb.detach().reshape(-1, d)
    rows = (pe.shape[0] + 7) // 8 * 8
    out = torch.zeros(rows, d, dtype=torch.bfloat16, device=pe.device)
    out[:pe.shape[0]] = pe
    return out


def conformer_block(x2d, layer, lens, pe_bf16, B, T, seed):
    if (USE_NATIVE_BLOCKS and layer.training and getattr(layer.self_attn, "att_window", None) is None
            and getattr(layer.self_attn, "att_context", None) is None):
        att = layer.self_attn
        if _lib.lib().ia_conformer_block_supported(x2d.shape[-1], layer.feed_forward1.linear1.weight.shape[0], att.h,
                                                   layer.conv.depthwise_conv.weight.shape[-1], T):
            return conformer_block_native(x2d, layer, lens, pe_bf16, B, T, seed)
    return _ConformerBlockFn.apply(x2d, layer, lens, pe_bf16, B, T, seed, *list(layer.parameters()))


USE_NATIVE_BLOCKS = True

_SAVED_FIELDS = ("y1", "h1p", "h1", "x1", "y2", "qkv", "pl", "ctxv", "x2", "y3", "c2", "z", "sums", "c3", "x3", "y4", "h4p", "h4", "x4", "lse")


def _saved_layout(N, d, dff, pos_rows, H):
    sizes = dict(y1=N * d * 2, h1p=N * dff * 2, h1=N * dff * 2, x1=N * d * 4, y2=N * d * 2, qkv=N * 3 * d * 2, pl=pos_rows * d * 2,
                 ctxv=N * d * 2, x2=N * d * 4, y3=N * d * 2, c2=N * 2 * d * 2, z=N * d * 4, sums=(2 * d + 64) * 4, c3=N * d * 2,
                 x3=N * d * 4, y4=N * d * 2, h4p=N * dff * 2, h4=N * dff * 2, x4=N * d * 4, lse=N * H * 4)
    lay, o = {}, 0
    for f in _SAVED_FIELDS:
        lay[f] = (o, sizes[f])
        o = (o + sizes[f] + 255) // 256 * 256
    return lay, o


class _BlockRuntime:

    def __init__(self, layer, dev):
        import ctypes
        d = layer.norm_out.weight.shape[0]
        dff = layer.feed_forward1.linear1.weight.shape[0]
        ksz = layer.conv.depthwise_conv.weight.shape[-1]
        self.d, self.dff, self.ksz = d, dff, ksz
        blocks = [("w_ff1a", dff * d), ("b_ff1a", dff), ("w_ff1b", d * dff), ("b_ff1b", d), ("w_qkv", 3 * d * d), ("b_qkv", 3 * d),
                  ("w_pos", d * d), ("w_out", d * d), ("b_out", d), ("w_pw1", 2 * d * d), ("b_pw1", 2 * d), ("w_pw2", d * d), ("b_pw2", d),
                  ("w_ff2a", dff * d), ("b_ff2a", dff), ("w_ff2b", d * dff), ("b_ff2b", d)]
        for nm in ("ln_ff1", "ln_att", "ln_conv", "ln_ff2", "ln_out"):
            blocks += [(nm + "_g", d), (nm + "_b", d)]
        blocks += [("dw_w", d * ksz), ("dw_b", d), ("bn_g", d), ("bn_b", d), ("pos_u", d), ("pos_v", d)]
        off, o = {}, 0
        for nm, n in blocks:
            off[nm] = (o, n)
            o += (n + 3) // 4 * 4
        self.arena = torch.zeros(o, dtype=torch.float32, device=dev)
        self.off = off
        base = self.arena.data_ptr()
        self.grads = _lib.BlockGrads()
        for nm, _ in _lib.BlockGrads._fields_:
            setattr(self.grads, nm, base + 4 * off[nm][0])
        self.pos_u = self.arena[off["pos_u"][0]:off["pos_u"][0] + d]
        self.pos_v = self.arena[off["pos_v"][0]:off["pos_v"][0] + d]
        att, cv, ff1, ff2 = layer.self_attn, layer.conv, layer.feed_forward1, layer.feed_forward2
        self.param_src = [
            (ff1.linear1.weight, "w_ff1a", 0), (ff1.linear1.bias, "b_ff1a", 0), (ff1.linear2.weight, "w_ff1b", 0), (ff1.linear2.bias, "b_ff1b", 0),
            (att.linear_q.weight, "w_qkv", 0), (att.linear_k.weight, "w_qkv", d * d), (att.linear_v.weight, "w_qkv", 2 * d * d),
            (att.linear_q.bias, "b_qkv", 0), (att.linear_k.bias, "b_qkv", d), (att.linear_v.bias, "b_qkv", 2 * d),
            (att.linear_pos.weight, "w_pos", 0), (att.linear_out.weight, "w_out", 0), (att.linear_out.bias, "b_out", 0),
            (att.pos_bias_u, "pos_u", 0), (att.pos_bias_v, "pos_v", 0),
            (cv.pointwise_conv1.weight, "w_pw1", 0), (cv.pointwise_conv1.bias, "b_pw1", 0), (cv.pointwise_conv2.weight, "w_pw2", 0),
            (cv.pointwise_conv2.bias, "b_pw2", 0), (cv.depthwise_conv.weight, "dw_w", 0), (cv.depthwise_conv.bias, "dw_b", 0),
            (cv.batch_norm.weight, "bn_g", 0), (cv.batch_norm.bias, "bn_b", 0),
            (ff2.linear1.weight, "w_ff2a", 0), (ff2.linear1.bias, "b_ff2a", 0), (ff2.linear2.weight, "w_ff2b", 0), (ff2.linear2.bias, "b_ff2b", 0),
            (layer.norm_feed_forward1.weight, "ln_ff1_g", 0), (layer.norm_feed_forward1.bias, "ln_ff1_b", 0),
            (layer.norm_self_att.weight, "ln_att_g", 0), (layer.norm_self_att.bias, "ln_att_b", 0),
            (layer.norm_conv.weight, "ln_conv_g", 0), (layer.norm_conv.bias, "ln_conv_b", 0),
            (layer.norm_feed_forward2.weight, "ln_ff2_g", 0), (layer.norm_feed_forward2.bias, "ln_ff2_b", 0),
            (layer.norm_out.weight, "ln_out_g", 0), (layer.norm_out.bias, "ln_out_b", 0)]
        self._table_key, self._table = None, None

    def add_table(self):
        key = tuple((q.grad.data_ptr() if (q.requires_grad and q.grad is not None) else 0) for q, _, _ in self.param_src)
        if key != self._table_key:
            rows = []
            base = self.arena.data_ptr()
            for (q, blk, sub), gp in zip(self.param_src, key):
                if gp:
                    rows.append((gp, base + 4 * (self.off[blk][0] + sub), q.numel()))
            self._table = torch.tensor(rows, dtype=torch.int64).to(self.arena.device) if rows else None
            self._table_key = key
            self._n_rows = len(rows)
        return self._table, (self._n_rows if self._table is not None else 0)


_RUNTIMES = {}
_BWD_WS = {}


def _runtime(layer, dev):
    rt = _RUNTIMES.get(id(layer))
    if rt is None or rt.arena.device != dev:
        import weakref
        rt = _RUNTIMES[id(layer)] = _BlockRuntime(layer, dev)
        weakref.finalize(layer, _RUNTIMES.pop, id(layer), None)
    return rt


class _ConformerBlockNativeFn(torch.autograd.Function):
    @staticmethod
    def forward(ctx, x, layer, lens, pe, B, T, seed, *params):
        import ctypes
        L = _lib.lib()
        N, d = x.shape
        dev = x.device
        rt = _runtime(layer, dev)
        tr = layer.training
        if not tr:
            raise RuntimeError("trainable fused block expects train-mode BatchNorm (batch statistics)")
        bp = fast._block_params(layer)
        x0 = x.contiguous()
        lay, nbytes = _saved_layout(N, d, rt.dff, pe.shape[0], layer.self_attn.h)
        arena = torch.empty(nbytes, dtype=torch.uint8, device=dev)
        saved = _lib.BlockSaved()
        base = arena.data_ptr()
        for f in _SAVED_FIELDS:
            setattr(saved, f, base + lay[f][0])
        out = torch.empty(N, d, dtype=torch.float32, device=dev)
        dw_scr = fast.scratch(dev, L.ia_dwconv_scratch_elems(B, T, d, rt.ksz))
        bn = layer.conv.batch_norm
        group = fast.bn_sync_group(bn)
        fwd_args = (ctypes.addressof(bp), _ptr(x0), _ptr(pe), pe.shape[0], _ptr(lens), B, T, int(seed) & 0xFFFFFFFF,
                    ctypes.addressof(saved), _ptr(out), _ptr(dw_scr))
        if group is None:
            _lib.check(L.ia_conformer_block_fwd(*fwd_args, _lib.stream_ptr()), "ia_conformer_block_fwd")
        else:
            _lib.check(L.ia_conformer_block_fwd_phase(*fwd_args, 1, _lib.stream_ptr()), "ia_conformer_block_fwd_phase")
            o = lay["sums"][0]
            fast.bn_sync_sums(arena[o:o + (2 * d + 1) * 4].view(torch.float32), N, d, bn, group)
            _lib.check(L.ia_conformer_block_fwd_phase(*fwd_args, 2, _lib.stream_ptr()), "ia_conformer_block_fwd_phase")
        ctx.group = group
        ctx.keep = (x0, arena, saved, lay, pe, lens, bp)
        ctx.meta = (layer, B, T, seed, [q.requires_grad for q in params], params)
        return out

    @staticmethod
    def backward(ctx, dout):
        import ctypes
        if ctx.keep is None:
            raise RuntimeError("fused Conformer block: trying to backward through the graph a second time (its saved "
                               "activations were released by the first backward)")
        L = _lib.lib()
        x0, arena, saved, lay, pe, lens, bp = ctx.keep
        ctx.keep = None
        layer, B, T, seed, req, params = ctx.meta
        N, d = x0.shape
        dev = x0.device
        rt = _runtime(layer, dev)
        att = layer.self_attn
        n_ws = L.ia_conformer_block_bwd_ws_bytes(B, T, d, rt.dff, rt.ksz)
        key = (dev.index, torch.cuda.current_stream(dev).cuda_stream)
        ws = _BWD_WS.get(key)
        if ws is None or ws.numel() < n_ws:
            ws = _BWD_WS[key] = torch.empty(n_ws, dtype=torch.uint8, device=dev)
        dout = dout.float().contiguous()
        dx2_p, dctx_p = ctypes.c_void_p(), ctypes.c_void_p()
        sp = _lib.stream_ptr()
        a_args = (ctypes.addressof(bp), ctypes.addressof(saved), ctypes.addressof(rt.grads), _ptr(dout), _ptr(lens), B, T,
                  int(seed) & 0xFFFFFFFF, _ptr(ws), n_ws, ctypes.addressof(dx2_p), ctypes.addressof(dctx_p))
        if ctx.group is None:
            _lib.check(L.ia_conformer_block_bwd_a(*a_args, sp), "ia_conformer_block_bwd_a")
        else:
            import torch.distributed as dist
            _lib.check(L.ia_conformer_block_bwd_a_phase(*a_args, 1, None, sp), "ia_conformer_block_bwd_a_phase")
            ob, og = rt.off["bn_b"][0], rt.off["bn_g"][0]
            Sg = torch.cat([rt.arena[ob:ob + d], rt.arena[og:og + d], torch.full((1,), float(N), dtype=torch.float32, device=dev)])
            fast.SYNC_BN_COLLECTIVES += 1
            dist.all_reduce(Sg, group=ctx.group)
            Sg = (Sg[:2 * d] * (float(N) / Sg[2 * d])).contiguous()
            _lib.check(L.ia_conformer_block_bwd_a_phase(*a_args, 2, _ptr(Sg), sp), "ia_conformer_block_bwd_a_phase")
        def view(buf, off, shape, dtype):
            n = 1
            for s_ in shape:
                n *= s_
            return buf[off:off + n * torch.empty(0, dtype=dtype).element_size()].view(dtype).view(*shape)
        qkv = view(arena, lay["qkv"][0], (N, 3 * d), torch.bfloat16)
        pl = view(arena, lay["pl"][0], (pe.shape[0], d), torch.bfloat16)
        ctxv = view(arena, lay["ctxv"][0], (N, d), torch.bfloat16)
        dctx = view(ws, dctx_p.value - ws.data_ptr(), (N, d), torch.bfloat16)
        lse = view(arena, lay["lse"][0], (B * att.h, T), torch.float32)
        patt = float(att.dropout_rate)
        dqkv, dpl, du, dv = fast.relpos_attention_flash_bwd(qkv, pl, att.pos_bias_u, att.pos_bias_v, lens, ctxv, dctx, lse, B, T, att.h,
                                                            att.d_k, patt, seed + 7, dub_out=(rt.pos_u, rt.pos_v))
        dx0 = torch.empty(N, d, dtype=torch.float32, device=dev)
        table, n_rows = rt.add_table() if DIRECT_ACCUMULATE else (None, 0)
        st = L.ia_conformer_block_bwd_b(ctypes.addressof(bp), ctypes.addressof(saved), ctypes.addressof(rt.grads), _ptr(x0), _ptr(pe), pe.shape[0],
                                        _ptr(dqkv), _ptr(dpl), B, T, int(seed) & 0xFFFFFFFF, _ptr(ws), n_ws, _ptr(dx0), _ptr(table),
                                        n_rows, sp)
        _lib.check(st, "ia_conformer_block_bwd_b")
        outs = []
        by_id = {id(q): (blk, sub) for q, blk, sub in rt.param_src}
        for r, q in zip(req, params):
            if not r:
                outs.append(None)
            elif DIRECT_ACCUMULATE and q.grad is not None and q.grad.dtype == torch.float32:
                outs.append(None)
            else:
                blk, sub = by_id[id(q)]
                o = rt.off[blk][0] + sub
                outs.append(rt.arena[o:o + q.numel()].view(q.shape).clone())
        return (dx0, None, None, None, None, None, None) + tuple(outs)


def conformer_block_native(x2d, layer, lens, pe_bf16, B, T, seed):
    return _ConformerBlockNativeFn.apply(x2d, layer, lens, pe_bf16, B, T, seed, *list(layer.parameters()))
```

Measured before the change: 3800 utterances/s.

## Use fused LN-FFN-residual-LN kernel in trainable Conformer block forward

Adds a training variant of the fused FFN kernel that runs layernorm, both FFN GEMMs, SiLU, dropout, the residual and the following layernorm in one launch. It also writes out the activations that backward needs (y, pre-activation, post-dropout h, x_out). Both macaron FFNs in the trainable block forward, in C and in Python, now use it by default. The aim is to cut kernel launches and the round trips of intermediates through global memory. In exchange, the kernel does extra stores and keeps more registers live. Dropout hashing and rounding are rewritten to match the unfused path bit-for-bit, which adds some ALU work.

```diff
diff --git a/include/indicasr.h b/include/indicasr.h
--- a/include/indicasr.h
+++ b/include/indicasr.h
@@ -266,6 +266,10 @@
                       const float* b1, const void* W2, const float* b2, float alpha, float p_ff, unsigned seed_ff, float p_res,
                       unsigned seed_res, const float* ln2_g, const float* ln2_b, void* y_out, int ln2_to_y_only, const void* Wt,
                       const float* bt, void* t_out, int nt, ia_stream_t stream);
+int ia_ffn_fused_train(const float* x_in, float* x_out, int N, int d, int d_ff, const float* ln_g, const float* ln_b, float eps,
+                       const void* W1, const float* b1, const void* W2, const float* b2, float alpha, float p_ff, unsigned seed_ff,
+                       float p_res, unsigned seed_res, void* y_save, void* hp_save, void* h_save, const float* ln2_g,
+                       const float* ln2_b, void* ln2_bf16, float* ln2_f32, ia_stream_t stream);
 
 typedef struct ia_block_params {
     const void *w_ff1a, *w_ff1b, *w_qkv, *w_pos, *w_out, *w_pw1, *w_pw2, *w_ff2a, *w_ff2b;
diff --git a/indic_cl_asr_amd/_lib.py b/indic_cl_asr_amd/_lib.py
--- a/indic_cl_asr_amd/_lib.py
+++ b/indic_cl_asr_amd/_lib.py
@@ -191,6 +191,8 @@
     "ia_gemm_tn_bf16": (_i, [_vp, _i, _vp, _i, _i, _i, _i, _vp, _vp, _vp, _vp]),
     "ia_ffn_fused_supported": (_i, [_i, _i]),
     "ia_ffn_fused": (_i, [_vp, _i, _i, _i, _vp, _vp, _f, _vp, _vp, _vp, _vp, _f, _f, _c.c_uint, _f, _c.c_uint, _vp, _vp, _vp, _i, _vp]),
+    "ia_ffn_fused_train": (_i, [_vp, _vp, _i, _i, _i, _vp, _vp, _f, _vp, _vp, _vp, _vp, _f, _f, _c.c_uint, _f, _c.c_uint, _vp, _vp, _vp,
+                                _vp, _vp, _vp, _vp, _vp]),
     "ia_ffn_fused_tail_supported": (_i, [_i, _i, _i]),
     "ia_ffn_fused_tail": (_i, [_vp, _i, _i, _i, _vp, _vp, _f, _vp, _vp, _vp, _vp, _f, _f, _c.c_uint, _f, _c.c_uint, _vp, _vp, _vp, _i,
                                _vp, _vp, _vp, _i, _vp]),
diff --git a/indic_cl_asr_amd/csrc/block_train.hip b/indic_cl_asr_amd/csrc/block_train.hip
--- a/indic_cl_asr_amd/csrc/block_train.hip
+++ b/indic_cl_asr_amd/csrc/block_train.hip
@@ -241,6 +241,11 @@
     return (d % 8 == 0 && d <= 1024 && d_ff % 8 == 0 && ksz <= 31 && (ksz & 1) == 1 && dk <= 64 && dk % 4 == 0 && T >= 1) ? 1 : 0;
 }
 
+static bool train_ffn_fused(int N, int d, int d_ff) {
+    const char* e = getenv("IA_TRAIN_FFN");
+    return !(e && e[0] == '0') && ia_ffn_fused_supported(d, d_ff) && (long long)N * d_ff < (1ll << 31);
+}
+
 extern "C" int ia_conformer_block_fwd(const ia_block_params* Lp, const float* x0, const void* pos_emb, int pos_rows,
                                       const int64_t* lens, int B, int T, unsigned seed, const ia_block_saved* Sp, float* out,
                                       float* dw_scratch, ia_stream_t stream) {
@@ -257,12 +262,18 @@
     const int d = L.d, d_ff = L.d_ff, H = L.n_heads, dk = d / (H > 0 ? H : 1), ksz = L.ksz, N = B * T;
     if (!ia_conformer_block_supported(d, d_ff, H, ksz, T) || pos_rows < 2 * T - 1 || L.att_window != 0 || L.att_style != 0) return IA_UNSUPPORTED;
     const float p = L.p_drop, pff = L.p_ff, patt = L.p_att;
+    const bool ffn_fused = train_ffn_fused(N, d, d_ff);
     if (phase != 2) {
+    if (ffn_fused) {
+        IA_TRY(ia_ffn_fused_train(x0, S.x1, N, d, d_ff, L.ln_ff1_g, L.ln_ff1_b, L.ln_eps, L.w_ff1a, L.b_ff1a, L.w_ff1b, L.b_ff1b, L.fc_factor,
+                                  pff, seed + 1, p, seed + 2, S.y1, S.h1p, S.h1, L.ln_att_g, L.ln_att_b, S.y2, nullptr, stream));
+    } else {
     IA_TRY(ia_layernorm(x0, d, N, d, L.ln_ff1_g, L.ln_ff1_b, L.ln_eps, nullptr, 0, nullptr, nullptr, S.y1, d, stream));
     IA_TRY(ia_gemm_bf16_ex(S.y1, d, L.w_ff1a, d, N, d_ff, d, L.b_ff1a, 1, pff, seed + 1, 1.f, nullptr, 0, nullptr, 0, S.h1, d_ff,
                            S.h1p, d_ff, nullptr, 0, stream));
     IA_TRY(ia_gemm_bf16(S.h1, d_ff, L.w_ff1b, d_ff, N, d, d_ff, L.b_ff1b, 0, p, seed + 2, L.fc_factor, x0, d, S.x1, d, nullptr, 0, stream));
     IA_TRY(ia_layernorm(S.x1, d, N, d, L.ln_att_g, L.ln_att_b, L.ln_eps, nullptr, 0, nullptr, nullptr, S.y2, d, stream));
+    }
     IA_TRY(ia_gemm_bf16(S.y2, d, L.w_qkv, d, N, 3 * d, d, L.b_qkv, 0, 0.f, 0, 1.f, nullptr, 0, nullptr, 0, S.qkv, 3 * d, stream));
     IA_TRY(ia_gemm_bf16(pos_emb, d, L.w_pos, d, pos_rows, d, d, nullptr, 0, 0.f, 0, 1.f, nullptr, 0, nullptr, 0, S.pl, d, stream));
     IA_TRY(ia_relpos_attention_flash_lse(S.qkv, S.pl, L.pos_u, L.pos_v, lens, B, T, H, dk, patt, seed + 7, S.ctxv, S.lse, stream));
@@ -282,6 +293,9 @@
                           synced ? nullptr : L.bn_nbt, L.bn_momentum, L.bn_eps, 1, S.c3, stream));
         IA_TRY(ia_gemm_bf16(S.c3, d, L.w_pw2, d, N, d, d, L.b_pw2, 0, p, seed + 4, 1.f, S.x2, d, S.x3, d, nullptr, 0, stream));
     }
+    if (ffn_fused)
+        return ia_ffn_fused_train(S.x3, S.x4, N, d, d_ff, L.ln_ff2_g, L.ln_ff2_b, L.ln_eps, L.w_ff2a, L.b_ff2a, L.w_ff2b, L.b_ff2b, L.fc_factor,
+                                  pff, seed + 5, p, seed + 6, S.y4, S.h4p, S.h4, L.ln_out_g, L.ln_out_b, nullptr, out, stream);
     IA_TRY(ia_layernorm(S.x3, d, N, d, L.ln_ff2_g, L.ln_ff2_b, L.ln_eps, nullptr, 0, nullptr, nullptr, S.y4, d, stream));
     IA_TRY(ia_gemm_bf16_ex(S.y4, d, L.w_ff2a, d, N, d_ff, d, L.b_ff2a, 1, pff, seed + 5, 1.f, nullptr, 0, nullptr, 0, S.h4, d_ff,
                            S.h4p, d_ff, nullptr, 0, stream));
diff --git a/indic_cl_asr_amd/csrc/ffn_fused.hip b/indic_cl_asr_amd/csrc/ffn_fused.hip
--- a/indic_cl_asr_amd/csrc/ffn_fused.hip
+++ b/indic_cl_asr_amd/csrc/ffn_fused.hip
@@ -29,6 +29,7 @@
     int ln2_y_only;
     int mode;
     const __bf16* Wt; const float* bt; __bf16* t_out; int nt;
+    float* x_out; __bf16* y_save; __bf16* hp_save; __bf16* h_save; float* ln2_f32;
 };
 
 __device__ __forceinline__ float half_wave_sum(float v) {
@@ -40,7 +41,7 @@
     return v;
 }
 
-template <int D, bool DROP_FF, bool DIAG, bool TAIL = false>
+template <int D, bool DROP_FF, bool DIAG, bool TAIL = false, bool TRAIN = false>
 __global__ __launch_bounds__(FF_THREADS, 2) void ffn_fused_kernel(FfnArgs a) {
     const int mode = DIAG ? a.mode : 0;
     static_assert(D == 256, "wave decomposition below is written for d_model = 256");
@@ -114,13 +115,28 @@
         const float4 x0 = *reinterpret_cast<const float4*>(a.x + (size_t)gm * D + vec * 8);
         const float4 x1 = *reinterpret_cast<const float4*>(a.x + (size_t)gm * D + vec * 8 + 4);
         float v[8] = {x0.x, x0.y, x0.z, x0.w, x1.x, x1.y, x1.z, x1.w};
-        float s = 0.f;
-#pragma unroll
-        for (int j = 0; j < 8; ++j) s += v[j];
+        float s = 0.f, qq = 0.f;
+        if constexpr (TRAIN) {
+            float sa = 0.f, sb = 0.f;
+            sa += v[0] + v[1] + v[2] + v[3];
+            sb += v[4] + v[5] + v[6] + v[7];
+            s = sa + sb;
+        } else {
+#pragma unroll
+            for (int j = 0; j < 8; ++j) s += v[j];
+        }
         const float mean = half_wave_sum(s) * (1.f / D);
-        float qq = 0.f;
-#pragma unroll
-        for (int j = 0; j < 8; ++j) { v[j] -= mean; qq += v[j] * v[j]; }
+        if constexpr (TRAIN) {
+#pragma unroll
+            for (int j = 0; j < 8; ++j) v[j] -= mean;
+            float qa = 0.f, qb = 0.f;
+            qa += v[0] * v[0] + v[1] * v[1] + v[2] * v[2] + v[3] * v[3];
+            qb += v[4] * v[4] + v[5] * v[5] + v[6] * v[6] + v[7] * v[7];
+            qq = qa + qb;
+        } else {
+#pragma unroll
+            for (int j = 0; j < 8; ++j) { v[j] -= mean; qq += v[j] * v[j]; }
+        }
         const float rstd = rsqrtf(half_wave_sum(qq) * (1.f / D) + a.eps);
         const float4 g0 = *reinterpret_cast<const float4*>(a.ln_g + vec * 8), g1 = *reinterpret_cast<const float4*>(a.ln_g + vec * 8 + 4);
         const float4 c0 = *reinterpret_cast<const float4*>(a.ln_b + vec * 8), c1 = *reinterpret_cast<const float4*>(a.ln_b + vec * 8 + 4);
@@ -131,6 +147,9 @@
         for (int j = 0; j < 8; ++j) o.h[j] = (__bf16)(v[j] * rstd * gg[j] + bb[j]);
         const int phys = (vec & 16) | ((vec & 15) ^ (r & 15));
         *reinterpret_cast<uint4*>(sY + r * YROW + phys * 16) = o.u;
+        if constexpr (TRAIN) {
+            if (m0 + r < a.N) *reinterpret_cast<uint4*>(a.y_save + (size_t)gm * D + vec * 8) = o.u;
+        }
     }
     __syncthreads();
     constexpr int KS = D / 16;
@@ -152,15 +171,39 @@
     const int w2sw = (((q * 64 + l31) >> 1) & 7);
     const unsigned char* w2row = sRing + (q * 64 + l31) * 128;
     const unsigned char* xrow = sX + (mi * 32 + l31) * XROW;
-    const unsigned gm_drop = (unsigned)(m0 + mi * 32 + l31);
+    const unsigned gm_drop = (TRAIN && m0 + mi * 32 + l31 >= a.N) ? (unsigned)(a.N - 1) : (unsigned)(m0 + mi * 32 + l31);
+    unsigned save_off = 0;
+    if constexpr (TRAIN) save_off = gm_drop * (unsigned)a.dff + (unsigned)(q * 32 + hh * 8);
+    uint2 hp_even = make_uint2(0u, 0u);
+    auto save_pair = [&](int c, int g, uint2 va, uint2 vb, __bf16* dst) {
+        typedef unsigned u2v __attribute__((ext_vector_type(2)));
+        const u2v s0 = __builtin_amdgcn_permlane32_swap(va.x, vb.x, false, false);
+        const u2v s1 = __builtin_amdgcn_permlane32_swap(va.y, vb.y, false, false);
+        *reinterpret_cast<uint4*>(dst + save_off + (unsigned)(c * FF_JC + g * 8)) = make_uint4(s0[0], s1[0], s0[1], s1[1]);
+    };
     const bool do_mfma = !(mode & 2);
     const unsigned sm_ff = ia_dm_hash32(a.seed_ff);
 
-    struct Act { float v[4]; unsigned w; };
+    struct Act { float v[4]; unsigned w; float x[TRAIN ? 4 : 1]; unsigned hp[TRAIN ? 2 : 1]; float b[TRAIN ? 4 : 1]; };
     auto act_begin = [&](int c, int g, Act& st) {
+        if constexpr (TRAIN) {
+            const unsigned baddr = (unsigned)(4 * SLOT + FF_M * XROW) + (unsigned)((c * FF_JC + q * 32 + g * 8 + hh * 4) * 4);
+            float4 bv;
+            asm volatile("ds_read_b128 %0, %1\n\ts_waitcnt lgkmcnt(0)" : "=&v"(bv) : "v"(baddr) : "memory");
+            st.b[0] = bv.x; st.b[TRAIN ? 1 : 0] = bv.y; st.b[TRAIN ? 2 : 0] = bv.z; st.b[TRAIN ? 3 : 0] = bv.w;
+            if (DROP_FF) {
+                const unsigned base = (gm_drop * (unsigned)a.dff + (unsigned)(c * FF_JC + q * 32 + g * 8)) * 0x9E3779B1u + a.seed_ff;
+                st.w = ia_dm_hash32(hh ? (base ^ 0x68E31DA4u) : base);
+            }
+        } else
         if (DROP_FF) st.w = ia_dm_word24(sm_ff, gm_drop * (unsigned)(a.dff >> 2) + (unsigned)((c * FF_JC + q * 32 + g * 8 + hh * 4) >> 2));
     };
     auto bias_init = [&](int c, f16v& acc) {
+        if constexpr (TRAIN) {
+#pragma unroll
+            for (int r = 0; r < 16; ++r) acc[r] = 0.f;
+            return;
+        }
         float4 b0, b1v, b2v, b3;
         const unsigned baddr = (unsigned)(4 * SLOT + FF_M * XROW) + (unsigned)((c * FF_JC + q * 32 + hh * 4) * 4);
         asm volatile("ds_read_b128 %0, %4\n\tds_read_b128 %1, %4 offset:32\n\tds_read_b128 %2, %4 offset:64\n\t"
@@ -176,6 +219,15 @@
             if (!(k & 1)) {
                 f2v t = {acc[4 * g + 2 * pr], acc[4 * g + 2 * pr + 1]};
                 asm volatile("" : "+v"(t));
+                if constexpr (TRAIN) {
+                    typedef __bf16 bf2v __attribute__((ext_vector_type(2)));
+                    union { bf2v h; unsigned u; } pk;
+                    t += (f2v){st.b[TRAIN ? 2 * pr : 0], st.b[TRAIN ? 2 * pr + 1 : 0]};
+                    pk.h = __builtin_convertvector(t, bf2v);
+                    st.hp[pr] = pk.u;
+                    t = (f2v){__uint_as_float(pk.u << 16), __uint_as_float(pk.u & 0xFFFF0000u)};
+                    st.x[2 * pr] = t.x; st.x[2 * pr + 1] = t.y;
+                }
                 const f2v m = t * (f2v){-1.44269504088896341f, -1.44269504088896341f};
                 f2v e = {__builtin_amdgcn_exp2f(m.x), __builtin_amdgcn_exp2f(m.y)};
                 asm volatile("" : "+v"(e));
@@ -185,7 +237,7 @@
                 asm volatile("" : "+v"(e));
                 const f2v d = e + (f2v){1.f, 1.f};
                 const f2v r = {__builtin_amdgcn_rcpf(d.x), __builtin_amdgcn_rcpf(d.y)};
-                f2v o2 = (f2v){acc[4 * g + 2 * pr], acc[4 * g + 2 * pr + 1]} * r;
+                f2v o2 = (TRAIN ? (f2v){st.x[TRAIN ? 2 * pr : 0], st.x[TRAIN ? 2 * pr + 1 : 0]} : (f2v){acc[4 * g + 2 * pr], acc[4 * g + 2 * pr + 1]}) * r;
                 asm volatile("" : "+v"(o2));
                 st.v[2 * pr] = o2.x; st.v[2 * pr + 1] = o2.y;
             }
@@ -193,7 +245,8 @@
             const int i = k - 4;
             float t = st.v[i];
             asm volatile("" : "+v"(t));
-            t = (((st.w >> (8 * i)) & 0xFFu) >= a.thr_ff) ? t : 0.f;
+            if constexpr (TRAIN) t = (((st.w >> (8 * i)) & 0xFFu) >= a.thr_ff) ? t * a.ks_ff : 0.f;
+            else t = (((st.w >> (8 * i)) & 0xFFu) >= a.thr_ff) ? t : 0.f;
             asm volatile("" : "+v"(t));
             st.v[i] = t;
         }
@@ -242,6 +295,17 @@
             out[i] = act_end(st[i]);
             asm volatile("" :: "v"(out[i].x), "v"(out[i].y));
         }
+        if constexpr (TRAIN && NG > 0) {
+            if (NG == 2) {
+                save_pair(c, g0, make_uint2(st[0].hp[0], st[0].hp[1]), make_uint2(st[NG - 1].hp[0], st[NG - 1].hp[1]), a.hp_save);
+                save_pair(c, g0, out[0], out[NG - 1], a.h_save);
+            } else if (g0 & 1) {
+                save_pair(c, g0 - 1, hp_even, make_uint2(st[0].hp[0], st[0].hp[1]), a.hp_save);
+                save_pair(c, g0 - 1, out[-1], out[0], a.h_save);
+            } else {
+                hp_even = make_uint2(st[0].hp[0], st[0].hp[1]);
+            }
+        }
     };
     const std::integral_constant<bool, false> PA{};
     const std::integral_constant<bool, true> PB{};
@@ -306,7 +370,7 @@
         const float4 e1 = *reinterpret_cast<const float4*>(sE + r * EROW + vec * 32 + 16);
         float v[8] = {e0.x, e0.y, e0.z, e0.w, e1.x, e1.y, e1.z, e1.w};
         const float4 b0 = *reinterpret_cast<const float4*>(a.b2 + vec * 8), b1 = *reinterpret_cast<const float4*>(a.b2 + vec * 8 + 4);
-        if (DROP_FF) {
+        if (DROP_FF && !TRAIN) {
 #pragma unroll
             for (int j = 0; j < 8; ++j) v[j] *= a.ks_ff;
         }
@@ -322,20 +386,46 @@
         const float4 r0 = *reinterpret_cast<const float4*>(a.x + (size_t)gmc * D + vec * 8);
         const float4 r1 = *reinterpret_cast<const float4*>(a.x + (size_t)gmc * D + vec * 8 + 4);
         const float rr[8] = {r0.x, r0.y, r0.z, r0.w, r1.x, r1.y, r1.z, r1.w};
+        if constexpr (TRAIN) {
+#pragma clang fp contract(off)
+#pragma unroll
+            for (int j = 0; j < 8; ++j) { const float t = v[j] * sc; v[j] = t + rr[j]; }
+        } else
 #pragma unroll
         for (int j = 0; j < 8; ++j) v[j] = v[j] * sc + rr[j];
+        if constexpr (TRAIN) {
+            if (live) {
+                *reinterpret_cast<float4*>(a.x_out + (size_t)gm * D + vec * 8) = make_float4(v[0], v[1], v[2], v[3]);
+                *reinterpret_cast<float4*>(a.x_out + (size_t)gm * D + vec * 8 + 4) = make_float4(v[4], v[5], v[6], v[7]);
+            }
+        } else
         if (a.ln2_y_only && live) {
             *reinterpret_cast<float4*>(a.x + (size_t)gm * D + vec * 8) = make_float4(v[0], v[1], v[2], v[3]);
             *reinterpret_cast<float4*>(a.x + (size_t)gm * D + vec * 8 + 4) = make_float4(v[4], v[5], v[6], v[7]);
         }
         if (a.ln2_g) {
-            float s = 0.f;
-#pragma unroll
-            for (int j = 0; j < 8; ++j) s += v[j];
+            float s = 0.f, qq = 0.f;
+            if constexpr (TRAIN) {
+                float sa = 0.f, sb = 0.f;
+                sa += v[0] + v[1] + v[2] + v[3];
+                sb += v[4] + v[5] + v[6] + v[7];
+                s = sa + sb;
+            } else {
+#pragma unroll
+                for (int j = 0; j < 8; ++j) s += v[j];
+            }
             const float mean = half_wave_sum(s) * (1.f / D);
-            float qq = 0.f;
-#pragma unroll
-            for (int j = 0; j < 8; ++j) { v[j] -= mean; qq += v[j] * v[j]; }
+            if constexpr (TRAIN) {
+#pragma unroll
+                for (int j = 0; j < 8; ++j) v[j] -= mean;
+                float qa = 0.f, qb = 0.f;
+                qa += v[0] * v[0] + v[1] * v[1] + v[2] * v[2] + v[3] * v[3];
+                qb += v[4] * v[4] + v[5] * v[5] + v[6] * v[6] + v[7] * v[7];
+                qq = qa + qb;
+            } else {
+#pragma unroll
+                for (int j = 0; j < 8; ++j) { v[j] -= mean; qq += v[j] * v[j]; }
+            }
             const float rstd = rsqrtf(half_wave_sum(qq) * (1.f / D) + a.eps);
             const float4 g0 = *reinterpret_cast<const float4*>(a.ln2_g + vec * 8), g1 = *reinterpret_cast<const float4*>(a.ln2_g + vec * 8 + 4);
             const float4 c0 = *reinterpret_cast<const float4*>(a.ln2_b + vec * 8), c1 = *reinterpret_cast<const float4*>(a.ln2_b + vec * 8 + 4);
@@ -351,6 +441,13 @@
         }
         if (TAIL)
             *reinterpret_cast<uint4*>(sY + r * YROW + ((vec & 16) | ((vec & 15) ^ (r & 15))) * 16) = ob.u;
+        if constexpr (TRAIN) {
+            if (live && a.ln2_g && a.ln2_f32) {
+                *reinterpret_cast<float4*>(a.ln2_f32 + (size_t)gm * D + vec * 8) = make_float4(v[0], v[1], v[2], v[3]);
+                *reinterpret_cast<float4*>(a.ln2_f32 + (size_t)gm * D + vec * 8 + 4) = make_float4(v[4], v[5], v[6], v[7]);
+            }
+            if (live && a.y_out) *reinterpret_cast<uint4*>(a.y_out + (size_t)gm * D + vec * 8) = ob.u;
+        } else
         if (live) {
             if (!a.ln2_y_only) {
                 *reinterpret_cast<float4*>(a.x + (size_t)gm * D + vec * 8) = make_float4(v[0], v[1], v[2], v[3]);
@@ -496,6 +593,7 @@
     if (ln2_to_y_only && (!ln2_g || (!y_out && !Wt))) return IA_INVALID_VALUE;
     a.ln2_g = ln2_g; a.ln2_b = ln2_b; a.y_out = (__bf16*)y_out; a.ln2_y_only = ln2_to_y_only ? 1 : 0;
     a.Wt = (const __bf16*)Wt; a.bt = bt; a.t_out = (__bf16*)t_out; a.nt = nt;
+    a.x_out = nullptr; a.y_save = nullptr; a.hp_save = nullptr; a.h_save = nullptr; a.ln2_f32 = nullptr;
     if (d_ff > 2048) return IA_UNSUPPORTED;
     const int LDS = 4 * 32768 + FF_M * FF_JC * 2 + d_ff * 4;
     static_assert(FF_M * (256 * 4 + 16) <= 4 * 32768, "epilogue tile aliases the ring");
@@ -523,3 +621,38 @@
     return IA_OK;
 }
 }
+
+extern "C" int ia_ffn_fused_train(const float* x_in, float* x_out, int N, int d, int d_ff, const float* ln_g, const float* ln_b,
+                                  float eps, const void* W1, const float* b1, const void* W2, const float* b2, float alpha,
+                                  float p_ff, unsigned seed_ff, float p_res, unsigned seed_res, void* y_save, void* hp_save,
+                                  void* h_save, const float* ln2_g, const float* ln2_b, void* ln2_bf16, float* ln2_f32,
+                                  ia_stream_t stream) {
+    if (!x_in || !x_out || !ln_g || !ln_b || !W1 || !b1 || !W2 || !b2 || !y_save || !hp_save || !h_save || N <= 0) return IA_INVALID_VALUE;
+    if ((ln2_g != nullptr) != (ln2_b != nullptr) || (!ln2_g && (ln2_bf16 || ln2_f32)) || (ln2_g && !ln2_bf16 && !ln2_f32)) return IA_INVALID_VALUE;
+    if (!ia_ffn_fused_supported(d, d_ff)) return IA_UNSUPPORTED;
+    if ((long long)N * d_ff >= (1ll << 31)) return IA_UNSUPPORTED;
+    if (p_ff < 0.f || p_ff >= 1.f || p_res < 0.f || p_res >= 1.f) return IA_INVALID_VALUE;
+    const void* al[] = {x_in, x_out, W1, W2, b1, b2, ln_g, ln_b, y_save, hp_save, h_save, ln2_g, ln2_b, ln2_bf16, ln2_f32};
+    for (const void* q : al)
+        if (q && !ia_is_aligned(q, 16)) return IA_INVALID_VALUE;
+    FfnArgs a;
+    a.x = const_cast<float*>(x_in); a.N = N; a.ln_g = ln_g; a.ln_b = ln_b; a.eps = eps;
+    a.W1 = (const __bf16*)W1; a.b1 = b1; a.W2 = (const __bf16*)W2; a.b2 = b2; a.dff = d_ff; a.alpha = alpha;
+    const ia_dropout_t drop_ff = ia_dropout_rule(p_ff), drop_res = ia_dropout_rule(p_res);
+    a.thr_ff = drop_ff.thr; a.ks_ff = drop_ff.keep_scale; a.seed_ff = seed_ff;
+    a.thr_res = drop_res.thr; a.ks_res = drop_res.keep_scale; a.seed_res = seed_res;
+    a.ln2_g = ln2_g; a.ln2_b = ln2_b; a.y_out = (__bf16*)ln2_bf16; a.ln2_y_only = 0; a.mode = 0;
+    a.Wt = nullptr; a.bt = nullptr; a.t_out = nullptr; a.nt = 0;
+    a.x_out = x_out; a.y_save = (__bf16*)y_save; a.hp_save = (__bf16*)hp_save; a.h_save = (__bf16*)h_save; a.ln2_f32 = ln2_f32;
+    const int LDS = 4 * 32768 + FF_M * FF_JC * 2 + d_ff * 4;
+    const dim3 grid((N + FF_M - 1) / FF_M), blk(FF_THREADS);
+    if (a.thr_ff > 0) {
+        IA_SET_MAX_LDS_ONCE((ffn_fused_kernel<256, true, false, false, true>), LDS);
+        hipLaunchKernelGGL((ffn_fused_kernel<256, true, false, false, true>), grid, blk, LDS, (hipStream_t)stream, a);
+    } else {
+        IA_SET_MAX_LDS_ONCE((ffn_fused_kernel<256, false, false, false, true>), LDS);
+        hipLaunchKernelGGL((ffn_fused_kernel<256, false, false, false, true>), grid, blk, LDS, (hipStream_t)stream, a);
+    }
+    IA_RETURN_IF_LAUNCH_FAILED();
+    return IA_OK;
+}
diff --git a/indic_cl_asr_amd/ops/block.py b/indic_cl_asr_amd/ops/block.py
--- a/indic_cl_asr_amd/ops/block.py
+++ b/indic_cl_asr_amd/ops/block.py
@@ -1,3 +1,5 @@
+import os
+
 import torch
 
 from .. import _lib
@@ -50,6 +52,29 @@
     _lib.check(_lib.lib().ia_silu_dropout(_ptr(h_pre), M, N, float(p), int(seed) & 0xFFFFFFFF, _ptr(out), _lib.stream_ptr()),
                "ia_silu_dropout")
     return out
+
+
+def train_ffn_fused(N, d, d_ff):
+    return (not os.environ.get("IA_TRAIN_FFN", "1").startswith("0") and bool(_lib.lib().ia_ffn_fused_supported(int(d), int(d_ff)))
+            and N * d_ff < 2 ** 31)
+
+
+def ffn_fused_train(x_in, ln, w1, b1, w2, b2, alpha, p_ff, seed_ff, p_res, seed_res, ln2=None, ln2_f32=False):
+    N, d = x_in.shape
+    dff = w1.shape[0]
+    dev = x_in.device
+    bf = lambda n: torch.empty(N, n, dtype=torch.bfloat16, device=dev)
+    y, hp, h = bf(d), bf(dff), bf(dff)
+    x_out = torch.empty(N, d, dtype=torch.float32, device=dev)
+    y2 = None if ln2 is None else torch.empty(N, d, dtype=torch.float32 if ln2_f32 else torch.bfloat16, device=dev)
+    st = _lib.lib().ia_ffn_fused_train(_ptr(x_in), _ptr(x_out), N, d, dff, _ptr(ln.weight), _ptr(ln.bias), float(ln.eps), _ptr(w1), _ptr(b1),
+                                       _ptr(w2), _ptr(b2), float(alpha), float(p_ff), int(seed_ff) & 0xFFFFFFFF, float(p_res),
+                                       int(seed_res) & 0xFFFFFFFF, _ptr(y), _ptr(hp), _ptr(h),
+                                       _ptr(ln2.weight) if ln2 is not None else None, _ptr(ln2.bias) if ln2 is not None else None,
+                                       _ptr(y2) if (ln2 is not None and not ln2_f32) else None,
+                                       _ptr(y2) if (ln2 is not None and ln2_f32) else None, _lib.stream_ptr())
+    _lib.check(st, "ia_ffn_fused_train")
+    return y, hp, h, x_out, y2
 
 
 def _silu_dropout_bwd(h_pre, dh, p, seed):
@@ -98,12 +123,17 @@
                  w1b=fast.bf16_shadow(ff2.linear1.weight), w2b=fast.bf16_shadow(ff2.linear2.weight))
         new = lambda: torch.empty(N, d, dtype=torch.float32, device=dev)
         x0 = x.contiguous()
-        y1 = fast.layernorm(x0, layer.norm_feed_forward1.weight, layer.norm_feed_forward1.bias, layer.norm_feed_forward1.eps)
-        _, h1p = fast.gemm(y1, W["w1"], ff1.linear1.bias)
-        h1 = _silu_dropout(h1p, pff1, seed + 1)
-        x1, _ = fast.gemm(h1, W["w2"], ff1.linear2.bias, dropout_p=p, seed=seed + 2, alpha=layer.fc_factor, residual=x0,
-                          out_f32=new(), want_bf16=False)
-        y2 = fast.layernorm(x1, layer.norm_self_att.weight, layer.norm_self_att.bias, layer.norm_self_att.eps)
+        ffn_fused = train_ffn_fused(N, d, W["w1"].shape[0])
+        if ffn_fused:
+            y1, h1p, h1, x1, y2 = ffn_fused_train(x0, layer.norm_feed_forward1, W["w1"], ff1.linear1.bias, W["w2"], ff1.linear2.bias,
+                                                  layer.fc_factor, pff1, seed + 1, p, seed + 2, ln2=layer.norm_self_att)
+        else:
+            y1 = fast.layernorm(x0, layer.norm_feed_forward1.weight, layer.norm_feed_forward1.bias, layer.norm_feed_forward1.eps)
+            _, h1p = fast.gemm(y1, W["w1"], ff1.linear1.bias)
+            h1 = _silu_dropout(h1p, pff1, seed + 1)
+            x1, _ = fast.gemm(h1, W["w2"], ff1.linear2.bias, dropout_p=p, seed=seed + 2, alpha=layer.fc_factor, residual=x0,
+                              out_f32=new(), want_bf16=False)
+            y2 = fast.layernorm(x1, layer.norm_self_att.weight, layer.norm_self_att.bias, layer.norm_self_att.eps)
         _, qkv = fast.gemm(y2, W["wqkv"], fast.f32_cat(att.linear_q.bias, att.linear_k.bias, att.linear_v.bias))
         _, pl = fast.gemm(pe, W["wpos"])
         if context is not None:
@@ -125,13 +155,17 @@
                                                    keep=True)
         x3, _ = fast.gemm(c3, W["wp2"], cv.pointwise_conv2.bias, dropout_p=p, seed=seed + 4, residual=x2, out_f32=new(),
                           want_bf16=False)
-        y4 = fast.layernorm(x3, layer.norm_feed_forward2.weight, layer.norm_feed_forward2.bias, layer.norm_feed_forward2.eps)
-        _, h4p = fast.gemm(y4, W["w1b"], ff2.linear1.bias)
-        h4 = _silu_dropout(h4p, pff2, seed + 5)
-        x4, _ = fast.gemm(h4, W["w2b"], ff2.linear2.bias, dropout_p=p, seed=seed + 6, alpha=layer.fc_factor, residual=x3,
-                          out_f32=new(), want_bf16=False)
-        out = new()
-        fast.layernorm(x4, layer.norm_out.weight, layer.norm_out.bias, layer.norm_out.eps, out_f32=out, want_bf16=False)
+        if ffn_fused:
+            y4, h4p, h4, x4, out = ffn_fused_train(x3, layer.norm_feed_forward2, W["w1b"], ff2.linear1.bias, W["w2b"], ff2.linear2.bias,
+                                                   layer.fc_factor, pff2, seed + 5, p, seed + 6, ln2=layer.norm_out, ln2_f32=True)
+        else:
+            y4 = fast.layernorm(x3, layer.norm_feed_forward2.weight, layer.norm_feed_forward2.bias, layer.norm_feed_forward2.eps)
+            _, h4p = fast.gemm(y4, W["w1b"], ff2.linear1.bias)
+            h4 = _silu_dropout(h4p, pff2, seed + 5)
+            x4, _ = fast.gemm(h4, W["w2b"], ff2.linear2.bias, dropout_p=p, seed=seed + 6, alpha=layer.fc_factor, residual=x3,
+                              out_f32=new(), want_bf16=False)
+            out = new()
+            fast.layernorm(x4, layer.norm_out.weight, layer.norm_out.bias, layer.norm_out.eps, out_f32=out, want_bf16=False)
         if not use_batch:
             raise RuntimeError("trainable fused block expects train-mode BatchNorm (batch statistics)")
         ctx.S = dict(x0=x0, y1=y1, h1p=h1p, h1=h1, x1=x1, y2=y2, qkv=qkv, pl=pl, ctxv=ctxv, lse=lse, x2=x2, y3=y3, c2=c2, z=z, sums=sums,
```

New measurement: 3639 utterances/s. 0.958x the previous value.
